# ziyanx02/multiagent-quadruped-environment

Hardware: AMD Instinct MI355X
Metric: env-steps/sec (agents x envs x steps/s), go1gate 4096 envs x 2 agents per GPU (higher is better)
Workload: dtype f32 (policy GEMMs and the actuator network's 32 x 32 layer: 2-plane split-f16, 22-bit)

## Files before the change

### multiagent-quadruped-environment_amd/csrc/kernels_gemm.hpp

```cpp
#pragma once
#include "mqe_common.hpp"

typedef float f32x16 __attribute__((ext_vector_type(16)));

#define GB_M 64
#define GB_N 64
#define GB_K 16

struct GemmArgs {
  const float* A; int lda; int a_rot4; int a_ring4;
  const float* Wt; int ldw;
  const float* bias;
  float* C; int ldc;
  int M, N, K;
  int act_cols;
};

__global__ void __launch_bounds__(256) k_gemm_f32(GemmArgs g) {
  __shared__ float As[GB_K][GB_M + 1];
  __shared__ float Bs[GB_K][GB_N + 4];
  const int tid = threadIdx.x, lane = tid & 63, wave = tid >> 6;
  const int wm = wave >> 1, wn = wave & 1;
  const int ntn = g.N / GB_N, ntm = (g.M + GB_M - 1) / GB_M;
  int bid = blockIdx.x;
  const int total = ntn * ntm;
  {
    const int xcd = bid & 7, slot = bid >> 3;
    const int per = (total + 7) >> 3;
    int lin = xcd * per + slot;
    if ((total & 7) == 0) bid = lin;
  }
  const int tm = bid / ntn, tn = bid - tm * ntn;
  const int m0 = tm * GB_M, n0 = tn * GB_N;
  f32x16 acc;
#pragma unroll
  for (int i = 0; i < 16; i++) acc[i] = 0.0f;
  const int am = tid >> 2, akq = (tid & 3) * 4;
  const int bk = tid >> 4, bnq = (tid & 15) * 4;
  const bool a_ok = (m0 + am) < g.M;
  const float* Arow = g.A + (size_t)(m0 + am) * g.lda;
  float4 av = make_float4(0.f, 0.f, 0.f, 0.f), bv;
  auto load_tile = [&](int k0) {
    if (a_ok) {
      int k4 = (k0 + akq) >> 2;
      if (g.a_ring4) { k4 += g.a_rot4; if (k4 >= g.a_ring4) k4 -= g.a_ring4; }
      av = *reinterpret_cast<const float4*>(Arow + (size_t)k4 * 4);
    }
    bv = *reinterpret_cast<const float4*>(g.Wt + (size_t)(k0 + bk) * g.ldw + n0 + bnq);
  };
  load_tile(0);
  for (int k0 = 0; k0 < g.K; k0 += GB_K) {
    __syncthreads();
    As[akq + 0][am] = av.x; As[akq + 1][am] = av.y; As[akq + 2][am] = av.z; As[akq + 3][am] = av.w;
    *reinterpret_cast<float4*>(&Bs[bk][bnq]) = bv;
    __syncthreads();
    if (k0 + GB_K < g.K) load_tile(k0 + GB_K);
#pragma unroll
    for (int kk = 0; kk < GB_K; kk += 2) {
      float a = As[kk + (lane >> 5)][wm * 32 + (lane & 31)];
      float b = Bs[kk + (lane >> 5)][wn * 32 + (lane & 31)];
      acc = __builtin_amdgcn_mfma_f32_32x32x2f32(a, b, acc, 0, 0, 0);
    }
  }
  const int col = n0 + wn * 32 + (lane & 31);
  const float bias = g.bias ? g.bias[col] : 0.0f;
  const bool do_act = col < g.act_cols;
#pragma unroll
  for (int r = 0; r < 16; r++) {
    int row = m0 + wm * 32 + (r & 3) + 8 * (r >> 2) + 4 * (lane >> 5);
    if (row < g.M) {
      float v = acc[r] + bias;
      if (do_act) v = v > 0 ? v : expm1f(v);
      g.C[(size_t)row * g.ldc + col] = v;
    }
  }
}

typedef _Float16 f16x8 __attribute__((ext_vector_type(8)));
typedef unsigned int h2_u32x4 __attribute__((ext_vector_type(4)));
typedef __attribute__((address_space(1))) h2_u32x4 h2_gvec;

#define H2_M 128
#define H2_N 192
#define H2_K 32
#define H2_KMULT 96
#define H2_THREADS 512
#define H2_ROWB 80
#define H2_ROWS (H2_M + H2_N)
#define H2_PLANE (H2_ROWS * H2_ROWB + 64)
#define H2_BUF (2 * H2_PLANE)
#define H2_LDS_BYTES (3 * H2_BUF)
#define H2_EPS 196
static_assert(H2_M * H2_EPS * 4 <= H2_LDS_BYTES, "epilogue staging");

struct Gemm2Args {
  const uint16_t* A; int lda; int a_rot8, a_ring8;
  const uint16_t* W; int ldw;
  const float* bias;
  float* C; int ldc;
  int M, N, K;
  int act_cols;
  float descale;
  const unsigned* irr; const float* ring; int ring_pos;
  const float* Wt32; int ldwt;
  int full_blocks, full_rows;
  long long* times; int times_blocks;
};
#define H2_STAMP(i) do { if (g.times != nullptr && threadIdx.x == 0 && (int)blockIdx.x < g.times_blocks) {                          \
    g.times[(size_t)blockIdx.x * 16 + 10 + (i)] = (long long)wall_clock64(); g.times[(size_t)blockIdx.x * 16 + 13 + (i)] = (long long)clock64(); } } while (0)
template <int TA>
__device__ __forceinline__ void gemm_h2_tile(const Gemm2Args& g, const int m0, const int n0, unsigned char* lds2) {
  constexpr int HM = 64 * TA;
  const int tid = threadIdx.x, lane = tid & 63, wave = __builtin_amdgcn_readfirstlane(tid >> 6);
  const int wm = (wave >> 1) & 1, wn = wave & 1;
  f32x16 acc00, acc01, acc02, acc10, acc11, acc12;
  H2_STAMP(0);
#pragma unroll
  for (int i = 0; i < 16; i++) { acc00[i] = 0.0f; acc01[i] = 0.0f; acc02[i] = 0.0f; acc10[i] = 0.0f; acc11[i] = 0.0f; acc12[i] = 0.0f; }
  const int stid = tid & 255, srow = stid >> 3, sc = stid & 7, sj = sc >> 1, sp = sc & 1;
  const char* Abase = reinterpret_cast<const char*>(g.A);
  const char* Wbase = reinterpret_cast<const char*>(g.W) + (size_t)n0 * g.ldw * 2;
  const unsigned a_row0 = (unsigned)min(m0 + srow, g.M - 1) * g.lda * 2, a_row1 = (unsigned)min(m0 + 32 + srow, g.M - 1) * g.lda * 2;
  const unsigned a_row2 = TA == 2 ? (unsigned)min(m0 + 64 + srow, g.M - 1) * g.lda * 2 : 0u, a_row3 = TA == 2 ? (unsigned)min(m0 + 96 + srow, g.M - 1) * g.lda * 2 : 0u;
  (void)a_row2; (void)a_row3;
  const unsigned w_row = (unsigned)srow * g.ldw * 2, w_row32 = 32u * g.ldw * 2;
  const unsigned st_ofs = sp * H2_PLANE + srow * H2_ROWB + sj * 16;
  const int frow = lane & 31, fk = (lane >> 5) * 16;
  const unsigned fa_ofs = (wm * 32 * TA + frow) * H2_ROWB + fk, fb_ofs = (H2_M + wn * 96 + frow) * H2_ROWB + fk;
  const int nkt = g.K / H2_K;
  unsigned char* buf0 = lds2;
  unsigned char* buf1 = lds2 + H2_BUF;
  unsigned char* buf2 = lds2 + 2 * H2_BUF;
  h2_u32x4 Pa0, Pa1, Pa2, Pa3, Pw0, Pw1, Pw2, Pw3, Pw4, Pw5;
  h2_u32x4 Qa0, Qa1, Qa2, Qa3, Qw0, Qw1, Qw2, Qw3, Qw4, Qw5;
  h2_u32x4 Ra0, Ra1, Ra2, Ra3, Rw0, Rw1, Rw2, Rw3, Rw4, Rw5;
  h2_u32x4 f0a00, f0a01, f0a10, f0a11, f0b00, f0b01, f0b10, f0b11, f0b20, f0b21;
  h2_u32x4 f1a00, f1a01, f1a10, f1a11, f1b00, f1b01, f1b10, f1b11, f1b20, f1b21;
  unsigned aoff, woff;
#define H2_ADDR(kt_)                                                                                            \
  {                                                                                                             \
    int kc_ = (kt_); if (kc_ > nkt - 1) kc_ = nkt - 1;           \
    woff = w_row + (unsigned)kc_ * 128u + (unsigned)sc * 16u;                                                   \
    int u_ = kc_ * 4 + sj;                                                                                      \
    if (g.a_ring8) { u_ += g.a_rot8; if (u_ >= g.a_ring8) u_ -= g.a_ring8; if (u_ >= g.a_ring8) u_ -= g.a_ring8; } \
    aoff = (unsigned)(u_ * 2 + sp) * 16u;                                                                       \
  }
#ifndef H2_LDA
#define H2_LDA(dst, i_) dst = *(const h2_gvec*)(Abase + a_row##i_ + aoff);
#endif
#ifndef H2_LDW
#define H2_LDW(dst, i_) dst = *(const h2_gvec*)(Wbase + (size_t)(i_) * w_row32 + woff);
#endif
#ifndef H2_ST
#define H2_ST(buf_, src_, r_) *reinterpret_cast<h2_u32x4*>((buf_) + st_ofs + (r_) * H2_ROWB) = src_;
#endif
#define H2_RDA(buf_, p_, t_, ks_) *reinterpret_cast<const h2_u32x4*>((buf_) + fa_ofs + (p_) * H2_PLANE + (t_) * 32 * H2_ROWB + (ks_) * 32)
#define H2_RDB(buf_, p_, u_, ks_) *reinterpret_cast<const h2_u32x4*>((buf_) + fb_ofs + (p_) * H2_PLANE + (u_) * 32 * H2_ROWB + (ks_) * 32)
#define H2_F16(x_) __builtin_bit_cast(f16x8, x_)
#ifndef H2_MFMA
#define H2_MFMA(a_, b_, c_) __builtin_amdgcn_mfma_f32_32x32x16_f16(H2_F16(a_), H2_F16(b_), c_, 0, 0, 0)
#endif
#define H2_PIN() __builtin_amdgcn_sched_barrier(0)
#if defined(H2_STAGER_TIMES) || defined(H2_MULT_TIMES)
  long long ts_prev = clock64(), ts_sum0 = 0, ts_sum1 = 0, ts_sum2 = 0, ts_sum3 = 0, tm_sum0 = 0, tm_sum1 = 0;
#endif
#ifdef H2_STAGER_TIMES
#define H2_TS(n) { const long long c_ = clock64(); ts_sum##n += c_ - ts_prev; ts_prev = c_; }
#define H2_TS_WAITV() asm volatile("s_waitcnt vmcnt(20)" ::: "memory")
#else
#define H2_TS(n)
#define H2_TS_WAITV()
#endif
#ifdef H2_MULT_TIMES
#define H2_TM(n) { const long long c_ = clock64(); tm_sum##n += c_ - ts_prev; ts_prev = c_; }
#else
#define H2_TM(n)
#endif
  if constexpr (TA == 2) {
#include "kernels_gemm_h2_loop.inc"
  } else {
#include "kernels_gemm_h2_loop_half.inc"
  }
#if defined(H2_STAGER_TIMES) || defined(H2_MULT_TIMES)
  if (g.times != nullptr && lane == 0 && (int)blockIdx.x < g.times_blocks) {
    long long* o = g.times + (size_t)blockIdx.x * 16;
    if (wave == 4) { o[0] = ts_sum0; o[1] = ts_sum1; o[2] = ts_sum2; o[3] = ts_sum3; }
    if (wave == 0) { o[4] = tm_sum0; o[5] = tm_sum1; }
  }
#endif
#undef H2_TS
#undef H2_TS_WAITV
#undef H2_TM
#undef H2_ADDR
#undef H2_LDA
#undef H2_LDW
#undef H2_ST
#undef H2_RDA
#undef H2_RDB
#undef H2_F16
#undef H2_MFMA
#undef H2_PIN
  H2_STAMP(1);
  __syncthreads();
  float* ep = reinterpret_cast<float*>(lds2);
#define H2_EPW(acc_, t_, u_)                                                                                    \
  _Pragma("unroll") for (int r = 0; r < 16; r++)                                                                \
    ep[(wm * 32 * TA + (t_) * 32 + (r & 3) + 8 * (r >> 2) + 4 * (lane >> 5)) * H2_EPS + wn * 96 + (u_) * 32 + (lane & 31)] = acc_[r];
  if (wave < 4) {
    H2_EPW(acc00, 0, 0) H2_EPW(acc01, 0, 1) H2_EPW(acc02, 0, 2)
    if constexpr (TA == 2) { H2_EPW(acc10, 1, 0) H2_EPW(acc11, 1, 1) H2_EPW(acc12, 1, 2) }
  }
#undef H2_EPW
  __syncthreads();
  constexpr int EP_IT = (HM * H2_N / 4) / H2_THREADS;
  float4 bbs[EP_IT];
  unsigned mks[EP_IT];
#pragma unroll
  for (int it = 0; it < EP_IT; it++) {
    const int i = it * H2_THREADS + tid, row = i / (H2_N / 4), c4 = i - row * (H2_N / 4);
    bbs[it] = g.bias ? *reinterpret_cast<const float4*>(g.bias + n0 + c4 * 4) : make_float4(0.f, 0.f, 0.f, 0.f);
    mks[it] = g.irr && m0 + row < g.M ? g.irr[m0 + row] : 0u;
  }
#pragma unroll
  for (int it = 0; it < EP_IT; it++) {
    const int i = it * H2_THREADS + tid, row = i / (H2_N / 4), c4 = i - row * (H2_N / 4);
    const int col = n0 + c4 * 4, grow = m0 + row;
    float4 v = *reinterpret_cast<const float4*>(ep + row * H2_EPS + c4 * 4);
    const float4 bb = bbs[it];
    v.x = fmaf(v.x, g.descale, bb.x); v.y = fmaf(v.y, g.descale, bb.y); v.z = fmaf(v.z, g.descale, bb.z); v.w = fmaf(v.w, g.descale, bb.w);
    unsigned mk = mks[it];
    if (mk) {
      float4 cr = make_float4(0.f, 0.f, 0.f, 0.f);
      do {
        const int s1 = __ffs((int)mk) - 1;
        mk &= mk - 1;
        const int p = s1 >= g.ring_pos ? s1 - g.ring_pos : s1 + MQE_HIST - g.ring_pos;
        if (p == 0) continue;
        const int s0 = s1 > 0 ? s1 - 1 : MQE_HIST - 1;
        const float* a2 = g.ring + ((size_t)grow * MQE_HIST + s1) * MQE_FRAME + 54;
        const float* a1 = g.ring + ((size_t)grow * MQE_HIST + s0) * MQE_FRAME + 42;
        const float* wr = g.Wt32 + (size_t)(p * MQE_FRAME + 54) * g.ldwt + col;
#pragma unroll 4
        for (int j = 0; j < 12; j++) {
          const float r = a2[j] - a1[j];
          const float4 w = *reinterpret_cast<const float4*>(wr + (size_t)j * g.ldwt);
          cr.x = fmaf(r, w.x, cr.x); cr.y = fmaf(r, w.y, cr.y); cr.z = fmaf(r, w.z, cr.z); cr.w = fmaf(r, w.w, cr.w);
        }
      } while (mk);
      v.x += cr.x; v.y += cr.y; v.z += cr.z; v.w += cr.w;
    }
    if (col < g.act_cols) {
      v.x = v.x > 0 ? v.x : __expf(v.x) - 1.0f; v.y = v.y > 0 ? v.y : __expf(v.y) - 1.0f;
      v.z = v.z > 0 ? v.z : __expf(v.z) - 1.0f; v.w = v.w > 0 ? v.w : __expf(v.w) - 1.0f;
    }
    if (grow < g.M) {
#ifdef H2_PLAIN_STORE
      *reinterpret_cast<float4*>(g.C + (size_t)grow * g.ldc + col) = v;
#else
      typedef float h2_f4 __attribute__((ext_vector_type(4)));
      h2_f4 nv; nv.x = v.x; nv.y = v.y; nv.z = v.z; nv.w = v.w;
      __builtin_nontemporal_store(nv, reinterpret_cast<h2_f4*>(g.C + (size_t)grow * g.ldc + col));
#endif
    }
  }
  H2_STAMP(2);
}
__global__ void __launch_bounds__(H2_THREADS, 1) k_gemm_h2(Gemm2Args g) {
  extern __shared__ __attribute__((aligned(16))) unsigned char lds2[];
  const int ntn = g.N / H2_N, ntm = (g.M + H2_M - 1) / H2_M;
  int bid = blockIdx.x;
  const int total = ntn * ntm;
  if ((total & 7) == 0) { const int xcd = bid & 7, slot = bid >> 3; bid = xcd * (total >> 3) + slot; }
  const int tm = bid / ntn, tn = bid - tm * ntn;
  gemm_h2_tile<2>(g, tm * H2_M, tn * H2_N, lds2);
}
__global__ void __launch_bounds__(H2_THREADS, 1) k_gemm_h2_mix(Gemm2Args g) {
  extern __shared__ __attribute__((aligned(16))) unsigned char lds2[];
  const int ntn = g.N / H2_N;
  int bid = blockIdx.x;
  if (bid < g.full_blocks) {
    const int total = g.full_blocks;
    if ((total & 7) == 0) { const int xcd = bid & 7, slot = bid >> 3; bid = xcd * (total >> 3) + slot; }
    const int tm = bid / ntn, tn = bid - tm * ntn;
    gemm_h2_tile<2>(g, tm * H2_M, tn * H2_N, lds2);
  } else {
    bid -= g.full_blocks;
    const int total = (int)gridDim.x - g.full_blocks;
    if ((total & 7) == 0) { const int xcd = bid & 7, slot = bid >> 3; bid = xcd * (total >> 3) + slot; }
    const int tm = bid / ntn, tn = bid - tm * ntn;
    gemm_h2_tile<1>(g, g.full_rows + tm * (H2_M / 2), tn * H2_N, lds2);
  }
}
```

### multiagent-quadruped-environment_amd/csrc/kernels_step.hpp

```cpp
#pragma once
#include <type_traits>
#include "mqe_common.hpp"

__device__ __forceinline__ void quat_rotate_inverse_f(const float* q, const float* v, float* o) {
  float qw = q[3];
  float s = 2.0f * qw * qw - 1.0f;
  float cx = q[1] * v[2] - q[2] * v[1], cy = q[2] * v[0] - q[0] * v[2], cz = q[0] * v[1] - q[1] * v[0];
  float dt = q[0] * v[0] + q[1] * v[1] + q[2] * v[2];
  o[0] = v[0] * s - cx * qw * 2.0f + q[0] * dt * 2.0f;
  o[1] = v[1] * s - cy * qw * 2.0f + q[1] * dt * 2.0f;
  o[2] = v[2] * s - cz * qw * 2.0f + q[2] * dt * 2.0f;
}
__device__ __forceinline__ float wrap2pi(float a) {
  const float T = 6.2831855f;
  float r = fmodf(a, T);
  if (r < 0) r += T;
  return r;
}
__device__ __forceinline__ void euler_xyz_f(const float* q, float* rpy) {
  float x = q[0], y = q[1], z = q[2], w = q[3];
  float sinr = 2.0f * (w * x + y * z), cosr = w * w - x * x - y * y + z * z;
  float sinp = 2.0f * (w * y - z * x);
  float siny = 2.0f * (w * z + x * y), cosy = w * w + x * x - y * y - z * z;
  float roll = atan2f(sinr, cosr);
  float pitch = fabsf(sinp) >= 1.0f ? copysignf(1.5707964f, sinp) : asinf(sinp);
  float yaw = atan2f(siny, cosy);
  rpy[0] = wrap2pi(roll); rpy[1] = wrap2pi(pitch); rpy[2] = wrap2pi(yaw);
}

__device__ __forceinline__ float mqe_rand(const DevModel* m, int env, int count, uint32_t k, float lo, float hi) {
  float u = mqe_u01((uint32_t)m->seed, (uint32_t)(env + m->env_id_offset), (uint32_t)count, k);
  return (hi - lo) * u + lo;
}

__device__ __forceinline__ float div_ieee(float a, float b) { return b != 0.0f ? a / b : (a > 0.0f ? 3.0e38f : (a < 0.0f ? -3.0e38f : 0.0f)); }
__device__ __forceinline__ float atan_ratio(float a, float b) { return b != 0.0f ? atanf(a / b) : (a > 0.0f ? 1.5707964f : (a < 0.0f ? -1.5707964f : 0.0f)); }

__device__ __forceinline__ void defender_command_dev(const DevModel* m, const DevState& st, int e, float* cmd3) {
  int A = m->A, P = m->P;
  const float* root = st.root + (size_t)e * (A + P) * 13;
  const float* dp = root + 2 * 13;
  const float* bp = root + A * 13;
  float gate[3] = {as_global(m->gate_pos)[e * 2], as_global(m->gate_pos)[e * 2 + 1], as_global(m->env_origins)[e * 3 + 2]};
  float tp[3];
  for (int k = 0; k < 3; k++) tp[k] = 0.6f * bp[k] + 0.4f * gate[k];
  float yaw = st.obs_bag[(size_t)(e * A + 2) * MQE_OBS_BAG + 5];
  float yaw_to_gate = 3.1415927f + atan_ratio(gate[1] - dp[1], gate[0] - dp[0]);
  float yc = clampf(yaw_to_gate - yaw, -0.3f, 0.3f) / 0.3f;
  float tdg = sqrtf((tp[0] - gate[0]) * (tp[0] - gate[0]) + (tp[1] - gate[1]) * (tp[1] - gate[1]));
  float ddg = sqrtf((dp[0] - gate[0]) * (dp[0] - gate[0]) + (dp[1] - gate[1]) * (dp[1] - gate[1]));
  float xc = clampf(tdg - ddg, -0.5f, 0.5f);
  float yy = -clampf(gate[1] + div_ieee((tp[1] - gate[1]) * (dp[0] - gate[0]), tp[0] - gate[0]) - dp[1], -0.5f, 0.5f);
  cmd3[0] = xc; cmd3[1] = yy; cmd3[2] = yc;
}

__global__ void k_defender_command(const DevModel* m, DevState st, float* out) {
  int e = blockIdx.x * blockDim.x + threadIdx.x;
  if (e >= m->N) return;
  float c[3];
  defender_command_dev(m, st, e, c);
  out[e * 3] = c[0]; out[e * 3 + 1] = c[1]; out[e * 3 + 2] = c[2];
}

__global__ void k_wrapper_command(const DevModel* m, DevState st, const float* __restrict__ actions) {
  int e = blockIdx.x * blockDim.x + threadIdx.x;
  if (e >= m->N) return;
  int A = m->A, Aw = m->Aw;
  const float scale[3] = {2.0f, 0.5f, 0.5f};
  for (int a = 0; a < Aw; a++)
    for (int k = 0; k < 3; k++) {
      float v = actions[((size_t)e * Aw + a) * 3 + k];
      if (m->task != MQE_TASK_TUG) v = clampf(v, -1.0f, 1.0f);
      st.cmd[((size_t)e * A + a) * 3 + k] = m->task == MQE_TASK_PLAIN ? v : v * scale[k];
    }
  if (m->task == MQE_TASK_FOOTBALL_DEFENDER) defender_command_dev(m, st, e, st.cmd + ((size_t)e * A + 2) * 3);
}

struct PreVal { float v, aux; unsigned mk; };
__device__ __forceinline__ PreVal pre_policy_load(const DevModel* m, const DevState& st, const float* __restrict__ command, int hist_slot,
                                                  const float* __restrict__ wrapper_actions, int i, int c) {
  const float* ob = st.obs_bag + (size_t)i * MQE_OBS_BAG;
  PreVal r; r.aux = 0.0f; r.mk = 0u;
  const bool cmd_col = c >= 3 && (c < 6 || (c < 18 && m->cmd_general));
  const float* src = nullptr;
  if (c < 3) src = ob + 60 + c;
  else if (c < 18) src = cmd_col ? nullptr : m->command_obs + c;
  else if (c < 42) src = ob + (c - 12);
  else if (c < 54) src = st.last_loco + (size_t)i * 12 + (c - 42);
  else if (c < 66) src = st.last_two_loco + (size_t)i * 12 + (c - 54);
  else if (c < 70) src = ob + (c - 3);
  float v = src != nullptr ? *src : 0.0f;
  if (cmd_col && m->cmd_general) {
    const int srcc = m->cmd_src[c];
    if (srcc < 0) v = m->command_obs[c];
    else {
      float x = command[(size_t)i * m->cmd_dims + srcc];
      if (m->clip_command) x = clampf(x, -1.0f, 1.0f);
      v = x * m->cmd_scale[c];
    }
  } else if (cmd_col) {
    float x;
    if (wrapper_actions) {
      const int A = m->A, Aw = m->Aw, e = i / A, a = i - e * A, k = c - 3;
      if (m->task == MQE_TASK_FOOTBALL_DEFENDER && a == 2) {
        float c3[3];
        defender_command_dev(m, st, e, c3);
        x = c3[k];
      } else if (a < Aw) {
        float w = wrapper_actions[((size_t)e * Aw + a) * 3 + k];
        if (m->task != MQE_TASK_TUG) w = clampf(w, -1.0f, 1.0f);
        x = m->task == MQE_TASK_PLAIN ? w : w * (k == 0 ? 2.0f : 0.5f);
      } else x = st.cmd[i * 3 + k];
      r.aux = x;
    } else x = command[i * 3 + (c - 3)];
    if (m->clip_command) x = clampf(x, -1.0f, 1.0f);
    v = x * (c < 5 ? m->cmd_lin_scale : m->cmd_ang_scale);
  }
  if (c >= 54 && c < 66 && st.hist2) {
    const int oldest = hist_slot + 1 >= MQE_HIST ? 0 : hist_slot + 1;
    r.aux = st.hist[((size_t)i * MQE_HIST + oldest) * MQE_FRAME + c];
  }
  if (c == 71 && st.hist2) {
    const int prev = hist_slot > 0 ? hist_slot - 1 : MQE_HIST - 1;
    const float* pa = st.hist + ((size_t)i * MQE_HIST + prev) * MQE_FRAME + 42;
    const float* na = st.last_two_loco + (size_t)i * 12;
    unsigned diff = 0;
#pragma unroll
    for (int j = 0; j < 12; j++) diff |= __float_as_uint(pa[j]) ^ __float_as_uint(na[j]);
    const unsigned bit = 1u << hist_slot;
    const unsigned mk = st.hist_irr[i];
    r.mk = diff ? (mk | bit) : (mk & ~bit);
  }
  r.v = v;
  return r;
}
__device__ __forceinline__ void pre_policy_store(const DevModel* m, const DevState& st, int hist_slot, bool have_wrapper_actions, int i, int c, const PreVal& r) {
  const float v = r.v;
  st.loco_obs[(size_t)i * MQE_FRAME + c] = v;
  st.hist[((size_t)i * MQE_HIST + hist_slot) * MQE_FRAME + c] = v;
  if (have_wrapper_actions && c >= 3 && c < 6) st.cmd[i * 3 + (c - 3)] = r.aux;
  if (st.hist2) {
    const int cc = c < 70 ? h2_col(c) : (c == 70 ? MQE_H2_FLAG_COL : -1);
    uint16_t* row2 = st.hist2 + (size_t)i * (2 * MQE_HIST * MQE_H2_FRAME);
    if (cc >= 0) {
      uint16_t h, l;
      split2(c < 70 ? v : 1.0f, MQE_H2_ASCALE, h, l);
      const size_t k = (size_t)hist_slot * MQE_H2_FRAME + cc;
      row2[h2_index(k, 0)] = h; row2[h2_index(k, 1)] = l;
    } else if (cc == -2) {
      const int oldest = hist_slot + 1 >= MQE_HIST ? 0 : hist_slot + 1;
      int slot = oldest + MQE_H2_CARRIER0 + (c - 54); if (slot >= MQE_HIST) slot -= MQE_HIST;
      uint16_t h, l;
      split2(r.aux, MQE_H2_ASCALE, h, l);
      const size_t k = (size_t)slot * MQE_H2_FRAME + MQE_H2_CARRIER_COL;
      row2[h2_index(k, 0)] = h; row2[h2_index(k, 1)] = l;
    } else if (c == 71) st.hist_irr[i] = r.mk;
  }
}
__device__ __forceinline__ void pre_policy_element(const DevModel* m, const DevState& st, const float* __restrict__ command, int hist_slot,
                                                   const float* __restrict__ wrapper_actions, int i, int c) {
  const PreVal r = pre_policy_load(m, st, command, hist_slot, wrapper_actions, i, c);
  pre_policy_store(m, st, hist_slot, wrapper_actions != nullptr, i, c, r);
}

__global__ void __launch_bounds__(256) k_pre_policy(const DevModel* m, DevState st, const float* __restrict__ command, int hist_slot,
                                                    const float* __restrict__ wrapper_actions) {
  const int lane = threadIdx.x & 63;
  const int i = blockIdx.x * (blockDim.x >> 6) + (threadIdx.x >> 6);
  if (i >= m->R) return;
  const int A = m->A, Aw = m->Aw, task = m->task, clip_command = m->clip_command;
  const float lin = m->cmd_lin_scale, ang = m->cmd_ang_scale;
  const int e = i / A, a = i - e * A;
  const bool wrap = wrapper_actions != nullptr;
  if (m->cmd_general || (wrap && task == MQE_TASK_FOOTBALL_DEFENDER && a == 2)) {
    pre_policy_element(m, st, command, hist_slot, wrapper_actions, i, lane);
    if (lane < MQE_FRAME - 64) pre_policy_element(m, st, command, hist_slot, wrapper_actions, i, 64 + lane);
    return;
  }
  const bool h2 = st.hist2 != nullptr;
  const float* ob = st.obs_bag + (size_t)i * MQE_OBS_BAG;
  const int oldest = hist_slot + 1 >= MQE_HIST ? 0 : hist_slot + 1, prev = hist_slot > 0 ? hist_slot - 1 : MQE_HIST - 1;
  const float* hist_i = st.hist + (size_t)i * MQE_HIST * MQE_FRAME;
  const unsigned mk = h2 ? st.hist_irr[i] : 0u;
  float x1[2], x2[2], x3[2], x4[2];
  bool on[2], cmdc[2], actc[2];
  int cc[2];
#pragma unroll
  for (int q = 0; q < 2; q++) {
    const int c = q * 64 + lane;
    cc[q] = c;
    on[q] = c < MQE_FRAME;
    cmdc[q] = c >= 3 && c < 6;
    actc[q] = c >= 54 && c < 66;
    const float* a1 = ob;
    if (c < 3) a1 = ob + 60 + c;
    else if (c < 6) a1 = ob;
    else if (c < 18) a1 = m->command_obs + c;
    else if (c < 42) a1 = ob + (c - 12);
    else if (c < 54) a1 = st.last_loco + (size_t)i * 12 + (c - 42);
    else if (c < 66) a1 = st.last_two_loco + (size_t)i * 12 + (c - 54);
    else if (c < 70) a1 = ob + (c - 3);
    const float* a2 = ob;
    if (cmdc[q]) a2 = wrap ? (a < Aw ? wrapper_actions + ((size_t)e * Aw + a) * 3 + (c - 3) : st.cmd + i * 3 + (c - 3)) : command + i * 3 + (c - 3);
    const float* a3 = ob;
    const float* a4 = ob;
    if (actc[q] && h2) { a3 = hist_i + oldest * MQE_FRAME + c; a4 = hist_i + prev * MQE_FRAME + (c - 12); }
    x1[q] = on[q] ? *a1 : 0.0f; x2[q] = on[q] ? *a2 : 0.0f; x3[q] = on[q] ? *a3 : 0.0f; x4[q] = on[q] ? *a4 : 0.0f;
  }
  PreVal r[2];
  bool differs = false;
#pragma unroll
  for (int q = 0; q < 2; q++) {
    const int c = cc[q];
    float v = (c < 70 && !cmdc[q]) ? x1[q] : 0.0f;
    r[q].aux = 0.0f; r[q].mk = 0u;
    if (cmdc[q]) {
      float x = x2[q];
      if (wrap) {
        if (a < Aw) {
          if (task != MQE_TASK_TUG) x = clampf(x, -1.0f, 1.0f);
          x = task == MQE_TASK_PLAIN ? x : x * (c == 3 ? 2.0f : 0.5f);
        }
        r[q].aux = x;
      }
      if (clip_command) x = clampf(x, -1.0f, 1.0f);
      v = x * (c < 5 ? lin : ang);
    }
    if (actc[q] && h2) {
      r[q].aux = x3[q];
      differs = differs || (on[q] && __float_as_uint(x4[q]) != __float_as_uint(x1[q]));
    }
    r[q].v = v;
  }
  const bool diff = __ballot(differs) != 0ull;
  const unsigned bit = 1u << hist_slot;
  if (lane == MQE_FRAME - 1 - 64) r[1].mk = diff ? (mk | bit) : (mk & ~bit);
  pre_policy_store(m, st, hist_slot, wrap, i, lane, r[0]);
  if (lane < MQE_FRAME - 64) pre_policy_store(m, st, hist_slot, wrap, i, 64 + lane, r[1]);
}

__global__ void k_post_policy(const DevModel* m, DevState st, const float* __restrict__ act, int ld) {
  int idx = blockIdx.x * blockDim.x + threadIdx.x;
  if (idx >= m->R * 12) return;
  int i = idx / 12, k = idx - i * 12;
  float a = act[(size_t)i * ld + k];
  st.last_two_loco[idx] = st.last_loco[idx];
  st.last_loco[idx] = a;
  st.actions[idx] = clampf(a, -m->clip_actions, m->clip_actions);
}

__global__ void k_body_l0_finish(float* __restrict__ P1, int ldp, int col0, int ncols, const float* __restrict__ lat, int ldl,
                                 const float* __restrict__ w_lat0, const float* __restrict__ w_lat1, int R) {
  int idx = blockIdx.x * blockDim.x + threadIdx.x;
  if (idx >= R * ncols) return;
  int i = idx / ncols, c = idx - i * ncols;
  float v = P1[(size_t)i * ldp + col0 + c];
  v = fmaf(lat[(size_t)i * ldl], w_lat0[c], v);
  v = fmaf(lat[(size_t)i * ldl + 1], w_lat1[c], v);
  P1[(size_t)i * ldp + col0 + c] = v > 0 ? v : expm1f(v);
}


struct LagSlots { size_t rd, wr; };
__device__ __forceinline__ LagSlots lag_slots(int pos, int lag_steps, size_t R12, size_t idx) {
  const int rd = pos + 1 >= lag_steps + 1 ? 0 : pos + 1;
  return {(size_t)rd * R12 + idx, (size_t)pos * R12 + idx};
}
__device__ __forceinline__ float lag_target(const DevModel* m, const DevState& st, size_t idx, float as, int pos) {
  if (m->lag_steps <= 0) return as;
  const LagSlots s = lag_slots(pos, m->lag_steps, (size_t)m->R * 12, idx);
  st.lag_buf[s.wr] = as;
  return st.lag_buf[s.rd];
}
__device__ __forceinline__ float joint_pd_torque(int ctrl, float asc, float q, float qd, const float* last_qd, int j, const DevModel* m) {
  float tau = asc;
  if (ctrl == MQE_CTRL_P) tau = m->kp * (asc + m->default_dof_pos[j] - q) - m->kd * qd;
  else if (ctrl == MQE_CTRL_V) tau = m->kp * (asc - qd) - m->kd * (qd - *last_qd) / m->dt;
  return tau;
}
__device__ __forceinline__ void substep_log(const DevModel* m, float* sub_dof_vel, uint8_t* sub_exceed, size_t o, int j, float q, float qd) {
  sub_dof_vel[o] = qd;
  sub_exceed[o] = (uint8_t)((q < m->soft_lo[j]) | (q > m->soft_hi[j]));
}

__global__ void __launch_bounds__(256) k_compute_torques(const DevModel* m, DevState st, int dec_i, int lag_pos) {
  int idx = blockIdx.x * blockDim.x + threadIdx.x;
  int R = m->R, A = m->A;
  if (idx >= R * 12) return;
  int i = idx / 12, j = idx - i * 12;
  int env = i / A, a = i - env * A;
  const float* ds = st.dof + ((size_t)env * m->ND + a * 12 + j) * 2;
  float q = ds[0], qd = ds[1];
  float as = st.actions[idx] * m->action_scale;
  const int ctrl = m->control_type;
  float tau;
  if (ctrl == MQE_CTRL_P || ctrl == MQE_CTRL_V || ctrl == MQE_CTRL_T) tau = joint_pd_torque(ctrl, as, q, qd, st.last_dof_vel + idx, j, m);
  else tau = 0.0f;
  float lim = m->torque_limits[j];
  tau = clampf(tau, -lim, lim);
  st.torques[idx] = tau;
  if (dec_i >= 0) st.sub_tau[((size_t)env * 4 + dec_i) * 12 * A + a * 12 + j] = tau;
}

__global__ void __launch_bounds__(256) k_compute_torques_mfma(const DevModel* m, DevState st, int dec_i, int lag_pos) {
  const int lane = threadIdx.x & 63, wave = threadIdx.x >> 6;
  const int j32 = lane & 31, h = lane >> 5;
  const int R = m->R, A = m->A;
  const int nj = R * 12;
  const int idx = (blockIdx.x * 4 + wave) * 32 + j32;
  const bool valid = idx < nj;
  const int ii = valid ? idx : nj - 1;
  const int i = ii / 12, j = ii - i * 12;
  const int env = i / A, a = i - env * A;
  float* e1 = st.act_hist; float* e2 = e1 + (size_t)R * 12; float* v1 = e2 + (size_t)R * 12; float* v2 = v1 + (size_t)R * 12;
  const float* ds = st.dof + ((size_t)env * m->ND + a * 12 + j) * 2;
  const float q = ds[0], qd = ds[1];
  float as = st.actions[ii] * m->action_scale;
  if (j % 3 == 0) as *= m->hip_scale_reduction;
  const float err = q - (lag_target(m, st, (size_t)ii, as, lag_pos) + m->default_dof_pos[j]);
  const float x1 = e1[ii], x2 = e2[ii], x4 = v1[ii], x5 = v2[ii];
  ActNet w;
  if (m->act_f16) act_load<true>(m, lane, h, w); else act_load<false>(m, lane, h, w);
  const mqe_f32x16 s1 = act_layer1(w, err, x1, x2, qd, x4, x5, h);
  const mqe_f32x16 acc2 = m->act_f16 ? act_layer2<true>(w, s1) : act_layer2<false>(w, s1);
  float tau = act_out(w, acc2);
  if (valid && h == 0) {
    e2[idx] = x1; e1[idx] = err;
    v2[idx] = x4; v1[idx] = qd;
    const float lim = m->torque_limits[j];
    tau = clampf(tau, -lim, lim);
    st.torques[idx] = tau;
    if (dec_i >= 0) st.sub_tau[((size_t)env * 4 + dec_i) * 12 * A + a * 12 + j] = tau;
  }
}


__device__ __forceinline__ unsigned robot_frame(const DevModel* m, const float* rs, const float* gpar, float gi0, const float* f3, float aoz, float dtp,
                                                float* lv, float* av, float* pgr, float* clk, float& gi1, float* rpy) {
  const float q[4] = {rs[3], rs[4], rs[5], rs[6]}, v[3] = {rs[7], rs[8], rs[9]}, w[3] = {rs[10], rs[11], rs[12]};
  const float g3[3] = {0.0f, 0.0f, -1.0f};
  quat_rotate_inverse_f(q, v, lv);
  quat_rotate_inverse_f(q, w, av);
  quat_rotate_inverse_f(q, g3, pgr);
  const float f = gpar[0], ph = gpar[1], off = gpar[2], bnd = gpar[3], dur = gpar[4];
  float gi = gi0 + dtp * f;
  gi = gi - floorf(gi);
  gi1 = gi;
  float fi[4] = {gi + ph + off + bnd, gi + off, gi + bnd, gi + ph};
#pragma unroll
  for (int k = 0; k < 4; k++) {
    const float r = fi[k] - floorf(fi[k]);
    if (r < dur) fi[k] = r * (0.5f / dur);
    else if (r > dur) fi[k] = 0.5f + (r - dur) * (0.5f / (1.0f - dur));
    clk[k] = sinf(6.2831855f * fi[k]);
  }
  unsigned fl = 0;
  if (m->terminate_on_base_contact && sqrtf(f3[0] * f3[0] + f3[1] * f3[1] + f3[2] * f3[2]) > 1.0f) fl |= 1u;
  euler_xyz_f(q, rpy);
  float r = rpy[0], p = rpy[1];
  if (r > 3.1415927f) r -= 6.2831855f;
  if (p > 3.1415927f) p -= 6.2831855f;
  const float z = rs[2] - aoz;
  if ((m->termination_flags & MQE_TERM_ROLL) && fabsf(r) > m->roll_thr) fl |= 2u;
  if ((m->termination_flags & MQE_TERM_PITCH) && fabsf(p) > m->pitch_thr) fl |= 4u;
  if ((m->termination_flags & MQE_TERM_Z_HIGH) && z > m->zhigh_thr) fl |= 8u;
  if ((m->termination_flags & MQE_TERM_Z_LOW) && z < m->zlow_thr) fl |= 16u;
  return fl;
}
__device__ __forceinline__ void env_flags_store(const DevModel* m, const DevState& st, int e, int ep, unsigned fl, uint8_t to, uint8_t reset) {
  st.ep_len[e] = ep;
  st.time_out[e] = to;
  if (m->termination_flags & MQE_TERM_ROLL) st.r_term[e] = (fl >> 1) & 1;
  if (m->termination_flags & MQE_TERM_PITCH) st.p_term[e] = (fl >> 2) & 1;
  if (m->termination_flags & MQE_TERM_Z_HIGH) st.zh_term[e] = (fl >> 3) & 1;
  st.reset_buf[e] = reset;
  st.wdone[e] = reset;
  if (m->terminate_on_base_contact) st.collide_buf[e] = reset;
}
__device__ __forceinline__ void robot_frame_store(const DevState& st, int i, const float* lv, const float* av, const float* pgr, const float* bq, const float* clk, float gi) {
#pragma unroll
  for (int k = 0; k < 3; k++) { st.blv[i * 3 + k] = lv[k]; st.bav[i * 3 + k] = av[k]; st.pg[i * 3 + k] = pgr[k]; }
#pragma unroll
  for (int k = 0; k < 4; k++) { st.bquat[i * 4 + k] = bq[k]; st.clock[i * 4 + k] = clk[k]; }
  st.gait[i] = gi;
}
__device__ __forceinline__ void push_robots(const DevModel* m, float* root, int e, int A, int push_count) {
  for (int b = 0; b < A; b++) {
    float* rv = root + b * 13 + 7;
    rv[0] = mqe_rand(m, e, (int)(MQE_RNG_PUSH + (uint32_t)push_count), (uint32_t)(2 * b), -m->max_push, m->max_push);
    rv[1] = mqe_rand(m, e, (int)(MQE_RNG_PUSH + (uint32_t)push_count), (uint32_t)(2 * b + 1), -m->max_push, m->max_push);
  }
}
__device__ __forceinline__ void obs_row_axis(float* ob, int k, float pos, float origin, float rpy, float lv, float av, float pg) {
  ob[k] = pos - origin; ob[3 + k] = rpy;
  ob[30 + k] = lv * 2.0f; ob[33 + k] = av * 0.25f; ob[60 + k] = pg;
}
__device__ __forceinline__ void obs_row_joint(const DevModel* m, float* ob, int j, float q, float qd, float act, float last_act) {
  ob[6 + j] = (q - m->default_dof_pos[j]) * 1.0f;
  ob[18 + j] = qd * 0.05f;
  ob[36 + j] = act;
  ob[48 + j] = last_act;
}
__device__ __forceinline__ void obs_row_quad(float* ob, int k, float clk, float bq) { ob[63 + k] = clk; ob[67 + k] = bq; }
constexpr int HIST_F4 = MQE_HIST * MQE_FRAME / 4;
constexpr int HIST2_U4 = 2 * MQE_HIST * MQE_H2_FRAME / 8;
__device__ __forceinline__ void zero_env_history(const DevModel* m, const DevState& st, int e, int t, int stride) {
  const int per = m->A * HIST_F4;
  float4* h4 = reinterpret_cast<float4*>(st.hist) + (size_t)e * per;
  for (int k = t; k < per; k += stride) h4[k] = make_float4(0.f, 0.f, 0.f, 0.f);
  if (st.hist2) {
    uint4* p4 = reinterpret_cast<uint4*>(st.hist2 + (size_t)e * m->A * (HIST2_U4 * 8));
    const int per2 = m->A * HIST2_U4;
    for (int k = t; k < per2; k += stride) p4[k] = make_uint4(0u, 0u, 0u, 0u);
#pragma unroll
    for (int a0 = 0; a0 < MQE_MAX_AGENTS; a0 += stride)
      if (t + a0 < m->A) st.hist_irr[(size_t)e * m->A + t + a0] = 0u;
  }
}

__device__ __forceinline__ void compute_observations_env(const DevModel* m, const DevState& st, int e, int in_step) {
  int A = m->A;
  for (int a = 0; a < A; a++) {
    int i = e * A + a;
    float* ob = st.obs_bag + (size_t)i * MQE_OBS_BAG;
    const float* rs = st.root + ((size_t)e * (A + m->P) + a) * 13;
    const float* ds = st.dof + ((size_t)e * m->ND + a * 12) * 2;
    float rpy[3];
    euler_xyz_f(st.bquat + i * 4, rpy);
    for (int k = 0; k < 3; k++) obs_row_axis(ob, k, rs[k], as_global(m->env_origins)[e * 3 + k], rpy[k], st.blv[i * 3 + k], st.bav[i * 3 + k], st.pg[i * 3 + k]);
    for (int j = 0; j < 12; j++) {
      float act = st.actions[i * 12 + j];
      obs_row_joint(m, ob, j, ds[2 * j], ds[2 * j + 1], act, in_step ? act : st.last_actions[i * 12 + j]);
    }
    for (int k = 0; k < 4; k++) obs_row_quad(ob, k, st.clock[i * 4 + k], st.bquat[i * 4 + k]);
  }
}

__global__ void __launch_bounds__(256) k_curriculum_snapshot(const DevModel* m, DevState st) {
  const int e = blockIdx.x * blockDim.x + threadIdx.x;
  if (e >= m->N) return;
  const float* rs = st.root + ((size_t)(e / m->A) * (m->A + m->P) + e % m->A) * 13;
  st.curr_xy[e * 2] = rs[0]; st.curr_xy[e * 2 + 1] = rs[1];
}
__device__ __forceinline__ void curriculum_move_dev(const DevModel* m, const DevState& st, int e) {
  const float dx = st.curr_xy[e * 2] - st.env_origins_live[e * 3], dy = st.curr_xy[e * 2 + 1] - st.env_origins_live[e * 3 + 1];
  const float distance = sqrtf(dx * dx + dy * dy);
  const int move_up = distance > m->terrain_env_length / 2 ? 1 : 0;
  int lvl = st.terrain_levels[e] + move_up;
  if (lvl >= m->terrain_rows) lvl = (int)(mqe_u01((uint32_t)m->seed, (uint32_t)(e + m->env_id_offset), (uint32_t)st.reset_count[e], 250u) * (float)m->terrain_rows);
  else if (lvl < 0) lvl = 0;
  if (lvl >= m->terrain_rows) lvl = m->terrain_rows - 1;
  st.terrain_levels[e] = lvl;
  for (int k = 0; k < 3; k++) st.env_origins_live[e * 3 + k] = as_global(m->terrain_origins)[((size_t)lvl * m->terrain_cols + as_global(m->terrain_types)[e]) * 3 + k];
}

__device__ __forceinline__ void reset_env_dev(const DevModel* m, const DevState& st, int e) {
  int A = m->A, P = m->P;
  float* root = st.root + (size_t)e * (A + P) * 13;
  float* dofs = st.dof + (size_t)e * m->ND * 2;
  int cnt = st.reset_count[e];
  if (m->curriculum) curriculum_move_dev(m, st, e);
  for (int a = 0; a < A; a++)
    for (int j = 0; j < 12; j++) {
      float ratio = mqe_rand(m, e, cnt, (uint32_t)(a * 12 + j), m->dof_ratio_lo, m->dof_ratio_hi);
      dofs[(a * 12 + j) * 2] = m->default_dof_pos[j] * ratio;
      dofs[(a * 12 + j) * 2 + 1] = 0.0f;
    }
  for (int k = 12 * A; k < m->ND; k++) { dofs[k * 2] = m->seesaw_default_angle; dofs[k * 2 + 1] *= 0.0f; }
  for (int a = 0; a < A; a++) {
    float* rs = root + a * 13;
    for (int k = 0; k < 13; k++) rs[k] = as_global(m->base_init)[a * 13 + k];
    for (int k = 0; k < 3; k++) rs[k] += as_global(m->agent_origins)[((size_t)e * A + a) * 3 + k];
  }
  for (int p = 0; p < P; p++) {
    float* rs = root + (A + p) * 13;
    for (int k = 0; k < 13; k++) rs[k] = as_global(m->npc_init)[p * 13 + k];
    for (int k = 0; k < 3; k++) rs[k] += st.env_origins_live[e * 3 + k];
  }
  if (m->has_base_pos_range)
    for (int a = 0; a < A; a++) {
      root[a * 13 + 0] += mqe_rand(m, e, cnt, (uint32_t)(64 + a), m->base_pos_x_lo, m->base_pos_x_hi);
      root[a * 13 + 1] += mqe_rand(m, e, cnt, (uint32_t)(72 + a), m->base_pos_y_lo, m->base_pos_y_hi);
    }
  if (m->has_npc_pos_range)
    for (int p = 0; p < P; p++) {
      root[(A + p) * 13 + 0] += mqe_rand(m, e, cnt, (uint32_t)(128 + p), m->npc_pos_x_lo, m->npc_pos_x_hi);
      root[(A + p) * 13 + 1] += mqe_rand(m, e, cnt, (uint32_t)(160 + p), m->npc_pos_y_lo, m->npc_pos_y_hi);
    }
  for (int a = 0; a < A; a++)
    for (int c = 0; c < 6; c++) root[a * 13 + 7 + c] = mqe_rand(m, e, cnt, (uint32_t)(80 + a * 6 + c), m->base_vel_lo, m->base_vel_hi);
  for (int k = 0; k < 12 * A; k++) st.last_actions[(size_t)e * 12 * A + k] = 0.0f;
  st.ep_len[e] = 0;
  st.reset_buf[e] = 1;
  st.wdone[e] = 1;
  for (int a = 0; a < A; a++) st.gait[e * A + a] = 0.0f;
  st.reset_count[e] = cnt + 1;
}

__device__ __forceinline__ float mqe_randn(const DevModel* m, int e, int step_no, uint32_t k) {
  const uint32_t cnt = MQE_RNG_NPC + (uint32_t)step_no, genv = (uint32_t)(e + m->env_id_offset);
  const float u1 = mqe_u01((uint32_t)m->seed, genv, cnt, 2u * k), u2 = mqe_u01((uint32_t)m->seed, genv, cnt, 2u * k + 1u);
  return sqrtf(-2.0f * logf(1.0f - u1)) * cosf(6.2831855f * u2);
}

typedef const __attribute__((address_space(3))) float* lds_cptr;
template <class NP>
__device__ __forceinline__ void sheep_flock_mean(const DevModel* m, NP npc_rows, float* avg) {
  const int P = m->P;
  avg[0] = 0; avg[1] = 0; avg[2] = 0;
  for (int p = 0; p < P; p++) for (int k = 0; k < 3; k++) avg[k] += npc_rows[p * 13 + k];
  for (int k = 0; k < 3; k++) avg[k] /= (float)P;
}
template <class NP>
__device__ __forceinline__ void sheep_flock_stats(const DevModel* m, const DevState& st, int e, NP npc_rows, const float* avg) {
  const int P = m->P;
  float var = 0;
  for (int k = 0; k < 2; k++) {
    float acc = 0;
    for (int p = 0; p < P; p++) { float t = npc_rows[p * 13 + k] - avg[k]; acc += t * t; }
    var += acc / (float)P;
  }
  st.sheep_avg[e * 2] = avg[0]; st.sheep_avg[e * 2 + 1] = avg[1];
  st.sheep_var[e] = var;
}
template <class NP, class RP>
__device__ __forceinline__ void sheep_increment(const DevModel* m, const DevState& st, int e, int p, NP npc_rows, RP rob_rows, const float* avg, int step_no, float* dv) {
  const int A = m->A, P = m->P;
  NP sp = npc_rows + p * 13;
  for (int k = 0; k < 3; k++) {
    const float z = m->noise_mode == MQE_NOISE_SCRIPTED ? st.npc_noise[((size_t)e * P + p) * 3 + k]
                                                        : (m->sheep_rand != 0.0f ? mqe_randn(m, e, step_no, (uint32_t)(p * 3 + k)) : 0.0f);
    dv[k] = m->sheep_rand * z * 2.0f;
  }
  if (P != 1) {
    float rel[3] = {avg[0] - sp[0], avg[1] - sp[1], avg[2] - sp[2]};
    float nr = sqrtf(rel[0] * rel[0] + rel[1] * rel[1] + rel[2] * rel[2]);
    if (nr > 0.0f) for (int k = 0; k < 3; k++) dv[k] += m->sheep_rand * rel[k] / nr / 1.5f;
  }
  for (int a = 0; a < A; a++) {
    RP dp = rob_rows + a * 13;
    float rel[3] = {sp[0] - dp[0], sp[1] - dp[1], sp[2] - dp[2]};
// ... 211 lines not shown
    }
    if (task == MQE_TASK_GATE || task == MQE_TASK_SHEEP || task == MQE_TASK_PUSHBOX) { o[c++] = gp0; o[c++] = gp1; }
    if (task == MQE_TASK_PUSHBOX) {
      o[c++] = npc[0] - eol[0]; o[c++] = npc[1] - eol[1];
      for (int k = 0; k < 4; k++) o[c++] = npc[3 + k];
    }
    if (task == MQE_TASK_SHEEP)
      for (int p = 0; p < P; p++) { o[c++] = npc[p * 13] - eo0; o[c++] = npc[p * 13 + 1] - eo1; }
    if (task == MQE_TASK_FOOTBALL_DEFENDER) {
      for (int k = 0; k < 3; k++) o[c++] = npc[k] - eol[k];
      for (int k = 0; k < 3; k++) o[c++] = npc[7 + k];
    }
  }
  if (early) return;
  if (task == MQE_TASK_TUG) {
    float* nd = st.dof + ((size_t)e * m->ND + 12 * A) * 2;
    const float npos = nd[0];
    bag_ptr ob0 = bag;
    bag_ptr ob1 = bag + (1) * MQE_OBS_BAG;
    const float x0 = ob0[0], y0 = ob0[1], x1 = ob1[0], y1 = ob1[1];
    if (is_reset_call) {
      st.w_last[e * MQE_MAX_AGENTS] = x0; st.w_last[e * MQE_MAX_AGENTS + 1] = y0;
      st.w_last2[e * 2] = npos;
      st.w_delayed_reset[e] = 0;
      for (int a = 0; a < Aw; a++) rew[a] = 0;
      return;
    }
    const float last_npc = st.w_last2[e * 2];
    const float lx = st.w_last[e * MQE_MAX_AGENTS] - 1.6f, ly = st.w_last[e * MQE_MAX_AGENTS + 1] - npos;
    const float cx = x0 - 1.6f, cy = y0 - npos;
    const float last_dis = sqrtf(lx * lx + ly * ly), dis = sqrtf(cx * cx + cy * cy);
    float r0 = 0.0f, sr = 0.0f, pu = 0.0f, pr = 0.0f, pp = 0.0f;
    if (sc[0] != 0) { if (npos < 0) sr = sc[0] * -npos; if (last_npc <= npos) sr /= 2; r0 += sr; rs[0] += sr; }
    if (sc[1] != 0) { if (npos > 0) pu = sc[1] * npos; if (last_npc > npos) pu /= 2; r0 -= pu; rs[1] += pu; }
    if (sc[2] != 0) { if (dis < last_dis) pr = (last_dis - dis) * sc[2]; r0 += pr; rs[2] += pr; }
    if (sc[3] != 0) { if (dis >= last_dis) pp = powf(2.0f, dis) * sc[3]; r0 -= pp; rs[3] += pp; }
    rs[4] += npos; rs[5] += pr + sr - pu; rs[6] += x0; rs[7] += y0; rs[8] += x1; rs[9] += y1;
    st.w_last[e * MQE_MAX_AGENTS] = x0; st.w_last[e * MQE_MAX_AGENTS + 1] = y0;
    st.w_last2[e * 2] = npos;
    rew[0] = r0;
    for (int a = 1; a < Aw; a++) rew[a] = 0;
    if (side_effects) {
      uint8_t cnt = st.reset_buf[e] ? 2 : st.w_delayed_reset[e];
      if (cnt > 0) { nd[0] = 0.0f; nd[1] = 0.0f; cnt--; }
      st.w_delayed_reset[e] = cnt;
    }
    return;
  }
  if (task == MQE_TASK_BRIDGE) {
    bag_ptr ob0 = bag;
    bag_ptr ob1 = bag + (1) * MQE_OBS_BAG;
    const float x0 = ob0[0], z0 = ob0[2], x1 = ob1[0], z1 = ob1[2];
    float S = st.w_last[e * MQE_MAX_AGENTS], tgt = st.w_last[e * MQE_MAX_AGENTS + 1];
    if (is_reset_call) {
      S = fabsf(x1 + x0); tgt = x1;
      st.w_last[e * MQE_MAX_AGENTS] = S; st.w_last[e * MQE_MAX_AGENTS + 1] = tgt;
    }
    float* o1 = obs + 1 * D;
    o1[0] = S - o1[0]; o1[4] = -o1[4]; o1[6] = S - o1[6]; o1[10] = -o1[10];
    if (is_reset_call) { for (int a = 0; a < Aw; a++) rew[a] = 0; return; }
    float r0 = 0.0f;
    if (sc[0] != 0 && z1 < 0.5f) { r0 += sc[0]; rs[0] += sc[0]; }
    if (sc[1] != 0 && z0 < 0.5f) { r0 -= sc[1]; rs[1] += sc[1]; }
    if (sc[2] != 0 && x0 > tgt) { r0 += sc[2]; rs[2] += sc[2]; }
    rew[0] = r0;
    for (int a = 1; a < Aw; a++) rew[a] = 0;
    return;
  }
  if (task == MQE_TASK_WRESTLING) {
    float* o1 = obs + 1 * D;
    o1[1] = -o1[1]; o1[4] = -o1[4]; o1[7] = -o1[7]; o1[10] = -o1[10];
    if (is_reset_call) { for (int a = 0; a < Aw; a++) rew[a] = 0; return; }
    float r0 = 0.0f;
    bool down0, down1;
    {
      bag_ptr ob = bag;
      float r = ob[3], p = ob[4];
      if (r > 3.1415927f) r -= 6.2831855f;
      if (p > 3.1415927f) p -= 6.2831855f;
      down0 = fabsf(p) > 3.1415927f * 0.9f || fabsf(r) >= 3.1415927f * 0.4f;
      ob += MQE_OBS_BAG;
      r = ob[3]; p = ob[4];
      if (r > 3.1415927f) r -= 6.2831855f;
      if (p > 3.1415927f) p -= 6.2831855f;
      down1 = fabsf(p) > 3.1415927f * 0.9f || fabsf(r) >= 3.1415927f * 0.4f;
    }
    if (sc[0] != 0 && down1) { r0 += sc[0]; rs[0] += sc[0]; }
    if (sc[1] != 0 && down0) { r0 -= sc[1]; rs[1] += sc[1]; }
    rew[0] = r0;
    for (int a = 1; a < Aw; a++) rew[a] = 0;
    return;
  }
  if (task == MQE_TASK_ROTATION) {
    float* o1 = obs + 1 * D;
    o1[1] = -o1[1]; o1[4] = -o1[4]; o1[7] = -o1[7]; o1[10] = -o1[10];
    const float tgt = m->wrapper_param[0];
    bag_ptr ob0 = bag;
    bag_ptr ob1 = bag + (1) * MQE_OBS_BAG;
    const float x0 = ob0[0], y0 = ob0[1], x1 = ob1[0];
    if (is_reset_call) {
      st.w_last[e * MQE_MAX_AGENTS] = sqrtf((x0 - tgt) * (x0 - tgt) + y0 * y0);
      for (int a = 0; a < Aw; a++) rew[a] = 0;
      return;
    }
    float r0 = 0.0f;
    if (sc[0] != 0 && x0 > tgt) { r0 += sc[0]; rs[0] += sc[0]; }
    if (sc[1] != 0 && x1 > tgt) { r0 -= sc[1]; rs[1] += sc[1]; }
    if (sc[2] != 0) {
      const float dis = sqrtf((x0 - tgt) * (x0 - tgt) + (y0 - tgt) * (y0 - tgt));
      if (dis < st.w_last[e * MQE_MAX_AGENTS]) { r0 += sc[2]; rs[2] += sc[2]; }
      st.w_last[e * MQE_MAX_AGENTS] = dis;
    }
    rew[0] = r0;
    for (int a = 1; a < Aw; a++) rew[a] = 0;
    return;
  }
  for (int a = 0; a < Aw; a++) rew[a] = 0;
}

#ifndef POST_EPW
#define POST_EPW 8
#endif

__device__ __forceinline__ void post_flush_rows(float* __restrict__ g, const float* lds, const int n, const int tid) {
  const int n4 = n >> 2;
  for (int i = tid; i < n4; i += 64) reinterpret_cast<float4*>(g)[i] = reinterpret_cast<const float4*>(lds)[i];
  for (int i = (n4 << 2) + tid; i < n; i += 64) g[i] = lds[i];
}

template <int AM, int PEPW, bool LDS_STATE = false>
__device__ __forceinline__ void post_body(const DevModel* m, const DevState& st, const int blk, const int tid, float* s_bag, float* s_la, float* s_npc,
                                          int wrapper_level, int push_count, int step_no,
                                          const float* root_l = nullptr, const float* dof_l = nullptr, const float* act_l = nullptr, int lds_env_stride = 0, int act_env_stride = 0,
                                          const int npc_stride = MQE_MAX_NPCS * 13, long long* taps = nullptr) {
  static_assert(PEPW * AM <= 64 && (PEPW & (PEPW - 1)) == 0, "agent lanes of PEPW envs must fit one wavefront");
#define ETAP(i) do { if (taps != nullptr && tid == 0) taps[i] = (long long)wall_clock64(); } while (0)
  const int A = m->A, P = m->P;
  const int le = tid & (PEPW - 1), a = tid / PEPW;
  const int e = blk * PEPW + le;
  const bool mine = e < m->N && a < A;
  const bool lead = e < m->N && a == 0;
  const int i = e * A + a;
  const int nrow = min(PEPW, m->N - blk * PEPW) * A;
  const float dtp = m->dt * (float)m->decimation;
  float* root = st.root + (size_t)e * (A + P) * 13;
  float* bag = s_bag + le * A * MQE_OBS_BAG;
  typedef typename std::conditional<LDS_STATE, lds_cptr, const float*>::type state_ptr;
  state_ptr root_src;
  if constexpr (LDS_STATE) root_src = (lds_cptr)(root_l + le * lds_env_stride); else root_src = root;
  float* la = s_la + le * A * 12;
  float rs[13], gpar[5], gi0 = 0.f, f3[3], aoz = 0.f, dq[24], act[12], eo[3];
  int ep = 0;
  if (mine) {
    ep = st.ep_len[e] + 1;
#pragma unroll
    for (int k = 0; k < 3; k++) eo[k] = as_global(m->env_origins)[e * 3 + k];
#pragma unroll
    for (int k = 0; k < 13; k++) rs[k] = root_src[a * 13 + k];
    const float* lo = st.loco_obs + (size_t)i * MQE_FRAME;
#pragma unroll
    for (int k = 0; k < 5; k++) gpar[k] = lo[7 + k];
    gi0 = st.gait[i];
    const float* cf3 = st.cf + ((size_t)e * m->NBR + a * MQE_NREP) * 3;
#pragma unroll
    for (int k = 0; k < 3; k++) f3[k] = cf3[k];
    aoz = as_global(m->agent_origins)[(size_t)i * 3 + 2];
    state_ptr ds, as;
    if constexpr (LDS_STATE) { ds = (lds_cptr)(dof_l + le * lds_env_stride + a * 24); as = (lds_cptr)(act_l + le * act_env_stride + a * 12); }
    else { ds = st.dof + ((size_t)e * m->ND + a * 12) * 2; as = st.actions + (size_t)i * 12; }
#pragma unroll
    for (int k = 0; k < 24; k++) dq[k] = ds[k];
#pragma unroll
    for (int k = 0; k < 12; k++) act[k] = as[k];
  }
  float bq[4], lv[3], av[3], pgr[3], clk[4], gi1 = 0.f;
  float rpy[3] = {0.f, 0.f, 0.f};
  unsigned fl = 0;
  if (mine) {
#pragma unroll
    for (int k = 0; k < 4; k++) bq[k] = rs[3 + k];
    fl = robot_frame(m, rs, gpar, gi0, f3, aoz, dtp, lv, av, pgr, clk, gi1, rpy);
  }
  ETAP(2);
#pragma unroll
  for (int d = PEPW; d < PEPW * AM; d <<= 1) fl |= (unsigned)__shfl_xor((int)fl, d);
  const uint8_t to = ep > m->max_episode_length;
  const uint8_t reset = (uint8_t)(mine && (fl != 0 || to));
  if (lead) env_flags_store(m, st, e, ep, fl, to, reset);
  if (mine) robot_frame_store(st, i, lv, av, pgr, bq, clk, gi1);
  ETAP(3);
  float* npc_pre = s_npc + le * npc_stride;
  {
    const int e0 = blk * PEPW, nenv = min(PEPW, m->N - e0), per = P * 13;
    for (int t = tid; t < nenv * per; t += 64) {
      const int sl = t / per, r = t - sl * per;
      if constexpr (LDS_STATE) s_npc[sl * npc_stride + r] = ((lds_cptr)(root_l + sl * lds_env_stride))[A * 13 + r];
      else s_npc[sl * npc_stride + r] = st.root[((size_t)(e0 + sl) * (A + P) + A) * 13 + r];
    }
    __syncthreads();
  }
  ETAP(4);
  if (m->npc_kind == MQE_NPC_SHEEP) {
    constexpr int LPE = 64 / PEPW, NPASS = (MQE_MAX_NPCS + LPE - 1) / LPE;
    float dvs[NPASS][3];
    if (e < m->N) {
      float avg[3];
      sheep_flock_mean(m, (lds_cptr)npc_pre, avg);
      if (lead) sheep_flock_stats(m, st, e, (lds_cptr)npc_pre, avg);
#pragma unroll
      for (int q = 0; q < NPASS; q++)
        if (a + q * LPE < P) sheep_increment(m, st, e, a + q * LPE, (lds_cptr)npc_pre, root_src, avg, step_no, dvs[q]);
    }
    __syncthreads();
    if (e < m->N) {
#pragma unroll
      for (int q = 0; q < NPASS; q++)
        if (a + q * LPE < P) sheep_apply(root, A, a + q * LPE, (lds_cptr)npc_pre, dvs[q]);
    }
    __threadfence_block();
    __syncthreads();
  }
  ETAP(5);
  if (lead) {
    if (reset) {
      reset_env_dev(m, st, e);
      for (int k = 0; k < P * 13; k++) npc_pre[k] = root[A * 13 + k];
    }
  }
  if (__ballot(reset != 0)) {
    __threadfence_block();
    __syncthreads();
    if (reset) {
#pragma unroll
      for (int k = 0; k < 13; k++) rs[k] = root[a * 13 + k];
      const float* ds = st.dof + ((size_t)e * m->ND + a * 12) * 2;
#pragma unroll
      for (int k = 0; k < 24; k++) dq[k] = ds[k];
      if (P == 0) {
#pragma unroll
        for (int k = 0; k < 4; k++) { bq[k] = rs[3 + k]; st.bquat[i * 4 + k] = bq[k]; }
        euler_xyz_f(bq, rpy);
      }
    }
  }
  ETAP(6);
  if (mine) {
    float* ob = bag + a * MQE_OBS_BAG;
#pragma unroll
    for (int k = 0; k < 3; k++) obs_row_axis(ob, k, rs[k], eo[k], rpy[k], lv[k], av[k], pgr[k]);
#pragma unroll
    for (int j = 0; j < 12; j++) obs_row_joint(m, ob, j, dq[2 * j], dq[2 * j + 1], act[j], act[j]);
#pragma unroll
    for (int k = 0; k < 4; k++) obs_row_quad(ob, k, clk[k], bq[k]);
#pragma unroll
    for (int k = 71; k < MQE_OBS_BAG; k++) ob[k] = 0.0f;
#pragma unroll
    for (int j = 0; j < 12; j++) {
      la[a * 12 + j] = act[j];
      la[PEPW * AM * 12 + a * 12 + j] = dq[2 * j + 1];
    }
  }
  __syncthreads();
  ETAP(7);
  if (lead) {
    wrapper_env_dev<true>(m, st, e, 0, npc_pre, wrapper_level, bag);
    if (push_count > 0 && !reset) push_robots(m, root, e, A, push_count);
  }
  ETAP(8);
  {
    const size_t r0 = (size_t)blk * PEPW * A;
    post_flush_rows(st.obs_bag + r0 * MQE_OBS_BAG, s_bag, nrow * MQE_OBS_BAG, tid);
    post_flush_rows(st.last_actions + r0 * 12, s_la, nrow * 12, tid);
    post_flush_rows(st.last_dof_vel + r0 * 12, s_la + PEPW * AM * 12, nrow * 12, tid);
  }
  ETAP(9);
  unsigned long long rm = __ballot(lead && reset != 0);
  while (rm) {
    const int l = __ffsll((long long)rm) - 1;
    rm &= rm - 1;
    zero_env_history(m, st, blk * PEPW + l, tid, 64);
  }
}

template <int AM>
__global__ void __launch_bounds__(64) k_post_physics(const DevModel* m, DevState st, int wrapper_level, int push_count, int step_no) {
  __shared__ float4 s_bag4[POST_EPW * AM * MQE_OBS_BAG / 4], s_la4[POST_EPW * AM * 24 / 4];
  __shared__ float s_npc[POST_EPW * MQE_MAX_NPCS * 13];
  post_body<AM, POST_EPW>(m, st, blockIdx.x, threadIdx.x, reinterpret_cast<float*>(s_bag4), reinterpret_cast<float*>(s_la4), s_npc, wrapper_level, push_count, step_no);
}

__global__ void k_reset_history(const DevModel* m, DevState st) {
  int idx = blockIdx.x * blockDim.x + threadIdx.x;
  int i = idx / HIST_F4;
  if (i >= m->R) return;
  if (!st.reset_buf[i / m->A]) return;
  reinterpret_cast<float4*>(st.hist)[idx] = make_float4(0.f, 0.f, 0.f, 0.f);
  if (st.hist2) {
    const int w = idx - i * HIST_F4;
    if (w < HIST2_U4) reinterpret_cast<uint4*>(st.hist2)[(size_t)i * HIST2_U4 + w] = make_uint4(0u, 0u, 0u, 0u);
    if (w == 0) st.hist_irr[i] = 0u;
  }
}

__global__ void k_hist2_rebuild(const DevModel* m, DevState st, int oldest) {
  const int idx = blockIdx.x * blockDim.x + threadIdx.x;
  const int i = idx / MQE_HIST, slot = idx - i * MQE_HIST;
  if (i >= m->R || !st.hist2) return;
  const float* fr = st.hist + ((size_t)i * MQE_HIST + slot) * MQE_FRAME;
  uint16_t* row2 = st.hist2 + (size_t)i * (2 * MQE_HIST * MQE_H2_FRAME);
  unsigned any = 0u;
  for (int c = 0; c < 70; c++) {
    const float v = fr[c];
    any |= __float_as_uint(v) & 0x7FFFFFFFu;
    const int cc = h2_col(c);
    if (cc >= 0) {
      uint16_t h, l;
      split2(v, MQE_H2_ASCALE, h, l);
      const size_t k = (size_t)slot * MQE_H2_FRAME + cc;
      row2[h2_index(k, 0)] = h; row2[h2_index(k, 1)] = l;
    }
  }
  uint16_t h, l;
  split2(any ? 1.0f : 0.0f, MQE_H2_ASCALE, h, l);
  size_t k = (size_t)slot * MQE_H2_FRAME + MQE_H2_FLAG_COL;
  row2[h2_index(k, 0)] = h; row2[h2_index(k, 1)] = l;
  int p = slot - oldest; if (p < 0) p += MQE_HIST;
  float carry = 0.0f;
  if (p >= MQE_H2_CARRIER0 && p < MQE_H2_CARRIER0 + 12) carry = st.hist[((size_t)i * MQE_HIST + oldest) * MQE_FRAME + 54 + (p - MQE_H2_CARRIER0)];
  split2(carry, MQE_H2_ASCALE, h, l);
  k = (size_t)slot * MQE_H2_FRAME + MQE_H2_CARRIER_COL;
  row2[h2_index(k, 0)] = h; row2[h2_index(k, 1)] = l;
  const int prev = slot > 0 ? slot - 1 : MQE_HIST - 1;
  const float* pa = st.hist + ((size_t)i * MQE_HIST + prev) * MQE_FRAME + 42;
  unsigned diff = 0u;
  for (int j = 0; j < 12; j++) diff |= __float_as_uint(pa[j]) ^ __float_as_uint(fr[54 + j]);
  if (diff) atomicOr(&st.hist_irr[i], 1u << slot);
}

__global__ void __launch_bounds__(64) k_post_staged(const DevModel* m, DevState st, int stages, int wrapper_level, int push_count, int step_no) {
  const int e = blockIdx.x * blockDim.x + threadIdx.x;
  if (e >= m->N) return;
  const int A = m->A, P = m->P;
  float* root = st.root + (size_t)e * (A + P) * 13;
  float* npc_pre = st.npc_pre + (size_t)e * (P ? P : 1) * 13;
  const float dtp = m->dt * (float)m->decimation;
  if (stages & MQE_POST_FRAME) {
    const int ep = st.ep_len[e] + 1;
    unsigned fl = 0;
    for (int a = 0; a < A; a++) {
      const int i = e * A + a;
      float rs[13], lv[3], av[3], pgr[3], clk[4], rpy[3], gi;
      for (int k = 0; k < 13; k++) rs[k] = root[a * 13 + k];
      fl |= robot_frame(m, rs, st.loco_obs + (size_t)i * MQE_FRAME + 7, st.gait[i], st.cf + ((size_t)e * m->NBR + a * MQE_NREP) * 3,
                        as_global(m->agent_origins)[(size_t)i * 3 + 2], dtp, lv, av, pgr, clk, gi, rpy);
      robot_frame_store(st, i, lv, av, pgr, rs + 3, clk, gi);
    }
    const uint8_t to = ep > m->max_episode_length;
    env_flags_store(m, st, e, ep, fl, to, (uint8_t)(fl != 0 || to));
    for (int k = 0; k < P * 13; k++) npc_pre[k] = root[A * 13 + k];
  }
  if ((stages & MQE_POST_NPC) && m->npc_kind == MQE_NPC_SHEEP) {
    float avg[3], dvs[MQE_MAX_NPCS][3];
    const float* nrows = root + A * 13;
    sheep_flock_mean(m, nrows, avg);
    sheep_flock_stats(m, st, e, nrows, avg);
    for (int p = 0; p < P; p++) sheep_increment(m, st, e, p, nrows, (const float*)root, avg, step_no, dvs[p]);
    for (int p = 0; p < P; p++) sheep_apply(root, A, p, nrows, dvs[p]);
  }
  if (stages & MQE_POST_RESET) {
    const uint8_t reset = st.reset_buf[e];
    st.wdone[e] = reset;
    if (m->terminate_on_base_contact) st.collide_buf[e] = reset;
    if (reset) {
      reset_env_dev(m, st, e);
      for (int k = 0; k < P * 13; k++) npc_pre[k] = root[A * 13 + k];
      if (P == 0)
        for (int a = 0; a < A; a++) for (int k = 0; k < 4; k++) st.bquat[(e * A + a) * 4 + k] = root[a * 13 + 3 + k];
      zero_env_history(m, st, e, 0, 1);
    }
  }
  if (stages & MQE_POST_OBS) {
    compute_observations_env(m, st, e, 1);
    for (int k = 0; k < 12 * A; k++) {
      st.last_actions[(size_t)e * 12 * A + k] = st.actions[(size_t)e * 12 * A + k];
      st.last_dof_vel[(size_t)e * 12 * A + k] = st.dof[((size_t)e * m->ND + k) * 2 + 1];
    }
  }
  if (stages & MQE_POST_WRAPPER) {
    wrapper_env_dev(m, st, e, 0, npc_pre, wrapper_level);
    if (push_count > 0 && !st.reset_buf[e]) push_robots(m, root, e, A, push_count);
  }
}

__global__ void __launch_bounds__(64) k_reset_all(const DevModel* m, DevState st, int no_post_step_yet) {
  int e = blockIdx.x * blockDim.x + threadIdx.x;
  if (e >= m->N) return;
  int A = m->A, P = m->P;
  reset_env_dev(m, st, e);
  const float* root = st.root + (size_t)e * (A + P) * 13;
  if (P == 0 || no_post_step_yet)
    for (int a = 0; a < A; a++) for (int k = 0; k < 4; k++) st.bquat[(e * A + a) * 4 + k] = root[a * 13 + 3 + k];
  compute_observations_env(m, st, e, 0);
  st.w_have_last[e] = 0;
  st.w_delayed_reset[e] = 0;
  wrapper_env_dev(m, st, e, 1, root + A * 13);
}

__global__ void __launch_bounds__(64) k_wrapper_eval(const DevModel* m, DevState st, int is_reset_call) {
  int e = blockIdx.x * blockDim.x + threadIdx.x;
  if (e >= m->N) return;
  if (is_reset_call) { st.w_have_last[e] = 0; st.w_delayed_reset[e] = 0; }
  wrapper_env_dev(m, st, e, is_reset_call, st.root + ((size_t)e * (m->A + m->P) + m->A) * 13);
}
```

### multiagent-quadruped-environment_amd/csrc/kernels_tail.hpp

```cpp
#pragma once
#include "mqe_common.hpp"
#include "kernels_gemm.hpp"

#define TL_ROWS 32
#ifndef TL_THREADS
#define TL_THREADS 512
#endif

#define TL_SX (2 * 512 + 16)
#define TL_SY (2 * 256 + 16)
#define TL_SZ (2 * 128 + 16)
#define TL_PX (TL_ROWS * TL_SX)
#define TL_PY (TL_ROWS * TL_SY)
#define TL_PZ (TL_ROWS * TL_SZ)
#define TL_C (64 + 640 + 1024 + 32 * 33)
#define TL_LDS_BYTES (2 * TL_PX + 2 * TL_PY + 2 * TL_PZ + TL_C * 4)
#define TL_ASCALE 1.0f

struct TailLayer { const uint16_t* W; const float* bias; float descale; };

struct TailArgs {
  const float* P1; int ldp; int ada_h0;
  TailLayer a1, a2, b1, b2, b3;
  const float *wl0, *wl1;
  float* lat; int ldl;
  float* act; int lda;
  float *last_loco, *last_two_loco, *actions; float clip_actions;
  int R;
  int block0;
  long long* times;
};
#define TL_STAMP(i) do { if (g.times != nullptr && tid == 0) g.times[(size_t)blockIdx.x * 16 + (i)] = (long long)wall_clock64(); } while (0)

__device__ __forceinline__ float elu_f(float v) { return v > 0 ? v : __expf(v) - 1.0f; }

template <int S, int NT, int D>
struct TlRing { h2_u32x4 w[D][NT][2]; };
template <int S, int NT, int D>
__device__ __forceinline__ void tl_fill(const h2_gvec* Wf, int tile_u4, int krot, TlRing<S, NT, D>& q) {
#pragma unroll
  for (int i = 0; i < D; i++) {
    const int sr = (i + krot) & (S - 1);
#pragma unroll
    for (int t = 0; t < NT; t++) { q.w[i][t][0] = Wf[t * tile_u4 + sr * 128]; q.w[i][t][1] = Wf[t * tile_u4 + sr * 128 + 64]; }
  }
}
template <int S, int NT, int D>
__device__ __forceinline__ void tl_mm(const unsigned char* Ahi, int plane, const h2_gvec* Wf, int tile_u4, int krot, TlRing<S, NT, D>& q, f32x16* acc) {
  h2_u32x4 aq[2][2];
  {
    const int sr = krot & (S - 1);
    aq[0][0] = *reinterpret_cast<const h2_u32x4*>(Ahi + sr * 32); aq[0][1] = *reinterpret_cast<const h2_u32x4*>(Ahi + plane + sr * 32);
  }
#pragma unroll
  for (int s = 0; s < S; s++) {
    if (s + 1 < S) {
      const int sr = (s + 1 + krot) & (S - 1);
      aq[(s + 1) & 1][0] = *reinterpret_cast<const h2_u32x4*>(Ahi + sr * 32);
      aq[(s + 1) & 1][1] = *reinterpret_cast<const h2_u32x4*>(Ahi + plane + sr * 32);
    }
    const f16x8 ah = __builtin_bit_cast(f16x8, aq[s & 1][0]), al = __builtin_bit_cast(f16x8, aq[s & 1][1]);
#pragma unroll
    for (int t = 0; t < NT; t++) {
      const f16x8 wh = __builtin_bit_cast(f16x8, q.w[s % D][t][0]), wl = __builtin_bit_cast(f16x8, q.w[s % D][t][1]);
      acc[t] = __builtin_amdgcn_mfma_f32_32x32x16_f16(ah, wh, acc[t], 0, 0, 0);
      acc[t] = __builtin_amdgcn_mfma_f32_32x32x16_f16(ah, wl, acc[t], 0, 0, 0);
      acc[t] = __builtin_amdgcn_mfma_f32_32x32x16_f16(al, wh, acc[t], 0, 0, 0);
    }
    if (s + D < S) {
      const int sr = (s + D + krot) & (S - 1);
#pragma unroll
      for (int t = 0; t < NT; t++) { q.w[s % D][t][0] = Wf[t * tile_u4 + sr * 128]; q.w[s % D][t][1] = Wf[t * tile_u4 + sr * 128 + 64]; }
    }
    __builtin_amdgcn_sched_barrier(0);
  }
}

__device__ __forceinline__ void tl_store_act(const f32x16& acc, float descale, const float* bias, int col0, unsigned char* out, int stride, int plane, int lane) {
  const int col = col0 + (lane & 31);
  const float b = bias[col];
#pragma unroll
  for (int r = 0; r < 16; r++) {
    const int row = (r & 3) + 8 * (r >> 2) + 4 * (lane >> 5);
    uint16_t h, l;
    split2(elu_f(fmaf(acc[r], descale, b)), TL_ASCALE, h, l);
    *reinterpret_cast<uint16_t*>(out + row * stride + col * 2) = h;
    *reinterpret_cast<uint16_t*>(out + plane + row * stride + col * 2) = l;
  }
}

__global__ void __launch_bounds__(TL_THREADS, 1) k_policy_tail(TailArgs g) {
  constexpr int TLT = TL_THREADS, NW = TLT / 64, NT4 = 8 / NW, QH = 2048 / TLT, QB = 4096 / TLT;
  constexpr int D1 = TLT == 256 ? 16 : 8;
  extern __shared__ __attribute__((aligned(16))) unsigned char tl_lds[];
  unsigned char* X = tl_lds;
  unsigned char* Y = X + 2 * TL_PX;
  unsigned char* Z = Y + 2 * TL_PY;
  float* latS = reinterpret_cast<float*>(Z + 2 * TL_PZ);
  float* bA1 = latS + 64;  float* bA2 = bA1 + 128;  float* bB1 = bA2 + 64;  float* bB2 = bB1 + 256;  float* bB3 = bB2 + 128;
  float* wL0 = bB3 + 64;   float* wL1 = wL0 + 512;  float* nar = wL1 + 512;
  const int tid = threadIdx.x, lane = tid & 63, wave = __builtin_amdgcn_readfirstlane(tid >> 6);
  const int r0 = blockIdx.x * TL_ROWS;
  TL_STAMP(0);
  const int krot = ((blockIdx.x + g.block0) * 7) & 31;
  const int frow = lane & 31, fhalf = lane >> 5;
  const h2_gvec* Wa1 = (const h2_gvec*)(g.a1.W) + lane;
  const h2_gvec* Wa2 = (const h2_gvec*)(g.a2.W) + lane;
  const h2_gvec* Wb1 = (const h2_gvec*)(g.b1.W) + lane;
  const h2_gvec* Wb2 = (const h2_gvec*)(g.b2.W) + lane;
  const h2_gvec* Wb3 = (const h2_gvec*)(g.b3.W) + lane;
  TlRing<16, 1, D1> q1;  TlRing<8, 1, 8> q2;
  if (wave < 4) tl_fill(Wa1 + wave * (16 * 128), 0, krot, q1);
  if (wave == 0) tl_fill(Wa2, 0, 0, q2);
  float4 vh[QH], vb[QB];
#pragma unroll
  for (int q = 0; q < QH; q++) {
    const int idx = tid + TLT * q, row = idx >> 6, k4 = idx & 63;
    vh[q] = *reinterpret_cast<const float4*>(g.P1 + (size_t)min(r0 + row, g.R - 1) * g.ldp + k4 * 4);
  }
#pragma unroll
  for (int q = 0; q < QB; q++) {
    const int idx = tid + TLT * q, row = idx >> 7, k4 = idx & 127;
    vb[q] = *reinterpret_cast<const float4*>(g.P1 + (size_t)min(r0 + row, g.R - 1) * g.ldp + g.ada_h0 + k4 * 4);
  }
  float ll_pre = 0.0f;
  if constexpr (TLT >= TL_ROWS * 12) { const int row = tid / 12; if (tid < TL_ROWS * 12 && r0 + row < g.R) ll_pre = g.last_loco[(size_t)r0 * 12 + tid]; }
  if constexpr (TLT == 512) {
    const float s0 = g.a1.bias[tid & 127], s1 = g.b2.bias[tid & 127], s2 = g.a2.bias[tid & 63], s3 = g.b3.bias[tid & 63], s4 = g.b1.bias[tid & 255],
                s5 = g.wl0[tid], s6 = g.wl1[tid];
    if (tid < 128) { bA1[tid] = s0; bB2[tid] = s1; }
    if (tid < 64) { bA2[tid] = s2; bB3[tid] = s3; }
    if (tid < 256) bB1[tid] = s4;
    wL0[tid] = s5; wL1[tid] = s6;
  } else {
    for (int i = tid; i < 128; i += TLT) { bA1[i] = g.a1.bias[i]; bB2[i] = g.b2.bias[i]; }
    for (int i = tid; i < 64; i += TLT) { bA2[i] = g.a2.bias[i]; bB3[i] = g.b3.bias[i]; }
    for (int i = tid; i < 256; i += TLT) bB1[i] = g.b1.bias[i];
    for (int i = tid; i < 512; i += TLT) { wL0[i] = g.wl0[i]; wL1[i] = g.wl1[i]; }
  }
#pragma unroll
  for (int q = 0; q < QH; q++) {
    const int idx = tid + TLT * q, row = idx >> 6, k4 = idx & 63;
    uint16_t h0, l0, h1, l1, h2, l2, h3, l3;
    split2(vh[q].x, TL_ASCALE, h0, l0); split2(vh[q].y, TL_ASCALE, h1, l1); split2(vh[q].z, TL_ASCALE, h2, l2); split2(vh[q].w, TL_ASCALE, h3, l3);
    *reinterpret_cast<uint2*>(Y + row * TL_SY + k4 * 8) = make_uint2(h0 | ((unsigned)h1 << 16), h2 | ((unsigned)h3 << 16));
    *reinterpret_cast<uint2*>(Y + TL_PY + row * TL_SY + k4 * 8) = make_uint2(l0 | ((unsigned)l1 << 16), l2 | ((unsigned)l3 << 16));
  }
  __syncthreads();
  TL_STAMP(1);
  f32x16 acc[2];
#define TL_ZERO(n_) _Pragma("unroll") for (int t_ = 0; t_ < (n_); t_++) _Pragma("unroll") for (int i_ = 0; i_ < 16; i_++) acc[t_][i_] = 0.0f;
  if (wave < 4) {
    TL_ZERO(1)
    tl_mm(Y + frow * TL_SY + fhalf * 16, TL_PY, Wa1 + wave * (16 * 128), 0, krot, q1, acc);
    tl_store_act(acc[0], g.a1.descale, bA1, wave * 32, Z, TL_SZ, TL_PZ, lane);
  }
#ifndef TL_D4
#define TL_D4 8
#endif
  TlRing<32, NT4, TL_D4> q4;
  tl_fill(Wb1 + (NT4 * wave) * (32 * 128), 32 * 128, krot, q4);
  __syncthreads();
  TL_STAMP(2);
  if (wave == 0) {
    TL_ZERO(1)
    tl_mm(Z + frow * TL_SZ + fhalf * 16, TL_PZ, Wa2, 0, 0, q2, acc);
#pragma unroll
    for (int r = 0; r < 16; r++) nar[((r & 3) + 8 * (r >> 2) + 4 * (lane >> 5)) * 33 + (lane & 31)] = acc[0][r];
  }
  __syncthreads();
  TL_STAMP(3);
  if (tid < TL_ROWS * 2) {
    const int row = tid >> 1, c = tid & 1;
    const float v = fmaf(nar[row * 33 + c], g.a2.descale, bA2[c]);
    latS[row * 2 + c] = v;
    if (r0 + row < g.R) g.lat[(size_t)(r0 + row) * g.ldl + c] = v;
  }
  __syncthreads();
  TL_STAMP(4);
#pragma unroll
  for (int q = 0; q < QB; q++) {
    const int idx = tid + TLT * q, row = idx >> 7, k4 = idx & 127;
    const float4 w0 = *reinterpret_cast<const float4*>(wL0 + k4 * 4), w1 = *reinterpret_cast<const float4*>(wL1 + k4 * 4);
    const float l0 = latS[row * 2], l1 = latS[row * 2 + 1];
    uint16_t h0, q0, h1, q1, h2, q2, h3, q3;
    split2(elu_f(fmaf(l1, w1.x, fmaf(l0, w0.x, vb[q].x))), TL_ASCALE, h0, q0);
    split2(elu_f(fmaf(l1, w1.y, fmaf(l0, w0.y, vb[q].y))), TL_ASCALE, h1, q1);
    split2(elu_f(fmaf(l1, w1.z, fmaf(l0, w0.z, vb[q].z))), TL_ASCALE, h2, q2);
    split2(elu_f(fmaf(l1, w1.w, fmaf(l0, w0.w, vb[q].w))), TL_ASCALE, h3, q3);
    *reinterpret_cast<uint2*>(X + row * TL_SX + k4 * 8) = make_uint2(h0 | ((unsigned)h1 << 16), h2 | ((unsigned)h3 << 16));
    *reinterpret_cast<uint2*>(X + TL_PX + row * TL_SX + k4 * 8) = make_uint2(q0 | ((unsigned)q1 << 16), q2 | ((unsigned)q3 << 16));
  }
  __syncthreads();
  TL_STAMP(5);
  TL_ZERO(NT4)
  tl_mm(X + frow * TL_SX + fhalf * 16, TL_PX, Wb1 + (NT4 * wave) * (32 * 128), 32 * 128, krot, q4, acc);
  TlRing<16, 1, D1> q5;  TlRing<8, 1, 8> q6;
  if (wave < 4) tl_fill(Wb2 + wave * (16 * 128), 0, krot, q5);
  if (wave == 0) tl_fill(Wb3, 0, 0, q6);
#pragma unroll
  for (int t = 0; t < NT4; t++) tl_store_act(acc[t], g.b1.descale, bB1, (NT4 * wave + t) * 32, Y, TL_SY, TL_PY, lane);
  __syncthreads();
  TL_STAMP(6);
  if (wave < 4) {
    TL_ZERO(1)
    tl_mm(Y + frow * TL_SY + fhalf * 16, TL_PY, Wb2 + wave * (16 * 128), 0, krot, q5, acc);
    tl_store_act(acc[0], g.b2.descale, bB2, wave * 32, Z, TL_SZ, TL_PZ, lane);
  }
  __syncthreads();
  TL_STAMP(7);
  if (wave == 0) {
    TL_ZERO(1)
    tl_mm(Z + frow * TL_SZ + fhalf * 16, TL_PZ, Wb3, 0, 0, q6, acc);
#pragma unroll
    for (int r = 0; r < 16; r++) nar[((r & 3) + 8 * (r >> 2) + 4 * (lane >> 5)) * 33 + (lane & 31)] = acc[0][r];
  }
#undef TL_ZERO
  __syncthreads();
  TL_STAMP(8);
  for (int idx = tid; idx < TL_ROWS * 12; idx += TLT) {
    const int row = idx / 12, c = idx - row * 12;
    if (r0 + row >= g.R) continue;
    const float v = fmaf(nar[row * 33 + c], g.b3.descale, bB3[c]);
    const size_t i = (size_t)(r0 + row);
    g.act[i * g.lda + c] = v;
    g.last_two_loco[i * 12 + c] = TLT >= TL_ROWS * 12 ? ll_pre : g.last_loco[i * 12 + c];
    g.last_loco[i * 12 + c] = v;
    g.actions[i * 12 + c] = clampf(v, -g.clip_actions, g.clip_actions);
  }
  TL_STAMP(9);
}
```

### multiagent-quadruped-environment_amd/csrc/mqe_engine.hip

```cpp
#include <hip/hip_runtime.h>

#include <cmath>
#include <cstdio>
#include <cstdlib>
#include <cstring>
#include <string>
#include <vector>

#include "mqe_common.hpp"
#include "kernels_step.hpp"
#include "kernels_tail.hpp"
#include "kernels_gemm.hpp"
#include "kernels_physics.hpp"
#include "kernels_camera.hpp"
#include "kernels_bodies.hpp"

static thread_local char g_err[512] = "";
static int fail(int code, const char* fmt, const char* a = "") {
  snprintf(g_err, sizeof g_err, fmt, a);
  return code;
}
#define HIPCHK(x)                                                        \
  do {                                                                   \
    hipError_t _e = (x);                                                 \
    if (_e != hipSuccess) return fail(-100, "HIP error: %s", hipGetErrorString(_e)); \
  } while (0)

enum SwitchKind { SW_FLAG, SW_INT };
enum SwitchId { SW_VERBOSE, SW_LANE_SWEEP, SW_PHYS_LDS_PAD, SW_ACT_F32, SW_ENVS_PER_WAVE, SW_NO_FUSE_SUBSTEPS, SW_NO_FUSE_POST, SW_DEBUG_STOP_PHASE,
                SW_GEMM_SPLIT, SW_GEMM_HALF, SW_NO_FUSED_TAIL, SW_TAIL_TIMES, SW_WAVE_TIMES, SW_PHASE_TIMES, SW_COUNT };
static const struct { const char* name; SwitchKind kind; } SWITCH_LIST[SW_COUNT] = {
  {"MQE_VERBOSE", SW_FLAG}, {"MQE_LANE_SWEEP", SW_FLAG}, {"MQE_PHYS_LDS_PAD", SW_INT}, {"MQE_ACT_F32", SW_FLAG}, {"MQE_ENVS_PER_WAVE", SW_INT},
  {"MQE_NO_FUSE_SUBSTEPS", SW_FLAG}, {"MQE_NO_FUSE_POST", SW_FLAG}, {"MQE_DEBUG_STOP_PHASE", SW_INT}, {"MQE_GEMM_SPLIT", SW_INT},
  {"MQE_GEMM_HALF", SW_INT}, {"MQE_NO_FUSED_TAIL", SW_FLAG}, {"MQE_TAIL_TIMES", SW_FLAG}, {"MQE_WAVE_TIMES", SW_FLAG}, {"MQE_PHASE_TIMES", SW_FLAG},
};
struct Switches {
  const char* text[SW_COUNT];
  int value[SW_COUNT];
  bool set(int id) const { return text[id] != nullptr; }
};
static Switches read_switches() {
  Switches sw;
  for (int i = 0; i < SW_COUNT; i++) {
    sw.text[i] = getenv(SWITCH_LIST[i].name);
    sw.value[i] = (sw.text[i] && SWITCH_LIST[i].kind == SW_INT) ? atoi(sw.text[i]) : 0;
  }
  return sw;
}

struct GemmLayer {
  float* Wt;
  float* bias;
  int K, N, Kpad, Npad;
  uint16_t* W2 = nullptr;
  float wscale = 1.0f;
  uint16_t* Wfrag = nullptr;
  float fscale = 1.0f;
  int Kpad3 = 0;
  std::vector<float> hW;
};

enum { PROF_GEMM_L0 = 0, PROF_GEMM_REST, PROF_TORQUES, PROF_SIMULATE, PROF_POST, PROF_MISC, PROF_N };

struct ShapeRow;
typedef void (*substeps_fn_t)(const DevModel*, DevState, int, int, PostArgs);
struct mqe_sim {
  mqe_sim_desc d;
  Switches sw;
  DevModel hm;
  DevModel* dm = nullptr;
  DevState st;
  std::vector<void*> allocs;
  std::vector<std::pair<void*, size_t>> state_bufs;
  bool reg_state = false;
  void* tens[MQE_T_COUNT];
  int N, A, P, R, ND, NBR, Aw, D;
  int hist_pos = 0, n_post_steps = 0;
  const ShapeRow* shape = nullptr;
  substeps_fn_t substeps_fn = nullptr;
  int substeps_epw = 1;
  int lag_pos = 0;
  GemmLayer l0;
  std::vector<GemmLayer> ada_rest, body_rest;
  float *w_lat0 = nullptr, *w_lat1 = nullptr;
  int ada_h0, body_h0;
  float *P1 = nullptr, *bufA = nullptr, *bufB = nullptr, *lat = nullptr, *act_out = nullptr;
  int ldP1, ldbuf, ldlat, ldact;
  bool gemm_split = false;
  bool gemm_half = true;
  bool cmd_general = false;
  bool phase_timed = false;
  bool tail_fused = false;
  long long* tail_times = nullptr;
  size_t phys_lds_bytes = 0;
  bool fuse_substeps = true;
  bool fuse_post = true;
  int dbg_stop_phase = -1;
  float* rbs = nullptr;
  bool rbs_refresh = false;
  RbsArgs rbs_args;
  bool prof = false, prof_now = false;
  int step_open = 0;
  int prof_every = 1; long prof_step = 0;
  std::vector<hipEvent_t> ev0[PROF_N], ev1[PROF_N];
  float prof_ms[PROF_N];
  int prof_cnt[PROF_N];
};

extern "C" const char* mqe_last_error(void) { return g_err; }
extern "C" int mqe_abi_version(void) { return MQE_ABI_VERSION; }
extern "C" int mqe_abi_limits(int32_t* out, int n) {
  const int32_t v[] = {MQE_ABI_VERSION, MQE_MAX_AGENTS, MQE_MAX_NPCS, MQE_MAX_SPHERES, MQE_MAX_PRIMS, MQE_MAX_SELF_PAIRS, MQE_MAX_LAYERS, MQE_MAX_REWARD_TERMS,
                       MQE_NBODY, MQE_NREP, MQE_NDOF, MQE_FRAME, MQE_HIST, MQE_T_COUNT};
  const int cnt = (int)(sizeof v / sizeof v[0]);
  for (int i = 0; i < cnt && i < n; i++) out[i] = v[i];
  return cnt;
}
extern "C" int mqe_sizeof_desc(void) { return (int)sizeof(mqe_sim_desc); }

template <typename T>
static int dalloc(mqe_sim* s, T** p, size_t n, int fill_zero = 1) {
  void* q = nullptr;
  size_t bytes = (n ? n : 1) * sizeof(T);
  if (hipMalloc(&q, bytes) != hipSuccess) return -1;
  if (fill_zero && hipMemset(q, 0, bytes) != hipSuccess) return -1;
  s->allocs.push_back(q);
  if (s->reg_state) s->state_bufs.push_back({q, bytes});
  *p = (T*)q;
  return 0;
}
static int upload(mqe_sim* s, const float** dst, const float* src, size_t n) {
  if (!src || !n) { *dst = nullptr; return 0; }
  float* q;
  if (dalloc(s, &q, n, 0)) return -1;
  if (hipMemcpy(q, src, n * 4, hipMemcpyHostToDevice) != hipSuccess) return -1;
  *dst = q;
  return 0;
}
static inline int rup(int v, int m) { return (v + m - 1) / m * m; }

static int make_layer(mqe_sim* s, GemmLayer* L, int K, int N) {
  L->K = K; L->N = N; L->Kpad = rup(K, GB_K); L->Npad = rup(N, GB_N); L->Kpad3 = rup(K, H2_KMULT);
  L->hW.assign((size_t)L->Npad * L->Kpad3, 0.0f);
  if (dalloc(s, &L->Wt, (size_t)L->Kpad * L->Npad)) return -1;
  if (dalloc(s, &L->bias, L->Npad)) return -1;
  return 0;
}
static int fill_layer(GemmLayer* L, int col0, const float* W, const float* b, int out, int in_used, int ldw_in,
                      const std::vector<int>* krow = nullptr, const std::vector<int>* k2row = nullptr, const std::vector<float>* k2scale = nullptr) {
  std::vector<float> tmp((size_t)L->Kpad * out, 0.0f);
  std::vector<double> acc;
  if (k2row) acc.assign((size_t)out * L->Kpad3, 0.0);
  for (int o = 0; o < out; o++)
    for (int k = 0; k < in_used; k++) {
      int kr = krow ? (*krow)[k] : k;
      tmp[(size_t)kr * out + o] = W[(size_t)o * ldw_in + k];
      if (k2row) acc[(size_t)o * L->Kpad3 + (*k2row)[k]] += (double)W[(size_t)o * ldw_in + k] * (double)(*k2scale)[k];
      else L->hW[(size_t)(col0 + o) * L->Kpad3 + kr] = W[(size_t)o * ldw_in + k];
    }
  if (k2row)
    for (int o = 0; o < out; o++)
      for (int k = 0; k < L->Kpad3; k++) L->hW[(size_t)(col0 + o) * L->Kpad3 + k] = (float)acc[(size_t)o * L->Kpad3 + k];
  if (hipMemcpy2D(L->Wt + col0, (size_t)L->Npad * 4, tmp.data(), (size_t)out * 4, (size_t)out * 4, L->Kpad, hipMemcpyHostToDevice) != hipSuccess) return -1;
  if (b && hipMemcpy(L->bias + col0, b, (size_t)out * 4, hipMemcpyHostToDevice) != hipSuccess) return -1;
  return 0;
}

static bool weight_scale(const std::vector<float>& w, float* scale) {
  float wmax = 0.0f;
  for (float v : w) wmax = std::max(wmax, std::fabs(v));
  if (!(wmax < 1e30f)) return false;
  int e = wmax > 0.0f ? (int)std::floor(std::log2(32768.0f / wmax)) : 0;
  e = std::min(std::max(e, -100), 100);
  *scale = std::ldexp(1.0f, e);
  return true;
}
static int finalize_layer(mqe_sim* s, GemmLayer* L) {
  const size_t n = (size_t)L->Npad * L->Kpad3;
  if (!weight_scale(L->hW, &L->wscale)) return -1;
  std::vector<uint16_t> pl(2 * n);
  for (int r = 0; r < L->Npad; r++)
    for (int k = 0; k < L->Kpad3; k++) {
      uint16_t* row = pl.data() + (size_t)r * 2 * L->Kpad3;
      split2(L->hW[(size_t)r * L->Kpad3 + k], L->wscale, row[h2_index(k, 0)], row[h2_index(k, 1)]);
    }
  if (dalloc(s, &L->W2, 2 * n, 0)) return -1;
  if (hipMemcpy(L->W2, pl.data(), 2 * n * 2, hipMemcpyHostToDevice) != hipSuccess) return -1;
  L->hW.clear(); L->hW.shrink_to_fit();
  return 0;
}

static int finalize_frag(mqe_sim* s, GemmLayer* L) {
  if (L->K % 16 || L->Npad % 32) return -1;
  if (!weight_scale(L->hW, &L->fscale)) return -1;
  const int S = L->K / 16, CT = L->Npad / 32;
  std::vector<uint16_t> pl((size_t)CT * S * 2 * 512);
  for (int ct = 0; ct < CT; ct++)
    for (int st = 0; st < S; st++)
      for (int l = 0; l < 64; l++)
        for (int q = 0; q < 8; q++) {
          const int col = ct * 32 + (l & 31), k = st * 16 + (l >> 5) * 8 + q;
          uint16_t h, lo;
          split2(L->hW[(size_t)col * L->Kpad3 + k], L->fscale, h, lo);
          const size_t blk = ((size_t)ct * S + st) * 2;
          pl[(blk + 0) * 512 + l * 8 + q] = h;
          pl[(blk + 1) * 512 + l * 8 + q] = lo;
        }
  if (dalloc(s, &L->Wfrag, pl.size(), 0)) return -1;
  if (hipMemcpy(L->Wfrag, pl.data(), pl.size() * 2, hipMemcpyHostToDevice) != hipSuccess) return -1;
  return 0;
}

enum SubShape { SH_A2, SH_A1, SH_A2_NOPAD, SH_A2_LINK, SH_A2_NPC_FEW, SH_A2_BOX_FEW, SH_A2_STATIC_FEW, SH_A3_NPC_ROW, SH_A2_NPC, SH_A4_NPC, SH_A2_GEN, SH_GEN, SH_COUNT };
struct ShapeRow {
  const char* name;
  substeps_fn_t fn[2];
  substeps_fn_t timed;
  bool epilogue;
  bool fuse_post;
  bool pairs;
  bool a2;
};
[[maybe_unused]] static constexpr substeps_fn_t TIMED_ORDER[] = {k_substeps<2, 0, 1, true>, k_substeps<2, PS_F_NPC, 1, true>, k_substeps<3, PS_F_NPC | PS_F_ROW, 1, true>};
template <int TA, int TP, bool ACT32, bool TIMED = false>
constexpr ShapeRow shape_row(const char* name, bool fuse_post = true) {
  constexpr bool pairs = TP == 0 && (TA == 1 || TA == 2);
  constexpr bool epilogue = ShapeClass<TP>::small || TP > 0;
  ShapeRow r = {name, {nullptr, nullptr}, nullptr, epilogue, epilogue && fuse_post, pairs, TA == 2 && TP == 0};
  if constexpr (pairs) r.fn[1] = k_substeps<TA, TP, 2, false, ACT32>;
  r.fn[0] = k_substeps<TA, TP, 1, false, ACT32>;
  if constexpr (TIMED && !ACT32) r.timed = k_substeps<TA, TP, 1, true>;
  return r;
}
template <bool ACT32>
static const ShapeRow* shape_row_of(SubShape sh) {
  static constexpr ShapeRow rows[] = {
    shape_row<2, 0, ACT32, true>("SH_A2"),
    shape_row<1, 0, ACT32>("SH_A1"),
    shape_row<2, PS_F_FEW, ACT32>("SH_A2_NOPAD"),
    shape_row<2, PS_F_LINK, ACT32>("SH_A2_LINK"),
    shape_row<2, PS_F_NPC | PS_F_FEW, ACT32>("SH_A2_NPC_FEW"),
    shape_row<2, PS_F_NPC | PS_F_BOX | PS_F_FEW, ACT32>("SH_A2_BOX_FEW"),
    shape_row<2, PS_F_STATIC | PS_F_FEW, ACT32>("SH_A2_STATIC_FEW"),
    shape_row<3, PS_F_NPC | PS_F_ROW, ACT32, true>("SH_A3_NPC_ROW", false),
    shape_row<2, PS_F_NPC, ACT32, true>("SH_A2_NPC"),
    shape_row<4, PS_F_NPC, ACT32>("SH_A4_NPC"),
    shape_row<2, -1, ACT32>("SH_A2_GEN"),
    shape_row<0, -1, ACT32>("SH_GEN"),
  };
  static_assert(sizeof rows / sizeof rows[0] == SH_COUNT, "one row per SubShape, in its order");
  return &rows[sh];
}
static SubShape pick_shape(const DevModel& m, size_t lds_bytes, int pad) {
  const int feat = (m.has_seesaw ? PS_F_LINK : 0) | (m.n_npc_dyn > 0 ? PS_F_NPC : 0) | (m.has_box ? PS_F_BOX : 0) | (m.n_static > 0 ? PS_F_STATIC : 0);
  if (m.rowgs && lds_bytes <= 10240 && m.maxc <= 32 && m.A + m.n_npc_dyn + (m.has_seesaw ? 1 : 0) <= 4) {
    if (feat == 0 && m.P == 0 && pad) {
      if (m.A == 2) return SH_A2;
      if (m.A == 1) return SH_A1;
    }
    if (feat == 0 && m.P == 0 && !pad && m.A == 2) return SH_A2_NOPAD;
    if (m.A == 2 && feat == PS_F_LINK) return SH_A2_LINK;
    if (m.A == 2 && feat == PS_F_NPC) return SH_A2_NPC_FEW;
    if (m.A == 2 && feat == (PS_F_NPC | PS_F_BOX)) return SH_A2_BOX_FEW;
    if (m.A == 2 && feat == PS_F_STATIC) return SH_A2_STATIC_FEW;
  }
  if (m.A == 3 && feat == PS_F_NPC && m.rowgs && m.maxc <= 32 && m.A + m.n_npc_dyn <= 4) return SH_A3_NPC_ROW;
  if (m.A == 2 && feat == PS_F_NPC && m.rowgs) return SH_A2_NPC;
  if (m.A == 4 && feat == PS_F_NPC && m.rowgs) return SH_A4_NPC;
  if (m.A == 2) return SH_A2_GEN;
  return SH_GEN;
}

static int wrapper_dims(const mqe_sim_desc* d, int* Aw, int* D) {
  int A = d->num_agents, P = d->num_npcs;
  switch (d->task) {
    case MQE_TASK_GATE: *Aw = A; *D = 14 + A; break;
    case MQE_TASK_SHEEP: *Aw = A; *D = 14 + 2 * P + A; break;
    case MQE_TASK_SEESAW: *Aw = A; *D = 12 + A; break;
    case MQE_TASK_FOOTBALL_DEFENDER: *Aw = 2; *D = 20; break;
    case MQE_TASK_PUSHBOX: *Aw = A; *D = 20 + A; break;
    case MQE_TASK_ROTATION: case MQE_TASK_BRIDGE: case MQE_TASK_WRESTLING: *Aw = A; *D = 12; break;
    case MQE_TASK_TUG: *Aw = A; *D = 10; break;
    default: *Aw = A; *D = 6 + A; break;
  }
  return 0;
}

static void h2_tiling(int M, int ntn, bool use_half, int* full_tiles, int* half_tiles) {
  const int ntm = (M + H2_M - 1) / H2_M, per_round = 256 / ntn > 0 ? 256 / ntn : 1;
  const int rem = ntm % per_round;
  *full_tiles = ntm; *half_tiles = 0;
  if (use_half && rem != 0 && 2 * rem <= per_round) {
    *full_tiles = ntm - rem;
    *half_tiles = (M - *full_tiles * H2_M + H2_M / 2 - 1) / (H2_M / 2);
  }
}
static const double L0_H2_ROUND_US = 80.0, L0_F32_US_AT_8192 = 255.0;
static bool l0_split_is_faster(int R, int ntn, bool half_tiles) {
  int ft = 0, ht = 0;
  h2_tiling(R, ntn, half_tiles, &ft, &ht);
  const double rounds = std::ceil(ft * (double)ntn / 256.0) + (ht ? 0.6 : 0.0);
  return rounds * L0_H2_ROUND_US < L0_F32_US_AT_8192 * R / 8192.0;
}

static size_t packed_floats(const mqe_sim* s) { return (size_t)s->N * s->Aw * s->D + (size_t)s->N * s->Aw + (s->N + 3) / 4; }
static void set_packed(mqe_sim* s, float* base) {
  s->st.wobs = base;
  s->st.wrew = base + (size_t)s->N * s->Aw * s->D;
  s->st.wdone = (uint8_t*)(s->st.wrew + (size_t)s->N * s->Aw);
}

#define UP(dst, src, n) if (upload(s, &(dst), (src), (n))) { return fail(-5, "device upload failed"); }
#define DA(p, n) if (dalloc(s, &(p), (n))) return fail(-5, "device alloc failed");

static int check_create_args(const mqe_sim_desc* d, mqe_sim** out) {
  if (!d || !out) return fail(-1, "null argument");
  if (d->abi_version != MQE_ABI_VERSION) return fail(-1, "abi version mismatch");
  if (d->num_agents < 1 || d->num_agents > MQE_MAX_AGENTS)
    return fail(-2, "num_agents must be 1 .. 4: one env is one 64-lane wavefront in the physics kernel (a body per lane: 13 per Go1 + the NPCs), a fifth robot does not fit");
  if (d->num_npcs < 0 || d->num_npcs > MQE_MAX_NPCS) return fail(-2, "num_npcs must be 0 .. 16 (MQE_MAX_NPCS)");
  int ndev = 0;
  if (hipGetDeviceCount(&ndev) != hipSuccess || ndev == 0) return fail(-3, "no HIP device: the engine has no CPU path");
  return 0;
}

static int stage_model(mqe_sim* s) {
  const mqe_sim_desc* d = &s->d;
  const int N = s->N = d->num_envs, A = s->A = d->num_agents, P = s->P = d->num_npcs;
  const int R = s->R = N * A;
  const int seesaw = d->npc_kind == MQE_NPC_SEESAW;
  s->ND = 12 * A + (seesaw ? P : 0);
  s->NBR = MQE_NREP * A + (seesaw ? 2 * P : (d->npc_kind == MQE_NPC_STATIC ? d->npc_reported_bodies * P : P));
  wrapper_dims(d, &s->Aw, &s->D);
  memset(s->tens, 0, sizeof s->tens);
  memset(s->prof_ms, 0, sizeof s->prof_ms);
  memset(s->prof_cnt, 0, sizeof s->prof_cnt);
  DevModel& m = s->hm;
  memset(&m, 0, sizeof m);
  m.N = N; m.A = A; m.P = P; m.R = R; m.ND = s->ND; m.NBR = s->NBR; m.Aw = s->Aw; m.D = s->D;
  m.npc_kind = d->npc_kind; m.task = d->task;
  m.n_npc_dyn = (d->npc_kind == MQE_NPC_BALL || d->npc_kind == MQE_NPC_SHEEP || d->npc_kind == MQE_NPC_BOX) ? P : 0;
  m.self_collision = d->self_collision != 0 && d->robot.n_self_pairs > 0;
  m.lag_steps = (d->control_type == MQE_CTRL_C && d->lag_timesteps > 0) ? d->lag_timesteps : 0; m.max_push = d->max_push_vel_xy;
  m.has_box = d->npc_kind == MQE_NPC_BOX; m.cap_npc = d->npc_contact_cap > 0 ? d->npc_contact_cap : 2;
  memcpy(m.npc_box_half, d->npc_box_half, sizeof m.npc_box_half);
  m.npc_lin_only = d->npc_kind == MQE_NPC_SHEEP;
  m.npc_dofs_each = seesaw ? 1 : (m.npc_lin_only ? 3 : 6);
  m.env_id_offset = d->env_id_offset; m.seed = d->seed; m.noise_mode = d->noise_mode;
  m.dt = d->dt; m.decimation = d->decimation; m.gravity_z = d->gravity_z; m.solver_iterations = d->solver_iterations;
  m.contact_offset = d->contact_offset; m.max_depen = d->max_depenetration_velocity; m.friction = d->friction; m.erp = d->erp;
  m.solver_type = d->solver_type == 1 ? 1 : 0; m.vel_iters = d->velocity_iterations > 0 ? d->velocity_iterations : 0;
  if (m.solver_type == 1 && d->solver_iterations < 1) return fail(-6, "solver_type = 1 (temporal Gauss-Seidel) needs num_position_iterations >= 1: its sub-step is dt / n");
  if (d->solver_iterations < 0 || d->solver_iterations > 64) return fail(-6, "solver_iterations out of range (0 .. 64)");
  m.robot = d->robot;
  m.npc_mass = d->npc_mass; m.npc_inertia = d->npc_inertia; m.npc_n_spheres = d->npc_n_spheres;
  memcpy(m.npc_sphere_center, d->npc_sphere_center, sizeof m.npc_sphere_center);
  memcpy(m.npc_sphere_radius, d->npc_sphere_radius, sizeof m.npc_sphere_radius);
  m.seesaw_default_angle = d->seesaw_default_angle;
  m.n_static = d->npc_kind == MQE_NPC_STATIC ? d->n_static_boxes : 0;
  memcpy(m.sb_center, d->static_box_center, sizeof m.sb_center); memcpy(m.sb_half, d->static_box_half, sizeof m.sb_half);
  m.has_seesaw = seesaw; m.ss_axis = (d->seesaw_axis == 2 || d->seesaw_axis == 3) ? d->seesaw_axis : 1; m.ss_link_cyl = d->seesaw_link_cylinder;
  memcpy(m.ss_joint_offset, d->seesaw_joint_offset, 12); memcpy(m.ss_plank_center, d->seesaw_plank_center, 12);
  memcpy(m.ss_plank_half, d->seesaw_plank_half, 12); memcpy(m.ss_base_half, d->seesaw_base_half, 12);
  m.ss_inertia = d->seesaw_plank_inertia_yy; m.ss_vel_limit = d->seesaw_vel_limit;
  m.ss_col_radius = d->seesaw_column_radius; m.ss_col_length = d->seesaw_column_length;
  m.ss_theta_lo = d->seesaw_theta_lo; m.ss_theta_hi = d->seesaw_theta_hi;
  m.control_type = d->control_type; m.action_scale = d->action_scale; m.hip_scale_reduction = d->hip_scale_reduction;
  m.clip_actions = d->clip_actions; memcpy(m.torque_limits, d->torque_limits, sizeof m.torque_limits);
  m.kp = d->kp; m.kd = d->kd; memcpy(m.default_dof_pos, d->default_dof_pos, sizeof m.default_dof_pos);
  memcpy(m.command_obs, d->command_obs, sizeof m.command_obs);
  m.cmd_lin_scale = d->cmd_lin_scale; m.cmd_ang_scale = d->cmd_ang_scale; m.clip_command = d->clip_command;
  m.cmd_dims = d->num_command_dims; m.cmd_general = d->num_command_dims != 3;
  for (int c = 0; c < 18; c++) {
    m.cmd_src[c] = d->command_src[c]; m.cmd_scale[c] = d->command_scale[c];
    if (d->command_src[c] >= d->num_command_dims) return fail(-6, "command_src points past num_command_dims");
    if (d->command_src[c] != (c >= 3 && c < 6 ? c - 3 : -1)) m.cmd_general = 1;
  }
  if (d->num_command_dims < 1) return fail(-6, "num_command_dims must be >= 1");
  s->cmd_general = m.cmd_general != 0;
  m.sdf_nx = d->sdf_nx; m.sdf_ny = d->sdf_ny; m.hs = d->horizontal_scale; m.wall_height = d->wall_height; m.ground_z = d->ground_z;
  m.termination_flags = d->termination_flags; m.terminate_on_base_contact = d->terminate_on_base_contact; m.max_episode_length = d->max_episode_length;
  m.roll_thr = d->roll_threshold; m.pitch_thr = d->pitch_threshold; m.zlow_thr = d->z_low_threshold; m.zhigh_thr = d->z_high_threshold;
  m.dof_ratio_lo = d->dof_ratio_lo; m.dof_ratio_hi = d->dof_ratio_hi; m.has_base_pos_range = d->has_base_pos_range; m.has_npc_pos_range = d->has_npc_pos_range;
  m.base_pos_x_lo = d->base_pos_x_lo; m.base_pos_x_hi = d->base_pos_x_hi; m.base_pos_y_lo = d->base_pos_y_lo; m.base_pos_y_hi = d->base_pos_y_hi;
  m.npc_pos_x_lo = d->npc_pos_x_lo; m.npc_pos_x_hi = d->npc_pos_x_hi; m.npc_pos_y_lo = d->npc_pos_y_lo; m.npc_pos_y_hi = d->npc_pos_y_hi;
  m.base_vel_lo = d->base_vel_lo; m.base_vel_hi = d->base_vel_hi;
  m.sheep_scale = d->sheep_movement_scale; m.sheep_rand = d->sheep_movement_randomness;
  memcpy(m.reward_scale, d->reward_scale, sizeof m.reward_scale); memcpy(m.wrapper_param, d->wrapper_param, sizeof m.wrapper_param);
  m.nbody_env = A * MQE_NBODY + m.n_npc_dyn;
  m.ndof_env = A * MQE_RD + m.n_npc_dyn * m.npc_dofs_each + (seesaw ? 1 : 0);
  m.nsph_env = A * d->robot.n_spheres + m.n_npc_dyn * d->npc_n_spheres;
  m.nprim_env = A * d->robot.n_prims;
  m.feat_sphere_mask = 0ull;
  for (int f = 0; f < d->robot.n_spheres; f++)
    if (d->robot.prim_type[d->robot.sphere_prim[f]] == MQE_PRIM_SPHERE) m.feat_sphere_mask |= 1ull << f;
  if (d->robot.n_spheres > MQE_MAX_SPHERES || d->robot.n_prims > MQE_MAX_PRIMS || d->robot.n_self_pairs > MQE_MAX_SELF_PAIRS) return fail(-6, "robot model: too many feature points / primitives / self-collision pairs");
  m.maxc = mqe_maxc(A, P, m.cap_npc);
  if (mqe_maxc_uncapped(A, P, m.cap_npc) > 64) return fail(-4, "the per-actor contact caps of this scene (8 per robot + cap per NPC + 8 two-actor slots) exceed the 64 contact lanes of the wavefront that owns an env");
  if (m.ndof_env > 128 || m.nbody_env > 64) { return fail(-4, "env has more than 64 bodies or 128 generalized velocities: does not fit one wavefront"); }
  return 0;
}

static int choose_epw(const mqe_sim* s) {
  const bool can = s->shape->pairs && 2 * s->phys_lds_bytes <= 64 * 1024 && s->d.robot.n_spheres <= 32;
  int want = (s->A == 1 && s->N >= 4096) ? 2 : 1;
  if (s->sw.set(SW_ENVS_PER_WAVE)) want = s->sw.value[SW_ENVS_PER_WAVE];
  return (can && want == 2) ? 2 : 1;
}
static void choose_fusion(mqe_sim* s, const PhysLds& L) {
  const Switches& sw = s->sw;
  s->fuse_substeps = !sw.set(SW_NO_FUSE_SUBSTEPS) && s->d.decimation <= 4;
  s->fuse_post = s->fuse_substeps && !sw.set(SW_NO_FUSE_POST) && s->shape->fuse_post;
  if (!s->fuse_post) return;
  const int epw = s->substeps_epw, amp = (s->A == 1 || s->A == 2) ? 2 : MQE_MAX_AGENTS;
  const int need = post_staging_floats(epw, amp, 12 * s->A, s->P);
  const int room = (epw == 1 ? L.total : L.total + L.root) - L.body;
  if (need > room) {
    if (sw.set(SW_VERBOSE)) fprintf(stderr, "mqe: post-physics epilogue needs %d floats of staging, the layout has %d: separate launch\n", need, room);
    s->fuse_post = false;
  }
}
static int stage_variant(mqe_sim* s) {
  const mqe_sim_desc* d = &s->d;
  const Switches& sw = s->sw;
  DevModel& m = s->hm;
  const int A = s->A, P = s->P;
  m.rowgs = 1;
  if (sw.set(SW_LANE_SWEEP)) m.rowgs = 0;
  int pad = (m.rowgs && m.P == 0 && !m.has_seesaw && m.n_npc_dyn == 0 && !m.has_box && m.n_static == 0 && (A == 1 || A == 2)) ? 1 : 0;
  PhysLds L = phys_lds_layout(A, P, s->ND, m.nbody_env, m.ndof_env, m.nsph_env, m.nprim_env, m.maxc, m.rowgs, pad);
  if (pad && (size_t)L.total * 4 > 10240) {
    pad = 0;
    L = phys_lds_layout(A, P, s->ND, m.nbody_env, m.ndof_env, m.nsph_env, m.nprim_env, m.maxc, m.rowgs, pad);
  }
  s->phys_lds_bytes = (size_t)L.total * 4;
  if (sw.set(SW_VERBOSE)) fprintf(stderr, "mqe: physics LDS %zu B per env (wavefront)\n", s->phys_lds_bytes);
  s->phys_lds_bytes += (size_t)sw.value[SW_PHYS_LDS_PAD];
  if ((L.total | L.body | L.sph | L.prim | L.con | L.side | L.leg | L.legc | L.basei | L.sinv | L.fcol | L.acc | L.rhs | L.phi | L.srec | L.wacc) & 3) { return fail(-4, "physics LDS layout: a 16 B record area is misaligned"); }
  if (s->phys_lds_bytes > 160 * 1024) { return fail(-4, "physics LDS footprint exceeds 160 KiB"); }
  {
    float w1max = 0.0f;
    if (d->actuator.n_layers == 3 && d->actuator.dims[1] == 32 && d->actuator.dims[2] == 32 && d->actuator.W[1])
      for (int i = 0; i < 32 * 32; i++) w1max = std::max(w1max, std::fabs(d->actuator.W[1][i]));
    m.act_f16 = (!sw.set(SW_ACT_F32) && w1max < 3.99f) ? 1 : 0;
  }
  const bool act32 = m.act_f16 == 0;
  const SubShape sh = pick_shape(m, s->phys_lds_bytes, pad);
  s->shape = act32 ? shape_row_of<true>(sh) : shape_row_of<false>(sh);
  s->substeps_epw = choose_epw(s);
  s->substeps_fn = s->shape->fn[s->substeps_epw - 1];
  if (sw.set(SW_PHASE_TIMES) && s->shape->timed && s->substeps_epw == 1) { s->substeps_fn = s->shape->timed; s->phase_timed = true; }
  {
    const size_t lds_sub = s->phys_lds_bytes * (size_t)s->substeps_epw;
    if (s->phys_lds_bytes > 48 * 1024 && hipFuncSetAttribute((const void*)k_simulate, hipFuncAttributeMaxDynamicSharedMemorySize, (int)s->phys_lds_bytes) != hipSuccess)
      return fail(-4, "cannot raise dynamic LDS limit");
    if (lds_sub > 48 * 1024 && hipFuncSetAttribute((const void*)s->substeps_fn, hipFuncAttributeMaxDynamicSharedMemorySize, (int)lds_sub) != hipSuccess)
      return fail(-4, "cannot raise dynamic LDS limit");
  }
  choose_fusion(s, L);
  if (sw.set(SW_DEBUG_STOP_PHASE)) {
    if (!s->shape->a2) { return fail(-4, "MQE_DEBUG_STOP_PHASE applies to two-robot scenes without objects only (k_simulate_a2)"); }
    s->dbg_stop_phase = sw.value[SW_DEBUG_STOP_PHASE];
  }
  if (sw.set(SW_VERBOSE)) {
    fprintf(stderr, "mqe: k_substeps runs %d env(s) per wavefront\n", s->substeps_epw);
    fprintf(stderr, "mqe: variant shape=%s epw=%d actuator=%s post=%s\n", s->shape->name, s->substeps_epw, act32 ? "f32" : "f16", s->fuse_post ? "fused" : "separate");
    for (int i = 0; i < SW_COUNT; i++)
      if (sw.set(i)) fprintf(stderr, "mqe: override in effect: %s=%s\n", SWITCH_LIST[i].name, sw.text[i]);
  }
  return 0;
}

static int stage_scene(mqe_sim* s) {
  const mqe_sim_desc* d = &s->d;
  DevModel& m = s->hm;
  const int N = s->N, A = s->A, P = s->P;
  UP(m.wall_sdf, d->wall_sdf, (size_t)d->sdf_nx * d->sdf_ny);
  UP(m.ground_height, d->ground_height, (size_t)d->sdf_nx * d->sdf_ny);
  UP(m.wall_top, d->wall_top, (size_t)d->sdf_nx * d->sdf_ny);
  if (d->edge_contacts & ~15) return fail(-6, "edge_contacts: bits 1 (wall edges), 2 (capsule axes against the scene's boxes), 4 (box edges against box primitives) and 8 (manifold reduction to the deepest contacts)");
  m.edge_mask = d->edge_contacts & 15;
  m.wall_corner = nullptr;
  if ((m.edge_mask & 1) && d->wall_corner) { UP(m.wall_corner, d->wall_corner, (size_t)d->sdf_nx * d->sdf_ny * 2); }
  for (int q = 0; q < MQE_MAX_PRIMS; q++) {
    m.prim_feat_t[q][0] = m.prim_feat_t[q][1] = -9.0f;
    if (q >= d->robot.n_prims || d->robot.prim_type[q] != MQE_PRIM_CAPSULE) continue;
    const float* ax = d->robot.prim_axis[q];
    const float aa = ax[0] * ax[0] + ax[1] * ax[1] + ax[2] * ax[2];
    int k = 0;
    for (int f = 0; f < d->robot.n_spheres && aa > 0.0f; f++)
      if (d->robot.sphere_prim[f] == q) {
        const float df[3] = {d->robot.sphere_center[f][0] - d->robot.prim_center[q][0], d->robot.sphere_center[f][1] - d->robot.prim_center[q][1], d->robot.sphere_center[f][2] - d->robot.prim_center[q][2]};
        const float tf = 0.5f + 0.5f * (df[0] * ax[0] + df[1] * ax[1] + df[2] * ax[2]) / aa;
        if (tf > -0.05f && tf < 1.05f && k < 2) m.prim_feat_t[q][k++] = tf;
      }
  }
  {
    const float soft = d->soft_dof_pos_limit > 0.0f ? d->soft_dof_pos_limit : 1.0f;
    for (int j = 0; j < MQE_NDOF; j++) {
      const float mid = (d->robot.dof_lower[j] + d->robot.dof_upper[j]) / 2, r = d->robot.dof_upper[j] - d->robot.dof_lower[j];
      m.soft_lo[j] = mid - 0.5f * r * soft; m.soft_hi[j] = mid + 0.5f * r * soft;
    }
  }
  UP(m.env_origins, d->env_origins, (size_t)N * 3);
  UP(m.agent_origins, d->agent_origins, (size_t)N * A * 3);
  m.curriculum = d->terrain_curriculum ? 1 : 0; m.terrain_rows = d->terrain_num_rows; m.terrain_cols = d->terrain_num_cols; m.terrain_env_length = d->terrain_env_length;
  m.terrain_origins = nullptr; m.terrain_types = nullptr;
  if (m.curriculum) {
    if (d->env_id_offset != 0) return fail(-6, "terrain curriculum: not defined for a shard of a larger batch (row e of the agents' root states belongs to another shard's env)");
    if (!d->terrain_origins || !d->terrain_levels || !d->terrain_types || d->terrain_num_rows < 1 || d->terrain_num_cols < 1) return fail(-6, "terrain curriculum: origin table / levels / types missing");
    UP(m.terrain_origins, d->terrain_origins, (size_t)d->terrain_num_rows * d->terrain_num_cols * 3);
    const float* tt = nullptr;
    UP(tt, reinterpret_cast<const float*>(d->terrain_types), (size_t)N);
    m.terrain_types = reinterpret_cast<const int32_t*>(tt);
  }
  UP(m.base_init, d->base_init_state, (size_t)A * 13);
  UP(m.npc_init, d->npc_init_state, (size_t)P * 13);
  UP(m.gate_pos, d->gate_pos, (size_t)N * 2);
  return 0;
}

static int stage_actuator(mqe_sim* s) {
  const mqe_sim_desc* d = &s->d;
  DevModel& m = s->hm;
  m.actuator.n_layers = d->actuator.n_layers;
  memcpy(m.actuator.dims, d->actuator.dims, sizeof m.actuator.dims);
  if (d->actuator.n_layers != 3 || d->actuator.dims[0] != 6 || d->actuator.dims[1] != 32 || d->actuator.dims[2] != 32 || d->actuator.dims[3] != 1)
    return fail(-6, "actuator network must be 6-32-32-1 (unitree_go1.pt)");
  for (int l = 0; l < 3; l++) UP(m.actuator.b[l], d->actuator.b[l], (size_t)d->actuator.dims[l + 1]);
  UP(m.actuator.W[2], d->actuator.W[2], (size_t)d->actuator.dims[2] * d->actuator.dims[3]);
  {
    std::vector<float> fr((size_t)19 * 64);
    for (int lane = 0; lane < 64; lane++) {
      const int j32 = lane & 31, h = lane >> 5;
      for (int r = 0; r < 16; r++) fr[(size_t)r * 64 + lane] = d->actuator.W[1][j32 * 32 + (r & 3) + 8 * (r >> 2) + 4 * h];
      for (int s2 = 0; s2 < 3; s2++) fr[(size_t)(16 + s2) * 64 + lane] = d->actuator.W[0][j32 * 6 + 2 * s2 + h];
    }
    UP(m.act_frag, fr.data(), fr.size());
    std::vector<uint16_t> f16((size_t)2 * 2 * 64 * 8);
    for (int s2 = 0; s2 < 2; s2++)
      for (int lane = 0; lane < 64; lane++)
        for (int i8 = 0; i8 < 8; i8++) {
          const int row = lane & 31, g = lane >> 5, u = (i8 & 3) + 16 * s2 + 8 * (i8 >> 2) + 4 * g;
          uint16_t hh, ll;
          split2(d->actuator.W[1][row * 32 + u], 16384.0f, hh, ll);
          f16[((size_t)(s2 * 2 + 0) * 64 + lane) * 8 + i8] = hh;
          f16[((size_t)(s2 * 2 + 1) * 64 + lane) * 8 + i8] = ll;
        }
    const float* t16;
    UP(t16, reinterpret_cast<const float*>(f16.data()), f16.size() / 2);
    m.act_frag16 = reinterpret_cast<const uint16_t*>(t16);
  }
  return 0;
}

static int stage_policy(mqe_sim* s) {
  const mqe_sim_desc* d = &s->d;
  const Switches& sw = s->sw;
  const int R = s->R;
  const mqe_mlp& ad = d->adaptation; const mqe_mlp& bd = d->body;
  if (ad.dims[0] != 2100 || bd.dims[0] != 2102 || bd.dims[bd.n_layers] != 12 || ad.dims[ad.n_layers] != 2)
    return fail(-6, "policy I/O must be adaptation 2100->2, body 2102->12 (go1.py:395,404,29)");
  s->ada_h0 = ad.dims[1]; s->body_h0 = bd.dims[1];
  if (s->ada_h0 % GB_N || s->body_h0 % GB_N) return fail(-6, "first hidden sizes must be multiples of 64");
  std::vector<int> krow(2100);
  for (int k = 0; k < 2100; k++) krow[k] = (k / 70) * MQE_FRAME + (k % 70);
  std::vector<int> k2row(2100);
  std::vector<float> k2scale(2100);
  for (int k = 0; k < 2100; k++) {
    const int f = k / 70, c = k % 70, cc = h2_col(c);
    if (cc == -2) k2row[k] = f > 0 ? (f - 1) * MQE_H2_FRAME + h2_col(c - 12) : (MQE_H2_CARRIER0 + c - 54) * MQE_H2_FRAME + MQE_H2_CARRIER_COL;
    else k2row[k] = f * MQE_H2_FRAME + (cc >= 0 ? cc : MQE_H2_FLAG_COL);
    k2scale[k] = cc == -1 ? d->command_obs[c] : 1.0f;
  }
  if (make_layer(s, &s->l0, MQE_HIST * MQE_FRAME, s->ada_h0 + s->body_h0)) return fail(-5, "alloc");
  s->l0.Kpad3 = rup(MQE_HIST * MQE_H2_FRAME, H2_KMULT);
  s->l0.hW.assign((size_t)s->l0.Npad * s->l0.Kpad3, 0.0f);
  if (fill_layer(&s->l0, 0, ad.W[0], ad.b[0], s->ada_h0, 2100, 2100, &krow, &k2row, &k2scale)) return fail(-5, "upload");
  if (fill_layer(&s->l0, s->ada_h0, bd.W[0], bd.b[0], s->body_h0, 2100, 2102, &krow, &k2row, &k2scale)) return fail(-5, "upload");
  {
    std::vector<float> w0(s->body_h0), w1(s->body_h0);
    for (int o = 0; o < s->body_h0; o++) { w0[o] = bd.W[0][(size_t)o * 2102 + 2100]; w1[o] = bd.W[0][(size_t)o * 2102 + 2101]; }
    const float* t;
    UP(t, w0.data(), w0.size()); s->w_lat0 = (float*)t;
    UP(t, w1.data(), w1.size()); s->w_lat1 = (float*)t;
  }
  s->gemm_half = !sw.set(SW_GEMM_HALF) || sw.value[SW_GEMM_HALF] != 0;
  const bool split = sw.set(SW_GEMM_SPLIT) ? sw.value[SW_GEMM_SPLIT] != 0 : l0_split_is_faster(R, s->l0.Npad / H2_N > 0 ? s->l0.Npad / H2_N : 1, s->gemm_half);
  s->gemm_split = s->l0.Npad % H2_N == 0 && split && !s->cmd_general;
  if (s->gemm_split) {
    if (finalize_layer(s, &s->l0)) return fail(-5, "upload");
    if (hipFuncSetAttribute((const void*)k_gemm_h2, hipFuncAttributeMaxDynamicSharedMemorySize, H2_LDS_BYTES) != hipSuccess ||
        hipFuncSetAttribute((const void*)k_gemm_h2_mix, hipFuncAttributeMaxDynamicSharedMemorySize, H2_LDS_BYTES) != hipSuccess)
      return fail(-4, "cannot raise dynamic LDS limit");
  }
  for (int l = 1; l < ad.n_layers; l++) {
    GemmLayer g;
    if (make_layer(s, &g, ad.dims[l], ad.dims[l + 1]) || fill_layer(&g, 0, ad.W[l], ad.b[l], ad.dims[l + 1], ad.dims[l], ad.dims[l])) return fail(-5, "upload");
    s->ada_rest.push_back(g);
  }
  for (int l = 1; l < bd.n_layers; l++) {
    GemmLayer g;
    if (make_layer(s, &g, bd.dims[l], bd.dims[l + 1]) || fill_layer(&g, 0, bd.W[l], bd.b[l], bd.dims[l + 1], bd.dims[l], bd.dims[l])) return fail(-5, "upload");
    s->body_rest.push_back(g);
  }
  s->tail_fused = !sw.set(SW_NO_FUSED_TAIL) && ad.n_layers == 3 && bd.n_layers == 4 && ad.dims[1] == 256 && ad.dims[2] == 128 &&
                  bd.dims[1] == 512 && bd.dims[2] == 256 && bd.dims[3] == 128;
  if (s->tail_fused) {
    if (hipFuncSetAttribute((const void*)k_policy_tail, hipFuncAttributeMaxDynamicSharedMemorySize, TL_LDS_BYTES) != hipSuccess)
      return fail(-4, "cannot raise dynamic LDS limit");
    for (auto& g : s->ada_rest) if (finalize_frag(s, &g)) return fail(-5, "upload");
    for (auto& g : s->body_rest) if (finalize_frag(s, &g)) return fail(-5, "upload");
  }
  if (s->tail_fused && sw.set(SW_TAIL_TIMES)) { if (dalloc(s, &s->tail_times, (size_t)16 * ((R + TL_ROWS - 1) / TL_ROWS))) return fail(-5, "alloc"); }
  return 0;
}

static int stage_work_buffers(mqe_sim* s) {
  const int R = s->R;
  int maxw = 64;
  for (auto& g : s->ada_rest) maxw = std::max(maxw, g.Npad);
  for (auto& g : s->body_rest) maxw = std::max(maxw, g.Npad);
  s->ldP1 = s->l0.Npad; s->ldbuf = maxw; s->ldlat = 64; s->ldact = 64;
  DA(s->P1, (size_t)R * s->ldP1); DA(s->bufA, (size_t)R * s->ldbuf); DA(s->bufB, (size_t)R * s->ldbuf);
  DA(s->lat, (size_t)R * s->ldlat); DA(s->act_out, (size_t)R * s->ldact);
  return 0;
}

static int stage_state(mqe_sim* s) {
  const mqe_sim_desc* d = &s->d;
  const int N = s->N, A = s->A, P = s->P, R = s->R;
  DevState& st = s->st;
  s->reg_state = true;
  DA(st.root, (size_t)N * (A + P) * 13); DA(st.dof, (size_t)N * s->ND * 2); DA(st.cf, (size_t)N * s->NBR * 3);
  DA(st.torques, (size_t)N * 12 * A); DA(st.actions, (size_t)N * 12 * A); DA(st.last_actions, (size_t)N * 12 * A);
  DA(st.loco_obs, (size_t)R * MQE_FRAME); DA(st.hist, (size_t)R * MQE_HIST * MQE_FRAME);
  st.hist2 = nullptr;
  st.hist_irr = nullptr;
  st.wave_times = nullptr;
  if (s->sw.set(SW_WAVE_TIMES) || s->sw.set(SW_PHASE_TIMES)) { DA(st.wave_times, (size_t)(4 + 64 + 16) * N); }
  if (s->gemm_split) { DA(st.hist2, (size_t)2 * R * MQE_HIST * MQE_H2_FRAME); DA(st.hist_irr, (size_t)R); }
  DA(st.last_loco, (size_t)R * 12); DA(st.last_two_loco, (size_t)R * 12); DA(st.act_hist, (size_t)4 * R * 12);
  DA(st.gait, R); DA(st.clock, (size_t)R * 4); DA(st.blv, (size_t)R * 3); DA(st.bav, (size_t)R * 3); DA(st.pg, (size_t)R * 3);
  DA(st.bquat, (size_t)R * 4); DA(st.obs_bag, (size_t)R * MQE_OBS_BAG); DA(st.wobs, packed_floats(s)); set_packed(s, st.wobs);
  DA(st.rsum, (size_t)N * MQE_MAX_REWARD_TERMS); DA(st.sheep_avg, (size_t)N * 2); DA(st.sheep_var, N);
  DA(st.sub_dof_vel, (size_t)N * 4 * 12 * A); DA(st.sub_exceed, (size_t)N * 4 * 12 * A); DA(st.overflow, 2 * (size_t)N);
  DA(st.sub_tau, (size_t)N * 4 * 12 * A); DA(st.npc_noise, (size_t)N * (P ? P : 1) * 3);
  DA(st.w_last, (size_t)N * MQE_MAX_AGENTS); DA(st.w_last2, (size_t)N * 2); DA(st.cmd, (size_t)R * 3);
  DA(st.ep_len, N); DA(st.reset_count, N); DA(st.last_dof_vel, (size_t)R * 12);
  DA(st.env_origins_live, (size_t)N * 3); DA(st.curr_xy, (size_t)N * 2); DA(st.terrain_levels, N); DA(st.npc_pre, (size_t)N * (P ? P : 1) * 13);
  if (hipMemcpy(st.env_origins_live, d->env_origins, (size_t)N * 12, hipMemcpyHostToDevice) != hipSuccess) return fail(-5, "upload");
  if (d->terrain_curriculum && hipMemcpy(st.terrain_levels, d->terrain_levels, (size_t)N * 4, hipMemcpyHostToDevice) != hipSuccess) return fail(-5, "upload");
  {
    std::vector<float> dp((size_t)R * 8, 0.0f);
    const uint32_t seed = (uint32_t)d->seed;
    for (int e = 0; e < N; e++) {
      const uint32_t genv = (uint32_t)(e + d->env_id_offset);
      float mu = d->friction;
      if (d->rand_friction) {
        const uint32_t bucket = mqe_hash(seed, genv, MQE_RNG_CREATE, 0) % 64u;
        mu = d->friction_lo + (d->friction_hi - d->friction_lo) * mqe_u01(seed, bucket, MQE_RNG_CREATE + 1u, 0);
      }
      for (int a = 0; a < A; a++) {
        float* p = dp.data() + ((size_t)e * A + a) * 8;
        p[0] = mu;
        if (d->rand_base_mass) p[1] = d->added_mass_lo + (d->added_mass_hi - d->added_mass_lo) * mqe_u01(seed, genv, MQE_RNG_CREATE, 16u + (uint32_t)a);
        if (d->rand_com)
          for (int k = 0; k < 3; k++) p[2 + k] = d->com_lo[k] + (d->com_hi[k] - d->com_lo[k]) * mqe_u01(seed, genv, MQE_RNG_CREATE, 32u + (uint32_t)(a * 3 + k));
      }
    }
    DA(st.dparams, (size_t)R * 8);
    if (hipMemcpy(st.dparams, dp.data(), dp.size() * 4, hipMemcpyHostToDevice) != hipSuccess) return fail(-5, "upload");
  }
  st.lag_buf = nullptr;
  if (s->hm.lag_steps > 0) { DA(st.lag_buf, (size_t)(s->hm.lag_steps + 1) * R * 12); }
  DA(st.reset_buf, N); DA(st.collide_buf, N); DA(st.time_out, N); DA(st.r_term, N); DA(st.p_term, N); DA(st.zh_term, N);
  DA(st.w_have_last, N); DA(st.w_delayed_reset, N);
  s->reg_state = false;
  {
    std::vector<float> h((size_t)N * (A + P) * 13, 0.0f);
    for (size_t i = 0; i < (size_t)N * (A + P); i++) h[i * 13 + 6] = 1.0f;
    HIPCHK(hipMemcpy(st.root, h.data(), h.size() * 4, hipMemcpyHostToDevice));
    std::vector<float> lo((size_t)R * MQE_FRAME, 0.0f), pg((size_t)R * 3, 0.0f), bq((size_t)R * 4, 0.0f);
    for (int i = 0; i < R; i++) { memcpy(&lo[(size_t)i * MQE_FRAME], d->command_obs, 70 * 4); pg[i * 3 + 2] = -1.0f; bq[i * 4 + 3] = 1.0f; }
    HIPCHK(hipMemcpy(st.loco_obs, lo.data(), lo.size() * 4, hipMemcpyHostToDevice));
    HIPCHK(hipMemcpy(st.pg, pg.data(), pg.size() * 4, hipMemcpyHostToDevice));
    HIPCHK(hipMemcpy(st.bquat, bq.data(), bq.size() * 4, hipMemcpyHostToDevice));
    HIPCHK(hipMemset(st.reset_buf, 1, N));
  }
  return 0;
}

static int stage_tensors(mqe_sim* s) {
  DevModel& m = s->hm;
  DevState& st = s->st;
  DevModel* dmp;
  if (dalloc(s, &dmp, 1)) return fail(-5, "alloc");
  mqe_fill_hot(m);
  HIPCHK(hipMemcpy(dmp, &m, sizeof m, hipMemcpyHostToDevice));
  s->dm = dmp;
  void** t = s->tens;
  t[MQE_T_ROOT_STATE] = st.root; t[MQE_T_DOF_STATE] = st.dof; t[MQE_T_CONTACT_FORCE] = st.cf; t[MQE_T_TORQUES] = st.torques;
  t[MQE_T_ACTIONS] = st.actions; t[MQE_T_LAST_ACTIONS] = st.last_actions; t[MQE_T_LOCOMOTION_OBS] = st.loco_obs;
  t[MQE_T_HISTORY] = st.hist; t[MQE_T_LAST_LOCO_ACTION] = st.last_loco; t[MQE_T_LAST_TWO_LOCO_ACTION] = st.last_two_loco;
  t[MQE_T_ACT_HIST] = st.act_hist; t[MQE_T_GAIT_INDICES] = st.gait; t[MQE_T_CLOCK_INPUTS] = st.clock;
  t[MQE_T_BASE_LIN_VEL] = st.blv; t[MQE_T_BASE_ANG_VEL] = st.bav; t[MQE_T_PROJECTED_GRAVITY] = st.pg; t[MQE_T_BASE_QUAT] = st.bquat;
  t[MQE_T_EPISODE_LENGTH] = st.ep_len; t[MQE_T_RESET_BUF] = st.reset_buf; t[MQE_T_COLLIDE_BUF] = st.collide_buf;
  t[MQE_T_TIME_OUT_BUF] = st.time_out; t[MQE_T_R_TERM] = st.r_term; t[MQE_T_P_TERM] = st.p_term; t[MQE_T_Z_HIGH_TERM] = st.zh_term;
  t[MQE_T_OBS_BAG] = st.obs_bag; t[MQE_T_WRAPPER_OBS] = st.wobs; t[MQE_T_WRAPPER_REWARD] = st.wrew; t[MQE_T_REWARD_SUMS] = st.rsum;
  t[MQE_T_SHEEP_POS_AVG] = st.sheep_avg; t[MQE_T_SHEEP_POS_VAR] = st.sheep_var; t[MQE_T_RESET_COUNT] = st.reset_count;
  t[MQE_T_SUBSTEP_TORQUES] = st.sub_tau; t[MQE_T_NPC_NOISE] = st.npc_noise; t[MQE_T_WRAPPER_PACKED] = st.wobs;
  t[MQE_T_DOMAIN_PARAMS] = st.dparams;
  t[MQE_T_SUBSTEP_DOF_VEL] = st.sub_dof_vel; t[MQE_T_SUBSTEP_EXCEED_DOF_POS_LIMITS] = st.sub_exceed; t[MQE_T_CONTACT_OVERFLOW] = st.overflow;
  t[MQE_T_ENV_ORIGINS] = st.env_origins_live; t[MQE_T_TERRAIN_LEVELS] = st.terrain_levels;
  t[MQE_T_CONTACT_REDUCED] = st.overflow + s->N;
  return 0;
}

extern "C" int mqe_sim_create(const mqe_sim_desc* d, mqe_sim** out) {
  if (int rc = check_create_args(d, out)) return rc;
  mqe_sim* s = new mqe_sim();
  struct Guard { mqe_sim* s; ~Guard() { if (s) mqe_sim_destroy(s); } } guard{s};
  s->d = *d;
  s->sw = read_switches();
  static int (*const stages[])(mqe_sim*) = {stage_model, stage_variant, stage_scene, stage_actuator, stage_policy, stage_work_buffers, stage_state, stage_tensors};
  for (auto stage : stages)
    if (int rc = stage(s)) return rc;
  HIPCHK(hipDeviceSynchronize());
  guard.s = nullptr;
  *out = s;
  return 0;
}
#undef UP
#undef DA

extern "C" int mqe_sim_destroy(mqe_sim* s) {
  if (!s) return 0;
  hipDeviceSynchronize();
  for (void* p : s->allocs) hipFree(p);
  for (int k = 0; k < PROF_N; k++) {
    for (auto e : s->ev0[k]) hipEventDestroy(e);
    for (auto e : s->ev1[k]) hipEventDestroy(e);
  }
  delete s;
  return 0;
}

static int rbs_alloc(mqe_sim* s) {
  if (s->rbs) return 0;
  if (s->NBR > RBS_THREADS) return fail(-4, "the rigid-body state kernel holds one env's rows in a workgroup: more than 256 reported bodies per env");
  RbsArgs& ra = s->rbs_args;
  memset(&ra, 0, sizeof ra);
  ra.epg = RBS_THREADS / s->NBR;
  const mqe_robot_model& rm = s->d.robot;
  for (int leg = 0; leg < 4; leg++)
    for (int q = 0; q < rm.n_prims && q < MQE_MAX_PRIMS; q++)
      if (rm.prim_reported[q] == 4 + 4 * leg && rm.prim_type[q] == MQE_PRIM_SPHERE && rm.prim_body[q] == 3 + 3 * leg)
        for (int k = 0; k < 3; k++) ra.foot[leg][k] = rm.prim_center[q][k];
  if (dalloc(s, &s->rbs, (size_t)s->N * s->NBR * 13)) return fail(-5, "device alloc failed (rigid-body state tensor)");
  ra.out = s->rbs;
  s->tens[MQE_T_RIGID_BODY_STATE] = s->rbs;
  return 0;
}
static void launch_rbs(mqe_sim* s, hipStream_t q) {
  hipLaunchKernelGGL(k_rigid_body_state, dim3((s->N + s->rbs_args.epg - 1) / s->rbs_args.epg), dim3(RBS_THREADS), 0, q, s->dm, s->st, s->rbs_args);
}

extern "C" int mqe_sim_tensor(mqe_sim* s, int kind, mqe_tensor_view* v) {
  if (!s || !v || kind < 0 || kind >= MQE_T_COUNT) return fail(-1, "bad tensor kind");
  memset(v, 0, sizeof *v);
  if (kind == MQE_T_RIGID_BODY_STATE) { if (int rc = rbs_alloc(s)) return rc; }
  v->ptr = s->tens[kind];
  const int N = s->N, A = s->A, P = s->P, R = s->R;
#define SH(nd, a, b, c, e, dt_) do { v->ndim = nd; v->shape[0] = a; v->shape[1] = b; v->shape[2] = c; v->shape[3] = e; v->dtype = dt_; } while (0)
  switch (kind) {
    case MQE_T_ROOT_STATE: SH(3, N, A + P, 13, 0, 0); break;
    case MQE_T_DOF_STATE: SH(3, N, s->ND, 2, 0, 0); break;
    case MQE_T_CONTACT_FORCE: SH(3, N, s->NBR, 3, 0, 0); break;
    case MQE_T_TORQUES: case MQE_T_ACTIONS: case MQE_T_LAST_ACTIONS: SH(2, N, 12 * A, 0, 0, 0); break;
    case MQE_T_LOCOMOTION_OBS: SH(2, R, MQE_FRAME, 0, 0, 0); break;
    case MQE_T_HISTORY: SH(3, R, MQE_HIST, MQE_FRAME, 0, 0); break;
    case MQE_T_LAST_LOCO_ACTION: case MQE_T_LAST_TWO_LOCO_ACTION: SH(2, R, 12, 0, 0, 0); break;
    case MQE_T_ACT_HIST: SH(3, 4, R, 12, 0, 0); break;
    case MQE_T_GAIT_INDICES: SH(1, R, 0, 0, 0, 0); break;
    case MQE_T_CLOCK_INPUTS: case MQE_T_BASE_QUAT: SH(2, R, 4, 0, 0, 0); break;
    case MQE_T_BASE_LIN_VEL: case MQE_T_BASE_ANG_VEL: case MQE_T_PROJECTED_GRAVITY: SH(2, R, 3, 0, 0, 0); break;
    case MQE_T_EPISODE_LENGTH: case MQE_T_RESET_COUNT: SH(1, N, 0, 0, 0, 1); break;
    case MQE_T_RESET_BUF: case MQE_T_COLLIDE_BUF: case MQE_T_TIME_OUT_BUF: case MQE_T_R_TERM: case MQE_T_P_TERM:
    case MQE_T_Z_HIGH_TERM: SH(1, N, 0, 0, 0, 2); break;
    case MQE_T_OBS_BAG: SH(2, R, MQE_OBS_BAG, 0, 0, 0); break;
    case MQE_T_WRAPPER_OBS: SH(3, N, s->Aw, s->D, 0, 0); break;
    case MQE_T_WRAPPER_REWARD: SH(2, N, s->Aw, 0, 0, 0); break;
    case MQE_T_REWARD_SUMS: SH(2, N, MQE_MAX_REWARD_TERMS, 0, 0, 0); break;
    case MQE_T_SHEEP_POS_AVG: SH(2, N, 2, 0, 0, 0); break;
    case MQE_T_SHEEP_POS_VAR: SH(1, N, 0, 0, 0, 0); break;
    case MQE_T_SUBSTEP_TORQUES: case MQE_T_SUBSTEP_DOF_VEL: SH(3, N, 4, 12 * A, 0, 0); break;
    case MQE_T_SUBSTEP_EXCEED_DOF_POS_LIMITS: SH(3, N, 4, 12 * A, 0, 2); break;
    case MQE_T_CONTACT_OVERFLOW: case MQE_T_TERRAIN_LEVELS: case MQE_T_CONTACT_REDUCED: SH(1, N, 0, 0, 0, 1); break;
    case MQE_T_ENV_ORIGINS: SH(2, N, 3, 0, 0, 0); break;
    case MQE_T_NPC_NOISE: SH(3, N, P, 3, 0, 0); break;
    case MQE_T_WRAPPER_PACKED: SH(1, (int)packed_floats(s), 0, 0, 0, 0); break;
    case MQE_T_DOMAIN_PARAMS: SH(2, s->R, 8, 0, 0, 0); break;
    case MQE_T_RIGID_BODY_STATE: SH(3, N, s->NBR, 13, 0, 0); break;
  }
  return 0;
}

static inline long prof_phase(int every) { return every > 2 ? 2 : 0; }
struct ProfScope {
  mqe_sim* s; int k; hipStream_t q; hipEvent_t e1;
  ProfScope(mqe_sim* s_, int k_, hipStream_t q_) : s(s_), k(k_), q(q_), e1(nullptr) {
    if (!s->prof_now) return;
    hipEvent_t e0;
    hipEventCreate(&e0); hipEventCreate(&e1);
    hipEventRecord(e0, q);
    s->ev0[k].push_back(e0); s->ev1[k].push_back(e1);
  }
  ~ProfScope() { if (e1) hipEventRecord(e1, q); }
};

extern "C" int mqe_profile_enable(mqe_sim* s, int on) {
  if (!s) return fail(-1, "null engine handle");
  s->prof = on != 0;
  s->prof_every = on > 0 ? on : 1;
  s->prof_step = 0;
  s->prof_now = s->prof;
  return 0;
}
extern "C" int mqe_profile_read(mqe_sim* s, float* ms, int n, int* n_launches) {
  if (!s) return fail(-1, "null engine handle");
  HIPCHK(hipDeviceSynchronize());
  for (int k = 0; k < PROF_N; k++) {
    for (size_t i = 0; i < s->ev0[k].size(); i++) {
      float t = 0;
      hipEventElapsedTime(&t, s->ev0[k][i], s->ev1[k][i]);
      s->prof_ms[k] += t; s->prof_cnt[k] += 1;
      hipEventDestroy(s->ev0[k][i]); hipEventDestroy(s->ev1[k][i]);
    }
    s->ev0[k].clear(); s->ev1[k].clear();
  }
  for (int k = 0; k < PROF_N && k < n; k++) ms[k] = s->prof_ms[k];
  for (int k = 0; k < PROF_N && PROF_N + k < n; k++) ms[PROF_N + k] = (float)s->prof_cnt[k];
  if (n_launches) *n_launches = s->prof_cnt[PROF_GEMM_L0];
  memset(s->prof_ms, 0, sizeof s->prof_ms);
  memset(s->prof_cnt, 0, sizeof s->prof_cnt);
  return 0;
}

static void launch_gemm(hipStream_t q, const float* A, int lda, int rot4, int ring4, const GemmLayer& L, float* C, int ldc, int M, int act_cols) {
  GemmArgs g;
  g.A = A; g.lda = lda; g.a_rot4 = rot4; g.a_ring4 = ring4; g.Wt = L.Wt; g.ldw = L.Npad; g.bias = L.bias;
  g.C = C; g.ldc = ldc; g.M = M; g.N = L.Npad; g.K = L.Kpad; g.act_cols = act_cols;
  int grid = ((M + GB_M - 1) / GB_M) * (L.Npad / GB_N);
  hipLaunchKernelGGL(k_gemm_f32, dim3(grid), dim3(256), 0, q, g);
}

static void launch_gemm2(hipStream_t q, const uint16_t* A, int lda, int rot8, int ring8, const GemmLayer& L,
                         float* C, int ldc, int M, int act_cols, const unsigned* irr = nullptr, const float* ring = nullptr, int ring_pos = 0, bool use_half = true, long long* times = nullptr, int times_blocks = 0) {
  Gemm2Args g;
  g.times = times; g.times_blocks = times_blocks;
  g.irr = irr; g.ring = ring; g.ring_pos = ring_pos; g.Wt32 = L.Wt; g.ldwt = L.Npad;
  g.A = A; g.lda = lda; g.a_rot8 = rot8; g.a_ring8 = ring8;
  g.W = L.W2; g.ldw = 2 * L.Kpad3; g.bias = L.bias;
  g.C = C; g.ldc = ldc; g.M = M; g.N = L.Npad; g.K = L.Kpad3; g.act_cols = act_cols;
  g.descale = 1.0f / (MQE_H2_ASCALE * L.wscale);
  int full_tiles, half_tiles;
  h2_tiling(M, L.Npad / H2_N, use_half, &full_tiles, &half_tiles);
  g.full_blocks = full_tiles * (L.Npad / H2_N); g.full_rows = full_tiles * H2_M;
  const int grid = (full_tiles + half_tiles) * (L.Npad / H2_N);
  if (half_tiles == 0) hipLaunchKernelGGL(k_gemm_h2, dim3(grid), dim3(H2_THREADS), H2_LDS_BYTES, q, g);
  else hipLaunchKernelGGL(k_gemm_h2_mix, dim3(grid), dim3(H2_THREADS), H2_LDS_BYTES, q, g);
}

static void policy_head(mqe_sim* s, const float* command, hipStream_t q, const float* wrapper_actions) {
  const int R = s->R;
  const int slot = s->hist_pos;
  s->hist_pos = (s->hist_pos + 1) % MQE_HIST;
  {
    ProfScope ps(s, PROF_MISC, q);
    hipLaunchKernelGGL(k_pre_policy, dim3((R + 3) / 4), dim3(256), 0, q, s->dm, s->st, command, slot, wrapper_actions);
  }
  {
    ProfScope ps(s, PROF_GEMM_L0, q);
    if (s->gemm_split)
      launch_gemm2(q, s->st.hist2, 2 * MQE_HIST * MQE_H2_FRAME, s->hist_pos * (MQE_H2_FRAME / 8), MQE_HIST * MQE_H2_FRAME / 8, s->l0,
                   s->P1, s->ldP1, R, s->ada_h0, s->st.hist_irr, s->st.hist, s->hist_pos, s->gemm_half, s->tail_times, (R + TL_ROWS - 1) / TL_ROWS);
    else
      launch_gemm(q, s->st.hist, MQE_HIST * MQE_FRAME, s->hist_pos * (MQE_FRAME / 4), MQE_HIST * MQE_FRAME / 4, s->l0, s->P1, s->ldP1, R, s->ada_h0);
  }
}
static void launch_chain(mqe_sim* s, hipStream_t q, const std::vector<GemmLayer>& layers, const float* x, int ldx, float* out, int ldout) {
  for (size_t l = 0; l < layers.size(); l++) {
    const bool last = l + 1 == layers.size();
    float* y = last ? out : ((l & 1) ? s->bufB : s->bufA);
    const int ldy = last ? ldout : s->ldbuf;
    launch_gemm(q, x, ldx, 0, 0, layers[l], y, ldy, s->R, last ? 0 : layers[l].Npad);
    x = y; ldx = ldy;
  }
}
static int policy_tail(mqe_sim* s, hipStream_t q) {
  const int R = s->R;
  ProfScope ps(s, PROF_GEMM_REST, q);
  if (s->tail_fused) {
    TailArgs t;
    t.P1 = s->P1; t.ldp = s->ldP1; t.ada_h0 = s->ada_h0;
    auto tl = [](const GemmLayer& L) { TailLayer r; r.W = L.Wfrag; r.bias = L.bias; r.descale = 1.0f / (TL_ASCALE * L.fscale); return r; };
    t.a1 = tl(s->ada_rest[0]); t.a2 = tl(s->ada_rest[1]);
    t.wl0 = s->w_lat0; t.wl1 = s->w_lat1;
    t.b1 = tl(s->body_rest[0]); t.b2 = tl(s->body_rest[1]); t.b3 = tl(s->body_rest[2]);
    t.lat = s->lat; t.ldl = s->ldlat; t.act = s->act_out; t.lda = s->ldact;
    t.last_loco = s->st.last_loco; t.last_two_loco = s->st.last_two_loco; t.actions = s->st.actions; t.clip_actions = s->hm.clip_actions;
    t.R = R;
    t.block0 = (int)(((long long)s->d.env_id_offset * s->A) / TL_ROWS);
    t.times = s->tail_times;
    hipLaunchKernelGGL(k_policy_tail, dim3((R + TL_ROWS - 1) / TL_ROWS), dim3(TL_THREADS), TL_LDS_BYTES, q, t);
    return 0;
  }
  launch_chain(s, q, s->ada_rest, s->P1, s->ldP1, s->lat, s->ldlat);
  {
    int n = R * s->body_h0;
    hipLaunchKernelGGL(k_body_l0_finish, dim3((n + 255) / 256), dim3(256), 0, q, s->P1, s->ldP1, s->ada_h0, s->body_h0,
                       (const float*)s->lat, s->ldlat, (const float*)s->w_lat0, (const float*)s->w_lat1, R);
  }
  launch_chain(s, q, s->body_rest, s->P1 + s->ada_h0, s->ldP1, s->act_out, s->ldact);
  int n = R * 12;
  hipLaunchKernelGGL(k_post_policy, dim3((n + 255) / 256), dim3(256), 0, q, s->dm, s->st, (const float*)s->act_out, s->ldact);
  return 0;
}

static int launched() { HIPCHK(hipGetLastError()); return 0; }
static int policy_step(mqe_sim* s, const float* command, hipStream_t q, const float* wrapper_actions = nullptr) {
  policy_head(s, command, q, wrapper_actions);
  return policy_tail(s, q);
}

static void advance_lag(mqe_sim* s, int n) { if (s->d.lag_timesteps > 0) s->lag_pos = (s->lag_pos + n) % (s->d.lag_timesteps + 1); }
static void launch_torques(mqe_sim* s, int dec_i, hipStream_t q) {
  ProfScope ps(s, PROF_TORQUES, q);
  int n = s->R * 12;
  if (s->d.control_type == MQE_CTRL_C)
    hipLaunchKernelGGL(k_compute_torques_mfma, dim3((n + 127) / 128), dim3(256), 0, q, s->dm, s->st, dec_i, s->lag_pos);
  else
    hipLaunchKernelGGL(k_compute_torques, dim3((n + 255) / 256), dim3(256), 0, q, s->dm, s->st, dec_i, s->lag_pos);
  advance_lag(s, 1);
}
static void launch_simulate(mqe_sim* s, hipStream_t q) {
  ProfScope ps(s, PROF_SIMULATE, q);
  PhysDebug dbg = {nullptr, nullptr, nullptr, 0, nullptr, -1};
  if (s->dbg_stop_phase >= 0) {
    dbg.stop_after = s->dbg_stop_phase;
    hipLaunchKernelGGL(k_simulate_a2, dim3(s->N), dim3(64), s->phys_lds_bytes, q, s->dm, s->st, 0, s->dbg_stop_phase < 100 ? 1 : 0, dbg);
    return;
  }
  hipLaunchKernelGGL(k_simulate, dim3(s->N), dim3(64), s->phys_lds_bytes, q, s->dm, s->st, 0, 0, dbg);
}
__global__ void k_post_decimation(const DevModel* m, DevState st, int dec_i) {
  const int idx = blockIdx.x * blockDim.x + threadIdx.x;
  const int nj = 12 * m->A;
  if (idx >= m->N * nj) return;
  const int e = idx / nj, jt = idx - e * nj, j = jt % 12;
  const size_t o = ((size_t)e * 4 + dec_i) * nj + jt;
  const float q = st.dof[((size_t)e * m->ND + jt) * 2], qd = st.dof[((size_t)e * m->ND + jt) * 2 + 1];
  st.sub_tau[o] = st.torques[idx];
  substep_log(m, st.sub_dof_vel, st.sub_exceed, o, j, q, qd);
}
__global__ void k_set_joint_actions(const DevModel* m, DevState st, const float* __restrict__ a12) {
  const int idx = blockIdx.x * blockDim.x + threadIdx.x;
  if (idx < m->R * 12) st.actions[idx] = clampf(a12[idx], -m->clip_actions, m->clip_actions);
}

static void launch_post_decimation(mqe_sim* s, int dec_i, hipStream_t q) {
  const int n = s->N * 12 * s->A;
  hipLaunchKernelGGL(k_post_decimation, dim3((n + 255) / 256), dim3(256), 0, q, s->dm, s->st, dec_i);
}
static void launch_curriculum_snapshot(mqe_sim* s, hipStream_t q) {
  if (s->hm.curriculum) hipLaunchKernelGGL(k_curriculum_snapshot, dim3((s->N + 255) / 256), dim3(256), 0, q, s->dm, s->st);
}
struct PostStep { int step_no, push_count; };
static PostStep begin_post_step(mqe_sim* s, bool advance = true) {
  const int step_no = s->n_post_steps + 1, every = s->d.push_interval;
  if (advance) s->n_post_steps = step_no;
  return {step_no, (every > 0 && step_no % every == 0) ? step_no / every : 0};
}
static void launch_post(mqe_sim* s, hipStream_t q, int wrapper_level) {
  ProfScope ps(s, PROF_POST, q);
  const PostStep p = begin_post_step(s);
  launch_curriculum_snapshot(s, q);
  const auto post = s->hm.A <= 2 ? k_post_physics<2> : k_post_physics<MQE_MAX_AGENTS>;
  hipLaunchKernelGGL(post, dim3((s->N + POST_EPW - 1) / POST_EPW), dim3(64), 0, q, s->dm, s->st, wrapper_level, p.push_count, p.step_no);
}

static int run_substeps_and_post(mqe_sim* s, hipStream_t q, int wrapper_level = 1) {
  if (s->fuse_substeps) {
    ProfScope ps(s, PROF_SIMULATE, q);
    PostArgs pa = {0, 0, 0, 0};
    const bool fuse_post = s->fuse_post && !s->rbs_refresh;
    if (fuse_post) {
      const PostStep p = begin_post_step(s);
      pa.on = 1; pa.wrapper_level = wrapper_level; pa.step_no = p.step_no; pa.push_count = p.push_count;
    }
    hipLaunchKernelGGL(s->substeps_fn, dim3((s->N + s->substeps_epw - 1) / s->substeps_epw), dim3(64), s->phys_lds_bytes * s->substeps_epw, q, s->dm, s->st, s->d.decimation, s->lag_pos, pa);
    advance_lag(s, s->d.decimation);
    if (fuse_post) {
      s->prof_now = s->prof;
      return launched();
    }
  } else {
    for (int k = 0; k < s->d.decimation; k++) {
      launch_torques(s, k < 4 ? k : 3, q);
      launch_simulate(s, q);
      launch_post_decimation(s, k < 4 ? k : 3, q);
    }
  }
  if (s->rbs_refresh) launch_rbs(s, q);
  launch_post(s, q, wrapper_level);
  s->prof_now = s->prof;
  return launched();
}

struct StateHeader { uint32_t magic, abi; int32_t N, A, P, nbuf; int32_t hist_pos, n_post_steps, lag_pos, reserved; uint64_t bytes; };
static const uint32_t STATE_MAGIC = 0x5345514du;
extern "C" long long mqe_state_size(mqe_sim* s) {
  if (!s) { fail(-1, "null engine handle"); return 0; }
  size_t n = sizeof(StateHeader);
  for (auto& b : s->state_bufs) n += (b.second + 15) / 16 * 16;
  return (long long)n;
}
extern "C" int mqe_state_save(mqe_sim* s, void* host_blob, void* stream) {
  if (!s || !host_blob) return fail(-1, "mqe_state_save: null argument");
  if (s->step_open) return fail(-8, "mqe_state_save inside an open step (mqe_step_begin / _head without mqe_step_end)");
  HIPCHK(hipStreamSynchronize((hipStream_t)stream));
  StateHeader h = {STATE_MAGIC, (uint32_t)MQE_ABI_VERSION, s->N, s->A, s->P, (int32_t)s->state_bufs.size(), s->hist_pos, s->n_post_steps, s->lag_pos, 0,
                   (uint64_t)mqe_state_size(s)};
  char* o = (char*)host_blob;
  memcpy(o, &h, sizeof h); o += sizeof h;
  for (auto& b : s->state_bufs) {
    HIPCHK(hipMemcpy(o, b.first, b.second, hipMemcpyDeviceToHost));
    o += (b.second + 15) / 16 * 16;
  }
  return 0;
}
extern "C" int mqe_state_load(mqe_sim* s, const void* host_blob, void* stream) {
  if (!s || !host_blob) return fail(-1, "mqe_state_load: null argument");
  if (s->step_open) return fail(-8, "mqe_state_load inside an open step");
  StateHeader h;
  memcpy(&h, host_blob, sizeof h);
  if (h.magic != STATE_MAGIC || h.abi != (uint32_t)MQE_ABI_VERSION) return fail(-6, "mqe_state_load: not a state blob of this ABI version");
  if (h.N != s->N || h.A != s->A || h.P != s->P || h.nbuf != (int32_t)s->state_bufs.size() || h.bytes != (uint64_t)mqe_state_size(s))
    return fail(-6, "mqe_state_load: the blob was saved from a handle of another shape (envs, agents, NPCs, layer-0 path)");
  HIPCHK(hipStreamSynchronize((hipStream_t)stream));
  const char* o = (const char*)host_blob + sizeof h;
  for (auto& b : s->state_bufs) {
    HIPCHK(hipMemcpy(b.first, o, b.second, hipMemcpyHostToDevice));
    o += (b.second + 15) / 16 * 16;
  }
  s->hist_pos = h.hist_pos; s->n_post_steps = h.n_post_steps; s->lag_pos = h.lag_pos;
  return 0;
}
extern "C" int mqe_render_depth(mqe_sim* s, float* out_dev, int height, int width, float horizontal_fov_deg, const float* cam_pos3, const float* cam_rpy3,
                                float far_m, void* stream) {
  if (!s || !out_dev || !cam_pos3 || !cam_rpy3) return fail(-1, "null argument");
  if (height <= 0 || width <= 0 || height * width > 1 << 16) return fail(-6, "camera resolution out of range");
  if (!(horizontal_fov_deg > 1.0f && horizontal_fov_deg < 179.0f) || !(far_m > 0.0f)) return fail(-6, "camera field of view / far plane out of range");
  CamArgs ca;
  ca.out = out_dev; ca.H = height; ca.W = width; ca.tan_half_h = tanf(0.5f * horizontal_fov_deg * 3.14159265358979f / 180.0f);
  for (int k = 0; k < 3; k++) { ca.pos[k] = cam_pos3[k]; ca.rpy[k] = cam_rpy3[k]; }
  ca.far_ = far_m;
  hipLaunchKernelGGL(k_depth_camera, dim3(s->N), dim3(256), 0, (hipStream_t)stream, s->dm, s->st, ca);
  return hipGetLastError() == hipSuccess ? 0 : fail(-4, "k_depth_camera launch failed");
}
extern "C" int mqe_refresh_rigid_body_state(mqe_sim* s, void* stream) {
  if (!s) return fail(-1, "null engine handle");
  if (int rc = rbs_alloc(s)) return rc;
  launch_rbs(s, (hipStream_t)stream);
  return hipGetLastError() == hipSuccess ? 0 : fail(-4, "k_rigid_body_state launch failed");
}
extern "C" int mqe_set_rigid_body_refresh(mqe_sim* s, int on) {
  if (!s) return fail(-1, "null engine handle");
  if (s->step_open) return fail(-8, "mqe_set_rigid_body_refresh inside an open step");
  if (on) { if (int rc = rbs_alloc(s)) return rc; }
  s->rbs_refresh = on != 0;
  return 0;
}
extern "C" int mqe_history_sync(mqe_sim* s, void* stream) {
  if (!s) return fail(-1, "null engine handle");
  if (!s->st.hist2) return 0;
  hipStream_t q = (hipStream_t)stream;
  if (hipMemsetAsync(s->st.hist_irr, 0, (size_t)s->R * sizeof(uint32_t), q) != hipSuccess) return fail(-4, "memset failed");
  const int n = s->R * MQE_HIST;
  hipLaunchKernelGGL(k_hist2_rebuild, dim3((n + 255) / 256), dim3(256), 0, q, s->dm, s->st, s->hist_pos);
  return hipGetLastError() == hipSuccess ? 0 : fail(-4, "k_hist2_rebuild launch failed");
}
static int copy_times(long long* out_host, const long long* src, size_t offset, size_t count, const char* refusal) {
  if (!src) return fail(-4, refusal);
  HIPCHK(hipDeviceSynchronize());
  HIPCHK(hipMemcpy(out_host, src + offset, count * sizeof(long long), hipMemcpyDeviceToHost));
  return 0;
}
static const char* const NEEDS_PHASE_TIMES = "create the handle with MQE_PHASE_TIMES=1 (go1gate-, go1sheep- or go1football-defender-shaped scene)";
extern "C" int mqe_debug_phase_times(mqe_sim* s, long long* out_host) {
  if (!s) return fail(-1, "null engine handle");
  return copy_times(out_host, s->phase_timed ? s->st.wave_times : nullptr, (size_t)4 * s->N, (size_t)64 * s->N, NEEDS_PHASE_TIMES);
}
extern "C" int mqe_debug_epilogue_times(mqe_sim* s, long long* out_host) {
  if (!s) return fail(-1, "null engine handle");
  return copy_times(out_host, s->phase_timed ? s->st.wave_times : nullptr, (size_t)68 * s->N, (size_t)16 * s->N, NEEDS_PHASE_TIMES);
}
extern "C" int mqe_debug_tail_times(mqe_sim* s, long long* out_host) {
  if (!s) return fail(-1, "null engine handle");
  return copy_times(out_host, s->tail_times, 0, (size_t)16 * ((s->R + TL_ROWS - 1) / TL_ROWS), "create the handle with MQE_TAIL_TIMES=1 (fused policy tail)");
}
extern "C" int mqe_debug_wave_times(mqe_sim* s, long long* out_host) {
  if (!s) return fail(-1, "null engine handle");
  return copy_times(out_host, s->st.wave_times, 0, (size_t)4 * s->N, "create the handle with MQE_WAVE_TIMES=1");
}
extern "C" int mqe_debug_stop_phase(mqe_sim* s, int tap) {
  if (!s) return fail(-1, "null engine handle");
  if (tap >= 0 && !s->shape->a2) return fail(-4, "phase taps exist for two-robot scenes without objects only (k_simulate_a2)");
  s->dbg_stop_phase = tap < 0 ? -1 : tap;
  return 0;
}
extern "C" int mqe_policy_step(mqe_sim* s, const float* command, void* stream) {
  if (!s) return fail(-1, "null engine handle");
  policy_step(s, command, (hipStream_t)stream);
  return launched();
}
extern "C" int mqe_defender_command(mqe_sim* s, float* out_dev, void* stream) {
  if (!s) return fail(-1, "null engine handle");
  if (s->d.task != MQE_TASK_FOOTBALL_DEFENDER) return fail(-7, "defender command needs the football-defender task");
  hipLaunchKernelGGL(k_defender_command, dim3((s->N + 63) / 64), dim3(64), 0, (hipStream_t)stream, s->dm, s->st, out_dev);
  return launched();
}
extern "C" int mqe_compute_torques(mqe_sim* s, void* stream) {
  if (!s) return fail(-1, "null engine handle");
  launch_torques(s, -1, (hipStream_t)stream);
  return launched();
}
extern "C" int mqe_simulate(mqe_sim* s, void* stream) {
  if (!s) return fail(-1, "null engine handle");
  launch_simulate(s, (hipStream_t)stream);
  return launched();
}
extern "C" int mqe_post_decimation_step(mqe_sim* s, int dec_i, void* stream) {
  if (!s) return fail(-1, "null engine handle");
  if (dec_i < 0 || dec_i >= 4) return fail(-1, "dec_i out of range");
  launch_post_decimation(s, dec_i, (hipStream_t)stream);
  return launched();
}
extern "C" int mqe_post_physics_step(mqe_sim* s, void* stream) {
  if (!s) return fail(-1, "null engine handle");
  if (s->rbs_refresh) launch_rbs(s, (hipStream_t)stream);
  launch_post(s, (hipStream_t)stream, 0);
  return launched();
}
extern "C" int mqe_post_physics_stage(mqe_sim* s, int stages, void* stream) {
  if (!s) return fail(-1, "null engine handle");
  if ((stages & ~(MQE_POST_ALL | MQE_POST_WRAPPER_LEVEL)) != 0 || (stages & MQE_POST_ALL) == 0) return fail(-2, "mqe_post_physics_stage: stages must be an OR of MQE_POST_*");
  hipStream_t q = (hipStream_t)stream;
  const PostStep p = begin_post_step(s, (stages & MQE_POST_WRAPPER) != 0);
  if ((stages & MQE_POST_FRAME) && s->rbs_refresh) launch_rbs(s, q);
  if (stages & MQE_POST_RESET) launch_curriculum_snapshot(s, q);
  hipLaunchKernelGGL(k_post_staged, dim3((s->N + 63) / 64), dim3(64), 0, q, s->dm, s->st, stages & MQE_POST_ALL, (stages & MQE_POST_WRAPPER_LEVEL) ? 1 : 0, p.push_count, p.step_no);
  return launched();
}
extern "C" int mqe_wrapper_eval(mqe_sim* s, int is_reset_call, void* stream) {
  if (!s) return fail(-1, "null engine handle");
  hipLaunchKernelGGL(k_wrapper_eval, dim3((s->N + 63) / 64), dim3(64), 0, (hipStream_t)stream, s->dm, s->st, is_reset_call);
  return launched();
}
extern "C" int mqe_set_actor_root_state_indexed(mqe_sim*, const int32_t*, int, void*) { return 0; }
extern "C" int mqe_set_dof_state_indexed(mqe_sim*, const int32_t*, int, void*) { return 0; }

extern "C" int mqe_reset_all(mqe_sim* s, void* stream) {
  if (!s) return fail(-1, "null engine handle");
  hipStream_t q = (hipStream_t)stream;
  launch_curriculum_snapshot(s, q);
  hipLaunchKernelGGL(k_reset_all, dim3((s->N + 63) / 64), dim3(64), 0, q, s->dm, s->st, s->n_post_steps == 0 ? 1 : 0);
  int n = s->R * (MQE_HIST * MQE_FRAME / 4);
  hipLaunchKernelGGL(k_reset_history, dim3((n + 255) / 256), dim3(256), 0, q, s->dm, s->st);
  return launched();
}

static int begin_step(mqe_sim* s, const char* name, bool hierarchical, const char* control_msg, const char* open_msg, bool wrapper_actions) {
  if (!s) return fail(-1, "null engine handle");
  if ((s->d.control_type == MQE_CTRL_C) != hierarchical) return fail(-7, control_msg, name);
  if (open_msg && s->step_open) return fail(-8, open_msg, name);
  if (wrapper_actions && s->cmd_general)
    return fail(-7, "%s takes wrapper-level (N, A', 3) actions; this handle's command layout (desc.command_src) is served by mqe_policy_step + the stage entry points", name);
  s->prof_now = s->prof && (s->prof_step++ % s->prof_every == prof_phase(s->prof_every));
  return 0;
}
static const char* const DRIVES_C = "%s drives the hierarchical controller (control type C)";
static const char* const DRIVES_C_NOT_JOINT = "%s drives the hierarchical controller (control type C); use mqe_step_joint for P / V / T";
static const char* const NOT_CLOSED = "%s: the previous step was not closed with mqe_step_end";

extern "C" int mqe_step_joint(mqe_sim* s, const float* actions12, void* stream) {
  if (int rc = begin_step(s, "mqe_step_joint", false, "%s drives control types P / V / T; use mqe_step for the hierarchical controller", nullptr, false)) return rc;
  hipStream_t q = (hipStream_t)stream;
  {
    ProfScope ps(s, PROF_MISC, q);
    const int n = s->R * 12;
    hipLaunchKernelGGL(k_set_joint_actions, dim3((n + 255) / 256), dim3(256), 0, q, s->dm, s->st, actions12);
  }
  return run_substeps_and_post(s, q);
}

extern "C" int mqe_step_command(mqe_sim* s, const float* command, void* stream) {
  if (int rc = begin_step(s, "mqe_step_command", true, DRIVES_C_NOT_JOINT, "%s inside an open step", false)) return rc;
  hipStream_t q = (hipStream_t)stream;
  policy_step(s, command, q);
  return run_substeps_and_post(s, q, 0);
}

extern "C" int mqe_step(mqe_sim* s, const float* actions, void* stream) {
  if (int rc = begin_step(s, "mqe_step", true, DRIVES_C_NOT_JOINT, nullptr, true)) return rc;
  hipStream_t q = (hipStream_t)stream;
  policy_step(s, s->st.cmd, q, actions);
  return run_substeps_and_post(s, q);
}

extern "C" int mqe_step_begin(mqe_sim* s, const float* actions, void* stream) {
  if (int rc = begin_step(s, "mqe_step_begin", true, DRIVES_C, NOT_CLOSED, true)) return rc;
  policy_step(s, s->st.cmd, (hipStream_t)stream, actions);
  s->step_open = 2;
  return launched();
}

extern "C" int mqe_step_head(mqe_sim* s, const float* actions, void* stream) {
  if (int rc = begin_step(s, "mqe_step_head", true, DRIVES_C, NOT_CLOSED, true)) return rc;
  policy_head(s, s->st.cmd, (hipStream_t)stream, actions);
  s->step_open = 1;
  return launched();
}

extern "C" int mqe_step_tail(mqe_sim* s, void* stream) {
  if (!s) return fail(-1, "null engine handle");
  if (s->step_open != 1) return fail(-8, "mqe_step_tail without mqe_step_head");
  policy_tail(s, (hipStream_t)stream);
  s->step_open = 2;
  return launched();
}

extern "C" int mqe_set_return_buffer(mqe_sim* s, float* packed_dev) {
  if (!s) return fail(-1, "mqe_set_return_buffer: no engine");
  set_packed(s, packed_dev ? packed_dev : (float*)s->tens[MQE_T_WRAPPER_PACKED]);
  return 0;
}

extern "C" int mqe_step_end(mqe_sim* s, void* stream) {
  if (!s) return fail(-1, "null engine handle");
  if (s->step_open != 2) return fail(-8, "mqe_step_end without mqe_step_begin (or mqe_step_head + mqe_step_tail)");
  s->step_open = 0;
  return run_substeps_and_post(s, (hipStream_t)stream);
}

static thread_local long long t_dbg_times[16];
extern "C" int mqe_debug_times(long long* out16) { memcpy(out16, t_dbg_times, sizeof t_dbg_times); return 0; }
extern "C" int mqe_debug_dynamics(mqe_sim* s, int env, int robot, float* minv_out_host, int* nc_out_host, float* contacts_out_host) {
  if (!s) return fail(-1, "null engine handle");
  struct Scratch { void* p = nullptr; ~Scratch() { if (p) hipFree(p); } } minv, con, nc, tm;
  HIPCHK(hipMalloc(&minv.p, 324 * 4)); HIPCHK(hipMalloc(&con.p, 64 * 8 * 4)); HIPCHK(hipMalloc(&nc.p, 4)); HIPCHK(hipMalloc(&tm.p, 16 * 8));
  HIPCHK(hipMemset(tm.p, 0, 16 * 8));
  PhysDebug dbg = {(float*)minv.p, (int*)nc.p, (float*)con.p, robot, (long long*)tm.p, -1};
  hipLaunchKernelGGL(k_simulate, dim3(1), dim3(64), s->phys_lds_bytes, 0, s->dm, s->st, env, 1, dbg);
  HIPCHK(hipDeviceSynchronize());
  HIPCHK(hipMemcpy(minv_out_host, minv.p, 324 * 4, hipMemcpyDeviceToHost));
  HIPCHK(hipMemcpy(nc_out_host, nc.p, 4, hipMemcpyDeviceToHost));
  HIPCHK(hipMemcpy(contacts_out_host, con.p, 64 * 8 * 4, hipMemcpyDeviceToHost));
  HIPCHK(hipMemcpy(t_dbg_times, tm.p, 16 * 8, hipMemcpyDeviceToHost));
  return 0;
}
```

Measured before the change: 40.09 million.

## Fold the newest history frame into the fused policy tail as a small late GEMM

```diff
diff --git a/multiagent-quadruped-environment_amd/csrc/kernels_gemm.hpp b/multiagent-quadruped-environment_amd/csrc/kernels_gemm.hpp
--- a/multiagent-quadruped-environment_amd/csrc/kernels_gemm.hpp
+++ b/multiagent-quadruped-environment_amd/csrc/kernels_gemm.hpp
@@ -101,7 +101,7 @@
   int M, N, K;
   int act_cols;
   float descale;
-  const unsigned* irr; const float* ring; int ring_pos;
+  const unsigned* irr; const float* ring; int ring_pos; int p_skip;
   const float* Wt32; int ldwt;
   int full_blocks, full_rows;
   long long* times; int times_blocks;
@@ -235,7 +235,7 @@
         const int s1 = __ffs((int)mk) - 1;
         mk &= mk - 1;
         const int p = s1 >= g.ring_pos ? s1 - g.ring_pos : s1 + MQE_HIST - g.ring_pos;
-        if (p == 0) continue;
+        if (p == 0 || p == g.p_skip) continue;
         const int s0 = s1 > 0 ? s1 - 1 : MQE_HIST - 1;
         const float* a2 = g.ring + ((size_t)grow * MQE_HIST + s1) * MQE_FRAME + 54;
         const float* a1 = g.ring + ((size_t)grow * MQE_HIST + s0) * MQE_FRAME + 42;
diff --git a/multiagent-quadruped-environment_amd/csrc/kernels_step.hpp b/multiagent-quadruped-environment_amd/csrc/kernels_step.hpp
--- a/multiagent-quadruped-environment_amd/csrc/kernels_step.hpp
+++ b/multiagent-quadruped-environment_amd/csrc/kernels_step.hpp
@@ -134,7 +134,12 @@
   r.v = v;
   return r;
 }
-__device__ __forceinline__ void pre_policy_store(const DevModel* m, const DevState& st, int hist_slot, bool have_wrapper_actions, int i, int c, const PreVal& r) {
+#define MQE_LT_K 64
+#define MQE_LT_OLD0 MQE_H2_FRAME
+#define MQE_LT_STRIDE (MQE_LT_K + 8)
+#define MQE_LT_PLANE (32 * MQE_LT_STRIDE)
+__device__ __forceinline__ void pre_policy_store(const DevModel* m, const DevState& st, int hist_slot, bool have_wrapper_actions, int i, int c, const PreVal& r,
+                                                 uint16_t* tile = nullptr) {
   const float v = r.v;
   st.loco_obs[(size_t)i * MQE_FRAME + c] = v;
   st.hist[((size_t)i * MQE_HIST + hist_slot) * MQE_FRAME + c] = v;
@@ -147,6 +152,11 @@
       split2(c < 70 ? v : 1.0f, MQE_H2_ASCALE, h, l);
       const size_t k = (size_t)hist_slot * MQE_H2_FRAME + cc;
       row2[h2_index(k, 0)] = h; row2[h2_index(k, 1)] = l;
+      if (tile) { tile[cc] = h; tile[MQE_LT_PLANE + cc] = l; }
+    } else if (cc == -2 && tile) {
+      uint16_t h, l;
+      split2(r.aux, MQE_H2_ASCALE, h, l);
+      tile[MQE_LT_OLD0 + (c - 54)] = h; tile[MQE_LT_PLANE + MQE_LT_OLD0 + (c - 54)] = l;
     } else if (cc == -2) {
       const int oldest = hist_slot + 1 >= MQE_HIST ? 0 : hist_slot + 1;
       int slot = oldest + MQE_H2_CARRIER0 + (c - 54); if (slot >= MQE_HIST) slot -= MQE_HIST;
@@ -154,44 +164,40 @@
       split2(r.aux, MQE_H2_ASCALE, h, l);
       const size_t k = (size_t)slot * MQE_H2_FRAME + MQE_H2_CARRIER_COL;
       row2[h2_index(k, 0)] = h; row2[h2_index(k, 1)] = l;
-    } else if (c == 71) st.hist_irr[i] = r.mk;
-  }
-}
-__device__ __forceinline__ void pre_policy_element(const DevModel* m, const DevState& st, const float* __restrict__ command, int hist_slot,
-                                                   const float* __restrict__ wrapper_actions, int i, int c) {
+    } else if (c == 71) {
+      st.hist_irr[i] = r.mk;
+      if (tile) {
+        const size_t k = (size_t)hist_slot * MQE_H2_FRAME + MQE_H2_CARRIER_COL;
+        row2[h2_index(k, 0)] = 0; row2[h2_index(k, 1)] = 0;
+      }
+    }
+  }
+}
+__device__ __forceinline__ PreVal pre_policy_element(const DevModel* m, const DevState& st, const float* __restrict__ command, int hist_slot,
+                                                     const float* __restrict__ wrapper_actions, int i, int c, uint16_t* tile = nullptr) {
   const PreVal r = pre_policy_load(m, st, command, hist_slot, wrapper_actions, i, c);
-  pre_policy_store(m, st, hist_slot, wrapper_actions != nullptr, i, c, r);
-}
-
-__global__ void __launch_bounds__(256) k_pre_policy(const DevModel* m, DevState st, const float* __restrict__ command, int hist_slot,
-                                                    const float* __restrict__ wrapper_actions) {
-  const int lane = threadIdx.x & 63;
-  const int i = blockIdx.x * (blockDim.x >> 6) + (threadIdx.x >> 6);
-  if (i >= m->R) return;
-  const int A = m->A, Aw = m->Aw, task = m->task, clip_command = m->clip_command;
-  const float lin = m->cmd_lin_scale, ang = m->cmd_ang_scale;
+  pre_policy_store(m, st, hist_slot, wrapper_actions != nullptr, i, c, r, tile);
+  return r;
+}
+__device__ __forceinline__ bool pre_policy_per_element(const DevModel* m, bool wrap, int i) {
+  return m->cmd_general || (wrap && m->task == MQE_TASK_FOOTBALL_DEFENDER && i % m->A == 2);
+}
+
+struct PreWave { float x1[2], x2[2], x4[2]; unsigned mk; };
+__device__ __forceinline__ void pre_policy_wave_load(const DevModel* m, const DevState& st, const float* __restrict__ command, int hist_slot,
+                                                     const float* __restrict__ wrapper_actions, int i, int lane, PreWave& w) {
+  const int A = m->A, Aw = m->Aw;
   const int e = i / A, a = i - e * A;
   const bool wrap = wrapper_actions != nullptr;
-  if (m->cmd_general || (wrap && task == MQE_TASK_FOOTBALL_DEFENDER && a == 2)) {
-    pre_policy_element(m, st, command, hist_slot, wrapper_actions, i, lane);
-    if (lane < MQE_FRAME - 64) pre_policy_element(m, st, command, hist_slot, wrapper_actions, i, 64 + lane);
-    return;
-  }
   const bool h2 = st.hist2 != nullptr;
   const float* ob = st.obs_bag + (size_t)i * MQE_OBS_BAG;
   const int oldest = hist_slot + 1 >= MQE_HIST ? 0 : hist_slot + 1, prev = hist_slot > 0 ? hist_slot - 1 : MQE_HIST - 1;
   const float* hist_i = st.hist + (size_t)i * MQE_HIST * MQE_FRAME;
-  const unsigned mk = h2 ? st.hist_irr[i] : 0u;
-  float x1[2], x2[2], x3[2], x4[2];
-  bool on[2], cmdc[2], actc[2];
-  int cc[2];
+  w.mk = h2 ? st.hist_irr[i] : 0u;
 #pragma unroll
   for (int q = 0; q < 2; q++) {
     const int c = q * 64 + lane;
-    cc[q] = c;
-    on[q] = c < MQE_FRAME;
-    cmdc[q] = c >= 3 && c < 6;
-    actc[q] = c >= 54 && c < 66;
+    const bool on = c < MQE_FRAME, cmdc = c >= 3 && c < 6, actc = c >= 54 && c < 66;
     const float* a1 = ob;
     if (c < 3) a1 = ob + 60 + c;
     else if (c < 6) a1 = ob;
@@ -201,21 +207,28 @@
     else if (c < 66) a1 = st.last_two_loco + (size_t)i * 12 + (c - 54);
     else if (c < 70) a1 = ob + (c - 3);
     const float* a2 = ob;
-    if (cmdc[q]) a2 = wrap ? (a < Aw ? wrapper_actions + ((size_t)e * Aw + a) * 3 + (c - 3) : st.cmd + i * 3 + (c - 3)) : command + i * 3 + (c - 3);
-    const float* a3 = ob;
+    if (cmdc) a2 = wrap ? (a < Aw ? wrapper_actions + ((size_t)e * Aw + a) * 3 + (c - 3) : st.cmd + i * 3 + (c - 3)) : command + i * 3 + (c - 3);
     const float* a4 = ob;
-    if (actc[q] && h2) { a3 = hist_i + oldest * MQE_FRAME + c; a4 = hist_i + prev * MQE_FRAME + (c - 12); }
-    x1[q] = on[q] ? *a1 : 0.0f; x2[q] = on[q] ? *a2 : 0.0f; x3[q] = on[q] ? *a3 : 0.0f; x4[q] = on[q] ? *a4 : 0.0f;
-  }
+    if (actc && h2) { a2 = hist_i + oldest * MQE_FRAME + c; a4 = hist_i + prev * MQE_FRAME + (c - 12); }
+    w.x1[q] = on ? *a1 : 0.0f; w.x2[q] = on ? *a2 : 0.0f; w.x4[q] = on ? *a4 : 0.0f;
+  }
+}
+__device__ __forceinline__ bool pre_policy_wave_store(const DevModel* m, const DevState& st, int hist_slot, bool wrap, int i, int lane, const PreWave& w,
+                                                      uint16_t* tile = nullptr) {
+  const int A = m->A, Aw = m->Aw, task = m->task, clip_command = m->clip_command;
+  const float lin = m->cmd_lin_scale, ang = m->cmd_ang_scale;
+  const int a = i % A;
+  const bool h2 = st.hist2 != nullptr;
   PreVal r[2];
   bool differs = false;
 #pragma unroll
   for (int q = 0; q < 2; q++) {
-    const int c = cc[q];
-    float v = (c < 70 && !cmdc[q]) ? x1[q] : 0.0f;
+    const int c = q * 64 + lane;
+    const bool on = c < MQE_FRAME, cmdc = c >= 3 && c < 6, actc = c >= 54 && c < 66;
+    float v = (c < 70 && !cmdc) ? w.x1[q] : 0.0f;
     r[q].aux = 0.0f; r[q].mk = 0u;
-    if (cmdc[q]) {
-      float x = x2[q];
+    if (cmdc) {
+      float x = w.x2[q];
       if (wrap) {
         if (a < Aw) {
           if (task != MQE_TASK_TUG) x = clampf(x, -1.0f, 1.0f);
@@ -226,17 +239,33 @@
       if (clip_command) x = clampf(x, -1.0f, 1.0f);
       v = x * (c < 5 ? lin : ang);
     }
-    if (actc[q] && h2) {
-      r[q].aux = x3[q];
-      differs = differs || (on[q] && __float_as_uint(x4[q]) != __float_as_uint(x1[q]));
+    if (actc && h2) {
+      r[q].aux = w.x2[q];
+      differs = differs || (on && __float_as_uint(w.x4[q]) != __float_as_uint(w.x1[q]));
     }
     r[q].v = v;
   }
   const bool diff = __ballot(differs) != 0ull;
   const unsigned bit = 1u << hist_slot;
-  if (lane == MQE_FRAME - 1 - 64) r[1].mk = diff ? (mk | bit) : (mk & ~bit);
-  pre_policy_store(m, st, hist_slot, wrap, i, lane, r[0]);
-  if (lane < MQE_FRAME - 64) pre_policy_store(m, st, hist_slot, wrap, i, 64 + lane, r[1]);
+  if (lane == MQE_FRAME - 1 - 64) r[1].mk = diff ? (w.mk | bit) : (w.mk & ~bit);
+  pre_policy_store(m, st, hist_slot, wrap, i, lane, r[0], tile);
+  if (lane < MQE_FRAME - 64) pre_policy_store(m, st, hist_slot, wrap, i, 64 + lane, r[1], tile);
+  return diff;
+}
+__global__ void __launch_bounds__(256) k_pre_policy(const DevModel* m, DevState st, const float* __restrict__ command, int hist_slot,
+                                                    const float* __restrict__ wrapper_actions) {
+  const int lane = threadIdx.x & 63;
+  const int i = blockIdx.x * (blockDim.x >> 6) + (threadIdx.x >> 6);
+  if (i >= m->R) return;
+  const bool wrap = wrapper_actions != nullptr;
+  if (pre_policy_per_element(m, wrap, i)) {
+    pre_policy_element(m, st, command, hist_slot, wrapper_actions, i, lane);
+    if (lane < MQE_FRAME - 64) pre_policy_element(m, st, command, hist_slot, wrapper_actions, i, 64 + lane);
+    return;
+  }
+  PreWave w;
+  pre_policy_wave_load(m, st, command, hist_slot, wrapper_actions, i, lane, w);
+  pre_policy_wave_store(m, st, hist_slot, wrap, i, lane, w);
 }
 
 __global__ void k_post_policy(const DevModel* m, DevState st, const float* __restrict__ act, int ld) {
@@ -1054,7 +1083,7 @@
   }
 }
 
-__global__ void k_hist2_rebuild(const DevModel* m, DevState st, int oldest) {
+__global__ void k_hist2_rebuild(const DevModel* m, DevState st, int oldest, int late) {
   const int idx = blockIdx.x * blockDim.x + threadIdx.x;
   const int i = idx / MQE_HIST, slot = idx - i * MQE_HIST;
   if (i >= m->R || !st.hist2) return;
@@ -1078,7 +1107,7 @@
   row2[h2_index(k, 0)] = h; row2[h2_index(k, 1)] = l;
   int p = slot - oldest; if (p < 0) p += MQE_HIST;
   float carry = 0.0f;
-  if (p >= MQE_H2_CARRIER0 && p < MQE_H2_CARRIER0 + 12) carry = st.hist[((size_t)i * MQE_HIST + oldest) * MQE_FRAME + 54 + (p - MQE_H2_CARRIER0)];
+  if (!late && p >= MQE_H2_CARRIER0 && p < MQE_H2_CARRIER0 + 12) carry = st.hist[((size_t)i * MQE_HIST + oldest) * MQE_FRAME + 54 + (p - MQE_H2_CARRIER0)];
   split2(carry, MQE_H2_ASCALE, h, l);
   k = (size_t)slot * MQE_H2_FRAME + MQE_H2_CARRIER_COL;
   row2[h2_index(k, 0)] = h; row2[h2_index(k, 1)] = l;
@@ -1087,6 +1116,15 @@
   unsigned diff = 0u;
   for (int j = 0; j < 12; j++) diff |= __float_as_uint(pa[j]) ^ __float_as_uint(fr[54 + j]);
   if (diff) atomicOr(&st.hist_irr[i], 1u << slot);
+}
+
+__global__ void k_hist2_zero_carrier(const DevModel* m, DevState st) {
+  const int idx = blockIdx.x * blockDim.x + threadIdx.x;
+  const int i = idx / MQE_HIST, slot = idx - i * MQE_HIST;
+  if (i >= m->R || !st.hist2) return;
+  uint16_t* row2 = st.hist2 + (size_t)i * (2 * MQE_HIST * MQE_H2_FRAME);
+  const size_t k = (size_t)slot * MQE_H2_FRAME + MQE_H2_CARRIER_COL;
+  row2[h2_index(k, 0)] = 0; row2[h2_index(k, 1)] = 0;
 }
 
 __global__ void __launch_bounds__(64) k_post_staged(const DevModel* m, DevState st, int stages, int wrapper_level, int push_count, int step_no) {
diff --git a/multiagent-quadruped-environment_amd/csrc/kernels_tail.hpp b/multiagent-quadruped-environment_amd/csrc/kernels_tail.hpp
--- a/multiagent-quadruped-environment_amd/csrc/kernels_tail.hpp
+++ b/multiagent-quadruped-environment_amd/csrc/kernels_tail.hpp
@@ -1,5 +1,6 @@
 #pragma once
 #include "mqe_common.hpp"
+#include "kernels_step.hpp"
 #include "kernels_gemm.hpp"
 
 #define TL_ROWS 32
@@ -15,6 +16,10 @@
 #define TL_PZ (TL_ROWS * TL_SZ)
 #define TL_C (64 + 640 + 1024 + 32 * 33)
 #define TL_LDS_BYTES (2 * TL_PX + 2 * TL_PY + 2 * TL_PZ + TL_C * 4)
+#define TL_LS (768 + 4)
+#define TL_LATE_LDS_BYTES (TL_LDS_BYTES + 2 * MQE_LT_PLANE * 2 + TL_ROWS * 4)
+static_assert(TL_ROWS * TL_LS * 4 <= 2 * TL_PX + 2 * TL_PY + 2 * TL_PZ, "late-frame staging");
+static_assert(TL_LATE_LDS_BYTES <= 160 * 1024, "LDS");
 #define TL_ASCALE 1.0f
 
 struct TailLayer { const uint16_t* W; const float* bias; float descale; };
@@ -28,6 +33,10 @@
   float *last_loco, *last_two_loco, *actions; float clip_actions;
   int R;
   int block0;
+  const DevModel* m; DevState st;
+  const float *command, *wrapper_actions; int hist_slot;
+  TailLayer l0p;
+  const float* Wt32; int ldwt;
   long long* times;
 };
 #define TL_STAMP(i) do { if (g.times != nullptr && tid == 0) g.times[(size_t)blockIdx.x * 16 + (i)] = (long long)wall_clock64(); } while (0)
@@ -89,7 +98,9 @@
   }
 }
 
+template <bool LATE>
 __global__ void __launch_bounds__(TL_THREADS, 1) k_policy_tail(TailArgs g) {
+  static_assert(!LATE || TL_THREADS == 512, "the late-frame order is written for eight wavefronts");
   constexpr int TLT = TL_THREADS, NW = TLT / 64, NT4 = 8 / NW, QH = 2048 / TLT, QB = 4096 / TLT;
   constexpr int D1 = TLT == 256 ? 16 : 8;
   extern __shared__ __attribute__((aligned(16))) unsigned char tl_lds[];
@@ -101,6 +112,8 @@
   float* wL0 = bB3 + 64;   float* wL1 = wL0 + 512;  float* nar = wL1 + 512;
   const int tid = threadIdx.x, lane = tid & 63, wave = __builtin_amdgcn_readfirstlane(tid >> 6);
   const int r0 = blockIdx.x * TL_ROWS;
+  uint16_t* At = reinterpret_cast<uint16_t*>(nar + 32 * 33);
+  int* diffS = reinterpret_cast<int*>(At + 2 * MQE_LT_PLANE);
   TL_STAMP(0);
   const int krot = ((blockIdx.x + g.block0) * 7) & 31;
   const int frow = lane & 31, fhalf = lane >> 5;
@@ -110,8 +123,16 @@
   const h2_gvec* Wb2 = (const h2_gvec*)(g.b2.W) + lane;
   const h2_gvec* Wb3 = (const h2_gvec*)(g.b3.W) + lane;
   TlRing<16, 1, D1> q1;  TlRing<8, 1, 8> q2;
-  if (wave < 4) tl_fill(Wa1 + wave * (16 * 128), 0, krot, q1);
-  if (wave == 0) tl_fill(Wa2, 0, 0, q2);
+  TlRing<4, 3, 4> qL;  PreWave pw[4];
+  const h2_gvec* WL = (const h2_gvec*)(g.l0p.W) + lane + (3 * wave) * (4 * 128);
+  if constexpr (LATE) {
+#pragma unroll
+    for (int j = 0; j < 4; j++) pre_policy_wave_load(g.m, g.st, g.command, g.hist_slot, g.wrapper_actions, min(r0 + wave * 4 + j, g.R - 1), lane, pw[j]);
+    tl_fill(WL, 4 * 128, 0, qL);
+  } else {
+    if (wave < 4) tl_fill(Wa1 + wave * (16 * 128), 0, krot, q1);
+    if (wave == 0) tl_fill(Wa2, 0, 0, q2);
+  }
   float4 vh[QH], vb[QB];
 #pragma unroll
   for (int q = 0; q < QH; q++) {
@@ -125,6 +146,51 @@
   }
   float ll_pre = 0.0f;
   if constexpr (TLT >= TL_ROWS * 12) { const int row = tid / 12; if (tid < TL_ROWS * 12 && r0 + row < g.R) ll_pre = g.last_loco[(size_t)r0 * 12 + tid]; }
+  if constexpr (LATE) {
+    __builtin_amdgcn_sched_barrier(0);
+    const bool wrap = g.wrapper_actions != nullptr;
+    unsigned elem = 0u;
+#pragma unroll
+    for (int j = 0; j < 4; j++) {
+      const int rl = wave * 4 + j, i = r0 + rl;
+      uint16_t* trow = At + rl * MQE_LT_STRIDE;
+      bool diff = false;
+      if (i >= g.R) { trow[lane] = 0; trow[MQE_LT_PLANE + lane] = 0; }
+      else if (pre_policy_per_element(g.m, wrap, i)) elem |= 1u << j;
+      else diff = pre_policy_wave_store(g.m, g.st, g.hist_slot, wrap, i, lane, pw[j], trow);
+      if (lane == 0) diffS[rl] = diff ? 1 : 0;
+      if (lane < 5) {
+        const int k = lane == 0 ? MQE_H2_CARRIER_COL : MQE_LT_OLD0 + 11 + lane;
+        trow[k] = 0; trow[MQE_LT_PLANE + k] = 0;
+      }
+    }
+#pragma unroll 1
+    for (int j = 0; j < 4; j++) {
+      if (!((elem >> j) & 1u)) continue;
+      const int rl = wave * 4 + j, i = r0 + rl;
+      uint16_t* trow = At + rl * MQE_LT_STRIDE;
+      pre_policy_element(g.m, g.st, g.command, g.hist_slot, g.wrapper_actions, i, lane, trow);
+      PreVal e1; e1.mk = 0u;
+      if (lane < MQE_FRAME - 64) e1 = pre_policy_element(g.m, g.st, g.command, g.hist_slot, g.wrapper_actions, i, 64 + lane, trow);
+      const bool diff = __ballot(lane == MQE_FRAME - 1 - 64 && ((e1.mk >> g.hist_slot) & 1u)) != 0ull;
+      if (lane == 0) diffS[rl] = diff ? 1 : 0;
+    }
+    __syncthreads();
+    TL_STAMP(13);
+    f32x16 accL[3];
+#pragma unroll
+    for (int t = 0; t < 3; t++)
+#pragma unroll
+      for (int i = 0; i < 16; i++) accL[t][i] = 0.0f;
+    tl_mm(reinterpret_cast<const unsigned char*>(At) + frow * (MQE_LT_STRIDE * 2) + fhalf * 16, MQE_LT_PLANE * 2, WL, 4 * 128, 0, qL, accL);
+    float* stg = reinterpret_cast<float*>(tl_lds);
+#pragma unroll
+    for (int t = 0; t < 3; t++)
+#pragma unroll
+      for (int r = 0; r < 16; r++) stg[((r & 3) + 8 * (r >> 2) + 4 * (lane >> 5)) * TL_LS + (3 * wave + t) * 32 + (lane & 31)] = accL[t][r];
+    __builtin_amdgcn_sched_barrier(0);
+    if (wave < 4) tl_fill(Wa1 + wave * (16 * 128), 0, krot, q1);
+  }
   if constexpr (TLT == 512) {
     const float s0 = g.a1.bias[tid & 127], s1 = g.b2.bias[tid & 127], s2 = g.a2.bias[tid & 63], s3 = g.b3.bias[tid & 63], s4 = g.b1.bias[tid & 255],
                 s5 = g.wl0[tid], s6 = g.wl1[tid];
@@ -138,6 +204,48 @@
     for (int i = tid; i < 256; i += TLT) bB1[i] = g.b1.bias[i];
     for (int i = tid; i < 512; i += TLT) { wL0[i] = g.wl0[i]; wL1[i] = g.wl1[i]; }
   }
+  if constexpr (LATE) {
+    __syncthreads();
+    TL_STAMP(14);
+    const float* stg = reinterpret_cast<const float*>(tl_lds);
+    const float dl = g.l0p.descale;
+    const int prev = g.hist_slot > 0 ? g.hist_slot - 1 : MQE_HIST - 1;
+    auto resid = [&](int row, int col, float4& v) {
+      const int i = r0 + row;
+      const float* a2 = g.last_two_loco + (size_t)i * 12;
+      const float* a1 = g.st.hist + ((size_t)i * MQE_HIST + prev) * MQE_FRAME + 42;
+      const float* wr = g.Wt32 + (size_t)((MQE_HIST - 1) * MQE_FRAME + 54) * g.ldwt + col;
+      float4 cr = make_float4(0.f, 0.f, 0.f, 0.f);
+#pragma unroll 4
+      for (int j = 0; j < 12; j++) {
+        const float r = a2[j] - a1[j];
+        const float4 w = *reinterpret_cast<const float4*>(wr + (size_t)j * g.ldwt);
+        cr.x = fmaf(r, w.x, cr.x); cr.y = fmaf(r, w.y, cr.y); cr.z = fmaf(r, w.z, cr.z); cr.w = fmaf(r, w.w, cr.w);
+      }
+      v.x += cr.x; v.y += cr.y; v.z += cr.z; v.w += cr.w;
+    };
+#pragma unroll
+    for (int q = 0; q < QH; q++) {
+      const int idx = tid + TLT * q, row = idx >> 6, k4 = idx & 63;
+      const float4 p = *reinterpret_cast<const float4*>(stg + row * TL_LS + k4 * 4);
+      float4 v = vh[q];
+      v.x = fmaf(p.x, dl, v.x); v.y = fmaf(p.y, dl, v.y); v.z = fmaf(p.z, dl, v.z); v.w = fmaf(p.w, dl, v.w);
+      if (diffS[row]) resid(row, k4 * 4, v);
+      vh[q] = make_float4(elu_f(v.x), elu_f(v.y), elu_f(v.z), elu_f(v.w));
+    }
+#pragma unroll
+    for (int q = 0; q < QB; q++) {
+      const int idx = tid + TLT * q, row = idx >> 7, k4 = idx & 127;
+      const float4 p = *reinterpret_cast<const float4*>(stg + row * TL_LS + g.ada_h0 + k4 * 4);
+      float4 v = vb[q];
+      v.x = fmaf(p.x, dl, v.x); v.y = fmaf(p.y, dl, v.y); v.z = fmaf(p.z, dl, v.z); v.w = fmaf(p.w, dl, v.w);
+      if (diffS[row]) resid(row, g.ada_h0 + k4 * 4, v);
+      vb[q] = v;
+    }
+    __builtin_amdgcn_sched_barrier(0);
+    if (wave == 0) tl_fill(Wa2, 0, 0, q2);
+    __syncthreads();
+  }
 #pragma unroll
   for (int q = 0; q < QH; q++) {
     const int idx = tid + TLT * q, row = idx >> 6, k4 = idx & 63;
diff --git a/multiagent-quadruped-environment_amd/csrc/mqe_engine.hip b/multiagent-quadruped-environment_amd/csrc/mqe_engine.hip
--- a/multiagent-quadruped-environment_amd/csrc/mqe_engine.hip
+++ b/multiagent-quadruped-environment_amd/csrc/mqe_engine.hip
@@ -28,11 +28,11 @@
 
 enum SwitchKind { SW_FLAG, SW_INT };
 enum SwitchId { SW_VERBOSE, SW_LANE_SWEEP, SW_PHYS_LDS_PAD, SW_ACT_F32, SW_ENVS_PER_WAVE, SW_NO_FUSE_SUBSTEPS, SW_NO_FUSE_POST, SW_DEBUG_STOP_PHASE,
-                SW_GEMM_SPLIT, SW_GEMM_HALF, SW_NO_FUSED_TAIL, SW_TAIL_TIMES, SW_WAVE_TIMES, SW_PHASE_TIMES, SW_COUNT };
+                SW_GEMM_SPLIT, SW_GEMM_HALF, SW_NO_FUSED_TAIL, SW_LATE_FRAME, SW_TAIL_TIMES, SW_WAVE_TIMES, SW_PHASE_TIMES, SW_COUNT };
 static const struct { const char* name; SwitchKind kind; } SWITCH_LIST[SW_COUNT] = {
   {"MQE_VERBOSE", SW_FLAG}, {"MQE_LANE_SWEEP", SW_FLAG}, {"MQE_PHYS_LDS_PAD", SW_INT}, {"MQE_ACT_F32", SW_FLAG}, {"MQE_ENVS_PER_WAVE", SW_INT},
   {"MQE_NO_FUSE_SUBSTEPS", SW_FLAG}, {"MQE_NO_FUSE_POST", SW_FLAG}, {"MQE_DEBUG_STOP_PHASE", SW_INT}, {"MQE_GEMM_SPLIT", SW_INT},
-  {"MQE_GEMM_HALF", SW_INT}, {"MQE_NO_FUSED_TAIL", SW_FLAG}, {"MQE_TAIL_TIMES", SW_FLAG}, {"MQE_WAVE_TIMES", SW_FLAG}, {"MQE_PHASE_TIMES", SW_FLAG},
+  {"MQE_GEMM_HALF", SW_INT}, {"MQE_NO_FUSED_TAIL", SW_FLAG}, {"MQE_LATE_FRAME", SW_INT}, {"MQE_TAIL_TIMES", SW_FLAG}, {"MQE_WAVE_TIMES", SW_FLAG}, {"MQE_PHASE_TIMES", SW_FLAG},
 };
 struct Switches {
   const char* text[SW_COUNT];
@@ -90,6 +90,9 @@
   bool gemm_half = true;
   bool cmd_general = false;
   bool phase_timed = false;
+  bool late_frame = false;
+  GemmLayer l0p;
+  const float *late_command = nullptr, *late_wrapper = nullptr; int late_slot = 0;
   bool tail_fused = false;
   long long* tail_times = nullptr;
   size_t phys_lds_bytes = 0;
@@ -567,11 +570,35 @@
   for (int k = 0; k < 2100; k++) krow[k] = (k / 70) * MQE_FRAME + (k % 70);
   std::vector<int> k2row(2100);
   std::vector<float> k2scale(2100);
+  s->l0.Npad = rup(s->ada_h0 + s->body_h0, GB_N);
+  s->gemm_half = !sw.set(SW_GEMM_HALF) || sw.value[SW_GEMM_HALF] != 0;
+  const bool split = sw.set(SW_GEMM_SPLIT) ? sw.value[SW_GEMM_SPLIT] != 0 : l0_split_is_faster(R, s->l0.Npad / H2_N > 0 ? s->l0.Npad / H2_N : 1, s->gemm_half);
+  s->gemm_split = s->l0.Npad % H2_N == 0 && split && !s->cmd_general;
+  s->tail_fused = !sw.set(SW_NO_FUSED_TAIL) && ad.n_layers == 3 && bd.n_layers == 4 && ad.dims[1] == 256 && ad.dims[2] == 128 &&
+                  bd.dims[1] == 512 && bd.dims[2] == 256 && bd.dims[3] == 128;
+  s->late_frame = s->gemm_split && s->tail_fused && !(sw.set(SW_LATE_FRAME) && sw.value[SW_LATE_FRAME] == 0);
+  std::vector<int> klate(2100, -1);
   for (int k = 0; k < 2100; k++) {
     const int f = k / 70, c = k % 70, cc = h2_col(c);
+    if (s->late_frame && f == MQE_HIST - 1 && cc != -2) klate[k] = cc >= 0 ? cc : MQE_H2_FLAG_COL;
+    if (s->late_frame && f == 0 && cc == -2) klate[k] = MQE_LT_OLD0 + (c - 54);
     if (cc == -2) k2row[k] = f > 0 ? (f - 1) * MQE_H2_FRAME + h2_col(c - 12) : (MQE_H2_CARRIER0 + c - 54) * MQE_H2_FRAME + MQE_H2_CARRIER_COL;
     else k2row[k] = f * MQE_H2_FRAME + (cc >= 0 ? cc : MQE_H2_FLAG_COL);
     k2scale[k] = cc == -1 ? d->command_obs[c] : 1.0f;
+  }
+  if (s->late_frame) {
+    GemmLayer& P = s->l0p;
+    P.K = P.Kpad3 = MQE_LT_K; P.N = P.Npad = s->l0.Npad;
+    std::vector<double> acc((size_t)P.Npad * MQE_LT_K, 0.0);
+    for (int k = 0; k < 2100; k++) {
+      if (klate[k] < 0) continue;
+      for (int o = 0; o < s->ada_h0; o++) acc[(size_t)o * MQE_LT_K + klate[k]] += (double)ad.W[0][(size_t)o * 2100 + k] * (double)k2scale[k];
+      for (int o = 0; o < s->body_h0; o++) acc[(size_t)(s->ada_h0 + o) * MQE_LT_K + klate[k]] += (double)bd.W[0][(size_t)o * 2102 + k] * (double)k2scale[k];
+      k2scale[k] = 0.0f;
+    }
+    P.hW.resize(acc.size());
+    for (size_t i = 0; i < acc.size(); i++) P.hW[i] = (float)acc[i];
+    if (finalize_frag(s, &P)) return fail(-5, "upload");
   }
   if (make_layer(s, &s->l0, MQE_HIST * MQE_FRAME, s->ada_h0 + s->body_h0)) return fail(-5, "alloc");
   s->l0.Kpad3 = rup(MQE_HIST * MQE_H2_FRAME, H2_KMULT);
@@ -585,9 +612,6 @@
     UP(t, w0.data(), w0.size()); s->w_lat0 = (float*)t;
     UP(t, w1.data(), w1.size()); s->w_lat1 = (float*)t;
   }
-  s->gemm_half = !sw.set(SW_GEMM_HALF) || sw.value[SW_GEMM_HALF] != 0;
-  const bool split = sw.set(SW_GEMM_SPLIT) ? sw.value[SW_GEMM_SPLIT] != 0 : l0_split_is_faster(R, s->l0.Npad / H2_N > 0 ? s->l0.Npad / H2_N : 1, s->gemm_half);
-  s->gemm_split = s->l0.Npad % H2_N == 0 && split && !s->cmd_general;
   if (s->gemm_split) {
     if (finalize_layer(s, &s->l0)) return fail(-5, "upload");
     if (hipFuncSetAttribute((const void*)k_gemm_h2, hipFuncAttributeMaxDynamicSharedMemorySize, H2_LDS_BYTES) != hipSuccess ||
@@ -604,10 +628,9 @@
     if (make_layer(s, &g, bd.dims[l], bd.dims[l + 1]) || fill_layer(&g, 0, bd.W[l], bd.b[l], bd.dims[l + 1], bd.dims[l], bd.dims[l])) return fail(-5, "upload");
     s->body_rest.push_back(g);
   }
-  s->tail_fused = !sw.set(SW_NO_FUSED_TAIL) && ad.n_layers == 3 && bd.n_layers == 4 && ad.dims[1] == 256 && ad.dims[2] == 128 &&
-                  bd.dims[1] == 512 && bd.dims[2] == 256 && bd.dims[3] == 128;
   if (s->tail_fused) {
-    if (hipFuncSetAttribute((const void*)k_policy_tail, hipFuncAttributeMaxDynamicSharedMemorySize, TL_LDS_BYTES) != hipSuccess)
+    if (hipFuncSetAttribute((const void*)k_policy_tail<false>, hipFuncAttributeMaxDynamicSharedMemorySize, TL_LDS_BYTES) != hipSuccess ||
+        hipFuncSetAttribute((const void*)k_policy_tail<true>, hipFuncAttributeMaxDynamicSharedMemorySize, TL_LATE_LDS_BYTES) != hipSuccess)
       return fail(-4, "cannot raise dynamic LDS limit");
     for (auto& g : s->ada_rest) if (finalize_frag(s, &g)) return fail(-5, "upload");
     for (auto& g : s->body_rest) if (finalize_frag(s, &g)) return fail(-5, "upload");
@@ -856,10 +879,10 @@
 }
 
 static void launch_gemm2(hipStream_t q, const uint16_t* A, int lda, int rot8, int ring8, const GemmLayer& L,
-                         float* C, int ldc, int M, int act_cols, const unsigned* irr = nullptr, const float* ring = nullptr, int ring_pos = 0, bool use_half = true, long long* times = nullptr, int times_blocks = 0) {
+                         float* C, int ldc, int M, int act_cols, const unsigned* irr = nullptr, const float* ring = nullptr, int ring_pos = 0, bool use_half = true, long long* times = nullptr, int times_blocks = 0, int p_skip = -1) {
   Gemm2Args g;
   g.times = times; g.times_blocks = times_blocks;
-  g.irr = irr; g.ring = ring; g.ring_pos = ring_pos; g.Wt32 = L.Wt; g.ldwt = L.Npad;
+  g.irr = irr; g.ring = ring; g.ring_pos = ring_pos; g.p_skip = p_skip; g.Wt32 = L.Wt; g.ldwt = L.Npad;
   g.A = A; g.lda = lda; g.a_rot8 = rot8; g.a_ring8 = ring8;
   g.W = L.W2; g.ldw = 2 * L.Kpad3; g.bias = L.bias;
   g.C = C; g.ldc = ldc; g.M = M; g.N = L.Npad; g.K = L.Kpad3; g.act_cols = act_cols;
@@ -876,6 +899,13 @@
   const int R = s->R;
   const int slot = s->hist_pos;
   s->hist_pos = (s->hist_pos + 1) % MQE_HIST;
+  if (s->late_frame) {
+    s->late_command = command; s->late_wrapper = wrapper_actions; s->late_slot = slot;
+    ProfScope ps(s, PROF_GEMM_L0, q);
+    launch_gemm2(q, s->st.hist2, 2 * MQE_HIST * MQE_H2_FRAME, s->hist_pos * (MQE_H2_FRAME / 8), MQE_HIST * MQE_H2_FRAME / 8, s->l0,
+                 s->P1, s->ldP1, R, 0, s->st.hist_irr, s->st.hist, s->hist_pos, s->gemm_half, s->tail_times, (R + TL_ROWS - 1) / TL_ROWS, MQE_HIST - 1);
+    return;
+  }
   {
     ProfScope ps(s, PROF_MISC, q);
     hipLaunchKernelGGL(k_pre_policy, dim3((R + 3) / 4), dim3(256), 0, q, s->dm, s->st, command, slot, wrapper_actions);
@@ -913,7 +943,11 @@
     t.R = R;
     t.block0 = (int)(((long long)s->d.env_id_offset * s->A) / TL_ROWS);
     t.times = s->tail_times;
-    hipLaunchKernelGGL(k_policy_tail, dim3((R + TL_ROWS - 1) / TL_ROWS), dim3(TL_THREADS), TL_LDS_BYTES, q, t);
+    t.m = s->dm; t.st = s->st; t.command = s->late_command; t.wrapper_actions = s->late_wrapper; t.hist_slot = s->late_slot;
+    t.l0p.W = s->l0p.Wfrag; t.l0p.bias = nullptr; t.l0p.descale = 1.0f / (MQE_H2_ASCALE * s->l0p.fscale);
+    t.Wt32 = s->l0.Wt; t.ldwt = s->l0.Npad;
+    if (s->late_frame) hipLaunchKernelGGL(k_policy_tail<true>, dim3((R + TL_ROWS - 1) / TL_ROWS), dim3(TL_THREADS), TL_LATE_LDS_BYTES, q, t);
+    else hipLaunchKernelGGL(k_policy_tail<false>, dim3((R + TL_ROWS - 1) / TL_ROWS), dim3(TL_THREADS), TL_LDS_BYTES, q, t);
     return 0;
   }
   launch_chain(s, q, s->ada_rest, s->P1, s->ldP1, s->lat, s->ldlat);
@@ -1055,6 +1089,11 @@
     o += (b.second + 15) / 16 * 16;
   }
   s->hist_pos = h.hist_pos; s->n_post_steps = h.n_post_steps; s->lag_pos = h.lag_pos;
+  if (s->late_frame) {
+    const int n = s->R * MQE_HIST;
+    hipLaunchKernelGGL(k_hist2_zero_carrier, dim3((n + 255) / 256), dim3(256), 0, (hipStream_t)stream, s->dm, s->st);
+    return hipGetLastError() == hipSuccess ? 0 : fail(-4, "k_hist2_zero_carrier launch failed");
+  }
   return 0;
 }
 extern "C" int mqe_render_depth(mqe_sim* s, float* out_dev, int height, int width, float horizontal_fov_deg, const float* cam_pos3, const float* cam_rpy3,
@@ -1088,7 +1127,7 @@
   hipStream_t q = (hipStream_t)stream;
   if (hipMemsetAsync(s->st.hist_irr, 0, (size_t)s->R * sizeof(uint32_t), q) != hipSuccess) return fail(-4, "memset failed");
   const int n = s->R * MQE_HIST;
-  hipLaunchKernelGGL(k_hist2_rebuild, dim3((n + 255) / 256), dim3(256), 0, q, s->dm, s->st, s->hist_pos);
+  hipLaunchKernelGGL(k_hist2_rebuild, dim3((n + 255) / 256), dim3(256), 0, q, s->dm, s->st, s->hist_pos, s->late_frame ? 1 : 0);
   return hipGetLastError() == hipSuccess ? 0 : fail(-4, "k_hist2_rebuild launch failed");
 }
 static int copy_times(long long* out_host, const long long* src, size_t offset, size_t count, const char* refusal) {
```

After: 39.41 million. 0.983x the previous value.
